# jac99/Egonn

Hardware: AMD Instinct MI355X
Metric: LiDAR scans/sec (descriptor extraction), 50k-pt clouds @ 0.1m voxel (higher is better)
Workload: dtype f32

## Files before the change

### egonn_amd/_lib.py

```python
from __future__ import annotations

import ctypes as C
import os
from typing import List, Optional, Sequence

import numpy as np
import torch

_HERE = os.path.dirname(os.path.abspath(__file__))
LIB_PATH = os.path.join(_HERE, "lib", "libegonn_hip.so")

QUANT_CARTESIAN, QUANT_POLAR = 0, 1
FLAG_DISABLE_GLOBAL, FLAG_DISABLE_LOCAL, FLAG_IGNORE_KP_REGRESSOR, FLAG_BF16 = 1, 2, 4, 8
FLAG_POOL_SPOC, FLAG_POOL_MAC = 16, 32
MINKFPN_SPLIT_TOPDOWN = 1
MINKFPN_BLOCKS = {'BasicBlock': 0, 'ECABasicBlock': 1}
MINKFPN_POOLING = {None: 0, 'GeM': 1, 'MAC': 2, 'SPoC': 3}

_P = C.c_void_p
_SIGS = [
    ("egonn_ctx_create", C.c_int, [C.POINTER(_P), C.c_int, C.c_int]),
    ("egonn_ctx_destroy", None, [_P]),
    ("egonn_last_error", C.c_char_p, []),
    ("egonn_debug_set_naive_conv", C.c_int, [_P, C.c_int]),
    ("egonn_debug_set_ksplit", C.c_int, [_P, C.c_int, C.c_int, C.c_int, C.c_int, C.c_int]),
    ("egonn_debug_set_resident", C.c_int, [_P, C.c_int, C.c_int]),
    ("egonn_debug_keep_level_features", C.c_int, [_P, C.c_int]),
    ("egonn_debug_set_trace", C.c_int, [_P]),
    ("egonn_prepare_maps", C.c_int, [_P, C.c_int, _P]),
    ("egonn_debug_rowgroup_tables", C.c_int, [_P, C.c_int, C.c_int, _P, _P, C.c_int64, C.POINTER(C.c_int64), _P]),
    ("egonn_debug_rowgroup_perm", C.c_int, [_P, C.c_int, C.c_int, _P, C.c_int64, C.POINTER(C.c_int64), _P]),
    ("egonn_debug_radix_sort_scratch_bytes", C.c_int64, [C.c_int64, C.c_int]),
    ("egonn_debug_radix_sort", C.c_int, [_P, _P, _P, _P, C.c_int64, C.c_int, _P, _P, C.c_int, C.c_int, C.c_int,
                                         C.POINTER(C.c_int32), _P, C.c_int64, _P]),
    ("egonn_debug_dense_group3", C.c_int, [_P, _P, _P, _P, _P, _P, _P]),
    ("egonn_debug_global_tail_scratch_bytes", C.c_int64, [C.c_int64]),
    ("egonn_debug_global_tail", C.c_int, [_P, _P, C.c_int, C.c_int64, _P, _P, _P, _P, _P, _P, C.c_int, C.c_int, _P, _P, _P, C.c_int64, _P]),
    ("egonn_voxelize", C.c_int, [_P, _P, C.POINTER(C.c_int64), C.c_int, C.c_int, C.POINTER(C.c_float), _P]),
    ("egonn_ctx_reserve", C.c_int, [_P, C.c_int64, C.c_int, C.POINTER(C.c_int64)]),
    ("egonn_voxelize_device", C.c_int, [_P, _P, C.c_int64, _P, C.c_int, C.c_int, C.POINTER(C.c_float), _P]),
    ("egonn_plan_status", C.c_int, [_P, _P]),
    ("egonn_ctx_set_exact_fp32", C.c_int, [_P, C.c_int]),
    ("egonn_ctx_set_operand_autoscale", C.c_int, [_P, C.c_int]),
    ("egonn_level_capacity", C.c_int, [_P, C.c_int, C.POINTER(C.c_int64)]),
    ("egonn_graph_begin", C.c_int, [_P]),
    ("egonn_graph_end", C.c_int, [_P, C.POINTER(_P)]),
    ("egonn_graph_launch", C.c_int, [_P, _P]),
    ("egonn_graph_destroy", None, [_P]),
    ("egonn_coords_set", C.c_int, [_P, _P, C.c_int64, C.c_int, _P]),
    ("egonn_level_count", C.c_int, [_P, C.c_int, C.POINTER(C.c_int64)]),
    ("egonn_level_batch_offsets", C.c_int, [_P, C.c_int, C.POINTER(C.c_int64)]),
    ("egonn_level_coords", C.c_int, [_P, C.c_int, _P, _P]),
    ("egonn_input_index", C.c_int, [_P, _P, _P]),
    ("egonn_conv", C.c_int, [_P, C.c_int, C.c_int, C.c_int, _P, C.c_int, _P, C.c_int, _P, _P, C.c_int, _P, _P]),
    ("egonn_conv_transpose", C.c_int, [_P, C.c_int, _P, C.c_int, _P, C.c_int, _P, _P]),
    ("egonn_sparse_conv", C.c_int, [_P, C.c_int, C.c_int, _P, C.c_int, _P, C.c_int, C.c_int, _P, _P, C.c_int, _P, _P, _P]),
    ("egonn_map_groups", C.c_int, [_P, C.c_int, C.c_int, C.POINTER(C.c_int64), C.POINTER(C.c_int64), _P]),
    ("egonn_global_avg_pool", C.c_int, [_P, C.c_int, _P, C.c_int, _P, _P]),
    ("egonn_bn_fold", C.c_int, [_P, _P, _P, _P, C.c_float, C.c_int, _P, _P, _P]),
    ("egonn_block_tail", C.c_int, [_P, C.c_int, _P, _P, C.c_int, _P, C.c_int, _P, _P]),
    ("egonn_gem", C.c_int, [_P, C.c_int, _P, C.c_int, _P, _P, _P]),
    ("egonn_global_max_pool", C.c_int, [_P, C.c_int, _P, C.c_int, _P, _P]),
    ("egonn_netvlad", C.c_int, [_P, C.c_int, _P, C.c_int, _P, _P, _P, _P, _P, _P, _P, _P, _P, _P, C.c_int, C.c_int, _P, _P]),
    ("egonn_netvlad_train_forward", C.c_int, [_P, C.c_int, _P, C.c_int, C.c_int, _P, _P, _P, _P, C.c_float, C.c_float, _P, _P,
                                              _P, C.c_int, _P, _P, _P, _P, _P, _P, _P]),
    ("egonn_netvlad_train_backward", C.c_int, [_P, C.c_int, _P, C.c_int, C.c_int, _P, _P, _P, _P, C.c_int, _P, _P, _P, _P, _P,
                                               _P, _P, _P, _P, _P, _P, _P]),
    ("egonn_global_max_pool_argmax", C.c_int, [_P, C.c_int, _P, C.c_int, _P, _P, _P]),
    ("egonn_global_max_pool_backward", C.c_int, [_P, C.c_int, _P, _P, C.c_int, _P, _P]),
    ("egonn_sigmoid_gate", C.c_int, [_P, _P, _P, C.c_int64, _P, _P, _P, _P]),
    ("egonn_add", C.c_int, [_P, _P, C.c_int64, _P, _P]),
    ("egonn_gather_input", C.c_int, [_P, _P, C.c_int, _P, _P]),
    ("egonn_model_create", C.c_int, [C.POINTER(_P)]),
    ("egonn_model_destroy", None, [_P]),
    ("egonn_model_set_tensor", C.c_int, [_P, C.c_char_p, _P, C.c_int, C.POINTER(C.c_int64)]),
    ("egonn_model_finalize", C.c_int, [_P, _P]),
    ("egonn_forward", C.c_int, [_P, _P, _P, C.c_int, C.POINTER(C.c_float), C.c_int, _P, _P, _P, _P, _P]),
    ("egonn_forward_level_features", C.c_int, [_P, C.c_int, _P, C.c_int, _P]),
    ("egonn_minkfpn_finalize", C.c_int, [_P, C.c_int, C.POINTER(C.c_int), C.POINTER(C.c_int), C.c_int, C.c_int, C.c_int, C.c_int, _P]),
    ("egonn_minkfpn_out_level", C.c_int, [C.c_int, C.c_int, C.POINTER(C.c_int)]),
    ("egonn_minkfpn_forward", C.c_int, [_P, _P, C.c_int, _P, _P, _P]),
    ("egonn_topdown_step", C.c_int, [_P, C.c_int, _P, _P, _P, _P, C.c_int, C.c_int, _P, _P]),
    ("egonn_select_keypoints", C.c_int, [_P, _P, _P, _P, C.c_int, _P, _P, _P, _P, _P]),
    ("egonn_topk_rows", C.c_int, [_P, _P, C.c_int, C.c_int, _P, _P, _P]),
    ("egonn_triplet_loss_scratch_floats", C.c_int64, [C.c_int]),
    ("egonn_triplet_loss", C.c_int, [_P, C.c_int, C.c_int, _P, _P, C.c_float, _P, _P, _P, _P, _P]),
    ("egonn_nn_search", C.c_int, [_P, C.c_int64, _P, _P, C.c_int64, _P, _P, _P]),
    ("egonn_matrix_min", C.c_int, [_P, C.c_int64, C.c_int64, _P, _P, _P, _P, _P]),
    ("egonn_softmax_cross_entropy", C.c_int, [_P, C.c_int64, C.c_int64, _P, _P, _P, _P, _P]),
    ("egonn_local_loss_scratch_bytes", C.c_int64, [C.c_int, C.c_int64, C.c_int64, C.c_int]),
    ("egonn_local_loss", C.c_int, [C.c_int, C.c_int64, C.c_int64, C.c_int64, C.c_int64, C.c_int] + [_P] * 13 +
                                  [C.POINTER(C.c_float)] + [_P] * 9 + [C.c_int64, _P]),
    ("egonn_dense", C.c_int, [_P, C.c_int64, C.c_int, _P, C.c_int, _P, C.c_int, C.c_int, _P, _P]),
    ("egonn_dense_pack_fragments", C.c_int, [_P, C.c_int, C.c_int, C.c_int, _P, _P]),
    ("egonn_dense_pack_fragments_host", C.c_int, [_P, C.c_int, C.c_int, C.c_int, _P]),
    ("egonn_debug_dense", C.c_int, [_P, C.c_int, C.c_int64, _P, C.c_int, C.c_int, _P, C.c_int, _P, _P, _P, _P, C.c_int, _P, C.c_int,
                                    _P, _P, C.c_int, _P, C.c_int, C.c_int, _P]),
    ("egonn_debug_dense_route", C.c_int, [C.c_int64, C.c_int, C.c_int, C.c_int, C.c_int, C.POINTER(C.c_int32)]),
    ("egonn_debug_sconv_choice", C.c_int, [C.POINTER(C.c_int32), C.c_int64, C.POINTER(C.c_int32)]),
    ("egonn_dense_backward_weight", C.c_int, [_P, C.c_int, _P, C.c_int, C.c_int64, _P, _P, C.c_int64, _P]),
    ("egonn_conv_backward_weight", C.c_int, [_P, C.c_int, C.c_int, C.c_int, C.c_int, _P, C.c_int, _P, C.c_int, _P, _P,
                                             C.c_int64, _P]),
    ("egonn_col_stats", C.c_int, [C.c_int, _P, _P, _P, _P, C.c_int64, C.c_int, _P, _P, C.c_int64, _P]),
    ("egonn_bn_train_finalize", C.c_int, [_P, _P, C.c_double, C.c_int, _P, _P, C.c_float, C.c_float, _P, _P, _P, _P]),
    ("egonn_bn_backward_finalize", C.c_int, [_P, _P, C.c_double, C.c_int, _P, _P, _P, _P, _P]),
    ("egonn_affine_act", C.c_int, [_P, _P, _P, C.c_int64, C.c_int, C.c_int, _P, _P]),
    ("egonn_affine3", C.c_int, [_P, _P, _P, _P, _P, _P, C.c_int64, C.c_int, _P, _P]),
    ("egonn_relu_backward", C.c_int, [_P, _P, C.c_int64, C.c_int, _P, _P]),
    ("egonn_contrastive_loss_scratch_floats", C.c_int64, [C.c_int]),
    ("egonn_contrastive_loss", C.c_int, [_P, C.c_int, C.c_int, _P, _P, C.c_float, C.c_float, _P, _P, _P, _P, _P]),
    ("egonn_se_gate", C.c_int, [_P, _P, _P, _P, _P, C.c_int, C.c_int, C.c_int, _P, _P, _P]),
    ("egonn_se_gate_backward", C.c_int, [_P, _P, _P, _P, _P, _P, C.c_int, C.c_int, C.c_int, _P, _P, _P, _P, _P, _P]),
    ("egonn_eca_gate", C.c_int, [_P, _P, C.c_int, C.c_int, C.c_int, _P, _P]),
    ("egonn_eca_gate_backward", C.c_int, [_P, _P, _P, _P, C.c_int, C.c_int, C.c_int, _P, _P, _P]),
    ("egonn_act_backward", C.c_int, [C.c_int, _P, _P, C.c_int64, C.c_int, _P, _P]),
    ("egonn_l2_normalize", C.c_int, [_P, _P, C.c_int64, C.c_int, _P, _P]),
    ("egonn_gate_residual", C.c_int, [_P, C.c_int, _P, _P, _P, C.c_int, C.c_int, _P, _P]),
    ("egonn_gate_residual_backward", C.c_int, [_P, C.c_int, _P, _P, _P, C.c_int, _P, _P, _P]),
    ("egonn_segment_sums", C.c_int, [_P, C.c_int, C.c_int, _P, _P, _P, _P, C.c_int, _P, _P, C.c_int64, _P]),
    ("egonn_segment_broadcast", C.c_int, [_P, C.c_int, _P, C.c_int, C.c_int, _P, _P]),
    ("egonn_gem_backward", C.c_int, [_P, C.c_int, _P, _P, _P, C.c_int, _P, _P]),
    ("egonn_filter_points_scratch_ints", C.c_int64, [C.c_int64]),
    ("egonn_filter_points", C.c_int, [_P, C.c_int64, C.c_int, _P, C.c_int, C.c_int, C.c_int, C.c_float, _P, _P, _P,
                                      C.c_int64, _P]),
    ("egonn_knn", C.c_int, [_P, C.c_int64, _P, C.c_int64, C.c_int, C.c_int, _P, _P, _P, C.c_int64, _P]),
    ("egonn_recall_counts", C.c_int, [_P, _P, _P, C.c_int64, C.c_int, C.c_int, _P, C.c_int, _P, _P]),
    ("egonn_registration_scratch_bytes", C.c_int64, [C.c_int, C.c_int, C.c_int]),
    ("egonn_match_mutual_scratch_bytes", C.c_int64, [C.c_int, C.c_int]),
    ("egonn_match_mutual", C.c_int, [_P, _P, _P, _P, C.c_int, C.c_int, C.c_int, _P, _P, _P, C.c_int64, _P]),
    ("egonn_ransac_pairs", C.c_int, [_P, _P, _P, _P, _P, _P, _P, C.c_int, C.c_int, C.c_int, C.c_uint64, C.c_double, _P,
                                     C.c_int64, _P, _P, _P]),
    ("egonn_registration_finish", C.c_int, [_P, _P, _P, _P, _P, _P, _P, C.c_int, C.c_int, C.c_int, C.c_uint64, C.c_double, _P,
                                            C.c_int64, _P, C.c_double, _P, _P, _P, _P, _P, _P, _P, _P, _P, _P, _P, _P]),
    ("egonn_spectral_verify_scratch_bytes", C.c_int64, [C.c_int, C.c_int]),
    ("egonn_spectral_verify", C.c_int, [_P] * 6 + [C.c_int, C.c_int, C.c_double, C.c_int, C.c_double, C.c_double, _P, C.c_double,
                                        _P, C.c_int64] + [_P] * 15),
    ("egonn_voxel_downsample_scratch_bytes", C.c_int64, [C.c_int64, C.c_int]),
    ("egonn_voxel_downsample", C.c_int, [_P, C.c_int64, _P, C.c_int, C.c_double, C.POINTER(C.c_float), _P, _P, _P, _P, _P,
                                         C.c_int64, _P]),
    ("egonn_icp_scratch_bytes", C.c_int64, [C.c_int64, C.c_int64, C.c_int]),
    ("egonn_icp_pairs", C.c_int, [_P, C.c_int64, _P, _P, C.c_int64, _P, C.c_int, _P, C.c_double, C.c_int, C.c_double, C.c_double,
                                  _P, _P, _P, _P, _P, _P, _P, _P, _P, C.c_int64, _P]),
    ("egonn_estimate_normals_scratch_bytes", C.c_int64, [C.c_int64, C.c_int]),
    ("egonn_estimate_normals", C.c_int, [_P, C.c_int64, _P, C.c_int, C.c_int, _P, _P, _P, _P, _P, C.c_int64, _P]),
    ("egonn_icp_plane_scratch_bytes", C.c_int64, [C.c_int64, C.c_int64, C.c_int]),
    ("egonn_icp_plane_pairs", C.c_int, [_P, C.c_int64, _P, _P, C.c_int64, _P, _P, C.c_int, _P, C.c_double, C.c_int, C.c_double,
                                        C.c_double, _P, _P, _P, _P, _P, _P, _P, _P, _P, C.c_int64, _P]),
    ("egonn_augment_scratch_bytes", C.c_int64, [C.c_int64, C.c_int]),
    ("egonn_augment_points", C.c_int, [_P, C.c_int64, _P, C.c_int, _P, _P, _P, _P, _P, _P, _P, _P, _P, C.c_int64, _P]),
    ("egonn_scan_context", C.c_int, [_P, C.c_int64, _P, C.c_int, C.c_int, C.c_int, C.c_double, C.c_double, _P, _P, _P]),
    ("egonn_scan_context_ringkey", C.c_int, [_P, C.c_int64, C.c_int, C.c_int, _P, _P]),
    ("egonn_scan_context_distance", C.c_int, [_P, C.c_int64, _P, C.c_int64, C.c_int, C.c_int, _P, C.c_int, _P, _P, _P]),
    ("egonn_scan_context_rerank", C.c_int, [_P, _P, _P, C.c_int64, C.c_int, _P, _P, _P, _P]),
    ("egonn_radius_count", C.c_int, [_P, C.c_int64, _P, C.c_int64, C.POINTER(C.c_double), C.c_int, C.c_int, _P, _P]),
    ("egonn_radius_fill", C.c_int, [_P, C.c_int64, _P, C.c_int64, C.c_double, C.c_int, _P, _P, C.c_int64, _P, _P]),
    ("egonn_pair_masks", C.c_int, [_P, C.c_int, _P, _P, C.c_int64, _P, _P, C.c_int64, C.c_int64, _P, _P, _P, _P]),
    ("egonn_relative_poses", C.c_int, [_P, C.c_int64, _P, _P, C.c_int64, C.c_int, _P, _P, _P]),
    ("egonn_gather_clouds", C.c_int, [_P, C.c_int64, _P, C.c_int64, _P, C.c_int, _P, C.c_int64, _P, _P, _P]),
    ("egonn_match_candidates_scratch_bytes", C.c_int64, [C.c_int, C.c_int, C.c_int]),
    ("egonn_match_candidates", C.c_int, [_P, _P, _P, _P, _P, C.c_int, C.c_int, C.c_int, C.c_int, C.c_int, _P, _P, _P, _P,
                                         C.c_int64, _P]),
    ("egonn_gather_candidates", C.c_int, [_P, _P, _P, _P, _P, _P, C.c_int, C.c_int, C.c_int, C.c_int, _P, _P, _P, _P, _P, _P]),
    ("egonn_pick_candidates", C.c_int, [_P, C.c_int, C.c_int, C.c_int, _P, _P, _P, _P, _P, _P, _P, _P, C.c_int] + [_P] * 12),
    ("egonn_time_windows", C.c_int, [_P, C.c_int64, _P, C.c_int64, C.c_double, C.c_double, _P, _P, _P, _P]),
    ("egonn_knn_window_scratch_bytes", C.c_int64, [C.c_int64, C.c_int]),
    ("egonn_knn_window", C.c_int, [_P, C.c_int64, _P, C.c_int64, C.c_int, C.c_int, _P, _P, _P, _P, _P, C.c_int64, _P]),
    ("egonn_window_radius", C.c_int, [_P, C.c_int64, _P, C.c_int64, C.c_int, _P, _P, C.c_float, _P, _P, _P, _P]),
    ("egonn_pr_curve_scratch_bytes", C.c_int64, [C.c_int64]),
    ("egonn_pr_curve", C.c_int, [_P, _P, _P, C.c_int64, _P, _P, _P, _P, _P, _P, _P, C.c_int64, _P]),
    ("egonn_pose_graph_scratch_bytes", C.c_int64, [C.c_int64, C.c_int64, C.c_int]),
    ("egonn_pose_graph_odometry", C.c_int, [_P, C.c_int64, _P, _P, _P]),
    ("egonn_pose_graph_plan", C.c_int, [_P, _P, _P, _P, C.c_int64, C.c_int64, _P, _P, _P, C.c_int64, _P]),
    ("egonn_pose_graph_cost", C.c_int, [_P, C.c_int64, C.c_int64, _P, C.c_double, _P, _P, _P, _P, _P, _P, _P, C.c_int64, _P]),
    ("egonn_pose_graph_hessvec", C.c_int, [_P, C.c_int64, C.c_int64, _P, C.c_double, C.c_double, _P, _P, _P, _P, C.c_int64, _P]),
    ("egonn_pose_graph_optimize", C.c_int, [_P, C.c_int64, C.c_int64, _P, C.c_double, C.c_int, C.c_int] + [C.c_double] * 6 +
     [_P] * 8 + [C.c_int64, _P]),
    ("egonn_loop_consistency_scratch_bytes", C.c_int64, [C.c_int64, C.c_int]),
    ("egonn_loop_consistency", C.c_int, [_P, C.c_int64, _P, _P, _P, C.c_int64, C.c_int] + [C.c_double] * 4 + [C.c_int] * 3 +
     [_P] * 8 + [C.c_int64, _P]),
    ("egonn_loop_cycle_errors", C.c_int, [_P, C.c_int64, _P, _P, C.c_int64, _P, C.c_int64, _P, _P]),
    ("egonn_profile_enable", C.c_int, [_P, C.c_int, C.c_char_p]),
    ("egonn_profile_fetch", C.c_int, [_P, C.c_int, C.POINTER(C.c_int), C.c_char_p, C.POINTER(C.c_float),
                                      C.POINTER(C.c_double), C.POINTER(C.c_double), _P]),
]
EXPORTED_SYMBOLS = [s[0] for s in _SIGS]

_lib = None


def load() -> C.CDLL:
# ... 48 lines not shown

def _ptr(t: Optional[torch.Tensor]) -> Optional[int]:
    return None if t is None else t.data_ptr()


def call(device: torch.device, fn, *args):
    idx = device.index
    if idx is None or torch.cuda.current_device() == idx:
        rc = fn(*args, _stream())
    else:
        with torch.cuda.device(device):
            rc = fn(*args, _stream())
    if rc != 0:
        check(rc)


def _dev_f32(t: torch.Tensor, device) -> torch.Tensor:
    return t.to(device=device, dtype=torch.float32).contiguous()


def as_dev(x, dev, dtype) -> torch.Tensor:
    return torch.as_tensor(x).to(device=dev, dtype=dtype).contiguous()


def scratch(nbytes: int, dev) -> torch.Tensor:
    return torch.empty((max(int(nbytes), 8) + 7) // 8, dtype=torch.int64, device=dev)


def check_cloud(name, x):
    shape = tuple(getattr(x, "shape", ()))
    if len(shape) != 2 or shape[1] != 3:
        raise ValueError(f"{name}: expected (n, 3) points, got shape {shape}")


def check_offsets(name, off) -> int:
    shape = tuple(getattr(off, "shape", (len(off),) if hasattr(off, "__len__") else ()))
    if len(shape) != 1 or shape[0] < 2:
        raise ValueError(f"{name}: offsets must be a 1-D sequence of n_clouds + 1 entries, got shape {shape}")
    return shape[0] - 1


def concat_clouds(clouds, dev):
    ts = [torch.as_tensor(c) for c in clouds]
    for c in ts:
        check_cloud("cloud", c)
    off = [0]
    for c in ts:
        off.append(off[-1] + c.shape[0])
    pts = torch.cat([c.to(device=dev, dtype=torch.float32) for c in ts]) if ts else torch.zeros((0, 3), device=dev)
    return pts, torch.tensor(off, dtype=torch.int64, device=dev)


def dense_pack_fragments(weight, out_in: bool):
    lib = load()
    co, ci = (weight.shape if out_in else weight.shape[::-1])
    if isinstance(weight, np.ndarray):
        w = np.ascontiguousarray(weight, dtype=np.float32)
        out = np.empty(ci * co, dtype=np.float32)
        check(lib.egonn_dense_pack_fragments_host(w.ctypes.data, int(bool(out_in)), int(ci), int(co), out.ctypes.data))
        return out
    w = weight.contiguous()
    out = torch.empty(ci * co, dtype=torch.float32, device=w.device)
    call(w.device, lib.egonn_dense_pack_fragments, w.data_ptr(), int(bool(out_in)), int(ci), int(co), out.data_ptr())
    return out


def debug_dense(x, weight, out_in: bool, out, form: int, n_dev=None, packed=None, bias=None, scale=None, shift=None, act: int = 0,
                residual=None, gate=None, boff=None):
    lib = load()
    cap, cin = x.shape
    cout = out.shape[1]
    B = 0 if boff is None else boff.numel() - 1
    bf = lambda t: int(t is not None and t.dtype == torch.bfloat16)
    call(x.device, lib.egonn_debug_dense, x.data_ptr(), bf(x), int(cap), _ptr(n_dev), int(cin), int(cout), weight.data_ptr(),
         int(bool(out_in)), _ptr(packed), _ptr(bias), _ptr(scale), _ptr(shift), int(act), _ptr(residual), bf(residual), _ptr(gate),
         _ptr(boff), B, out.data_ptr(), bf(out), int(form))
    return out


CONV_PRODUCT, CONV_PLAIN, CONV_RING, CONV_COOP, CONV_RING2, CONV_DMA, CONV_DMA3, CONV_TRACED = 0, 1, 2, 4, 8, 16, 32, 128
CONV_SPLIT = 1000
CFG_NW4, CFG_NW8, CFG_RESIDENT = 142, 182, 183
CFG_PARTS, CFG_TRACED = 400, 9000
SCONV_ROUTES = ("plain", "split", "tail_split", "wg", "dma", "rg")
SCONV_CHOICE_FIELDS = ("route", "kernel", "NW", "NSW", "KW", "KS", "GATED", "TRACE", "resident", "KSP", "D", "G", "SPLIT", "PIPE",
                       "gx", "gy", "gz", "block", "lds", "kparts")


def debug_sconv_choice(kind: int, level: int, cin: int, cout: int, cap_groups: int, *, code: int = 0, bf16: int = 0, gated: int = 0,
                       split_io: int = 0, residual: int = 0, split_max_level: int = 5, autoscale: int = 0, resident_mask: int = -1,
                       max_workgroups: int = 0, kparts: int = -1, kw: int = -1, col_parts: int = -1) -> dict:
    arg = (C.c_int32 * 16)(int(code), kind, level, cin, cout, int(bf16), int(gated), split_io, int(residual), split_max_level,
                           int(autoscale), resident_mask, max_workgroups, kparts, kw, col_parts)
    out = (C.c_int32 * 20)()
    check(load().egonn_debug_sconv_choice(arg, int(cap_groups), out))
    d = dict(zip(SCONV_CHOICE_FIELDS, out))
    d["route"], d["kernel"] = SCONV_ROUTES[d["route"]], SCONV_ROUTES[d["kernel"]]
    return d


DENSE_ROUTES = ("none", "stream", "lds", "small", "tile", "plain")


def debug_dense_route(rows: int, cin: int, cout: int, form: int = -1, gate_scans: int = 0):
    out = (C.c_int32 * 5)()
    check(load().egonn_debug_dense_route(int(rows), int(cin), int(cout), int(form), int(gate_scans), out))
    return (DENSE_ROUTES[out[0]],) + tuple(out[1:])


def debug_radix_sort(keys_in, vals_in, keys_out, vals_out, n: int, nbits: int, n_dev=None, seg_offsets=None, idx_bits: int = 0,
                     either_pair: bool = False, scratch_buf=None, scratch_bytes: Optional[int] = None) -> int:
    lib = load()
    B = 0 if seg_offsets is None else seg_offsets.numel() - 1
    need = lib.egonn_debug_radix_sort_scratch_bytes(int(n), B)
    if scratch_buf is None:
        scratch_buf = scratch(need, keys_in.device)
    pair = C.c_int32(-1)
    call(keys_in.device, lib.egonn_debug_radix_sort, keys_in.data_ptr(), vals_in.data_ptr(), keys_out.data_ptr(),
         vals_out.data_ptr(), int(n), int(nbits), _ptr(n_dev), _ptr(seg_offsets), B, int(idx_bits), int(bool(either_pair)),
         C.byref(pair), scratch_buf.data_ptr(), need if scratch_bytes is None else int(scratch_bytes))
    return pair.value


def debug_dense_group3(xs, capacities, counts, ws, packed: bool):
    lib = load()
    dev = xs[0].device
    arr = lambda ptrs: (C.c_void_p * 3)(*ptrs)
    nds = [torch.tensor([int(c)], dtype=torch.int32, device=dev) for c in counts]
    pks = [dense_pack_fragments(w, False) for w in ws] if packed else [None] * 3
    bufs = [torch.full((max(int(c), 1), 128), -12345.0, dtype=torch.float32, device=dev) for c in capacities]
    call(dev, lib.egonn_debug_dense_group3, arr([x.data_ptr() for x in xs]), (C.c_int64 * 3)(*[int(c) for c in capacities]),
         arr([n.data_ptr() for n in nds]), arr([w.data_ptr() for w in ws]), arr([_ptr(p) for p in pks]),
         arr([b.data_ptr() for b in bufs]))
    return [b[:int(c)] for b, c in zip(bufs, capacities)]


GLOBAL_TAIL_POOLING = {"GeM": 1, "MAC": 2, "SPoC": 3}


def debug_global_tail(g5, row_offsets, n_dev, w0, b0, w1, b1, p, pooling: str, form: int):
    lib = load()
    B = row_offsets.numel() - 1
    cap = g5.shape[0]
    need = lib.egonn_debug_global_tail_scratch_bytes(int(cap))
    buf = scratch(need, g5.device)
    partial = torch.empty((B, 32, 256), dtype=torch.float32, device=g5.device)
    out = torch.empty((B, 256), dtype=torch.float32, device=g5.device)
    call(g5.device, lib.egonn_debug_global_tail, g5.data_ptr(), row_offsets.data_ptr(), B, int(cap), n_dev.data_ptr(), w0.data_ptr(),
         b0.data_ptr(), w1.data_ptr(), b1.data_ptr(), _ptr(p), GLOBAL_TAIL_POOLING[pooling], int(form), partial.data_ptr(),
         out.data_ptr(), buf.data_ptr(), need)
    return partial, out


def require_gpu() -> torch.device:
    if not torch.cuda.is_available():
        raise RuntimeError("egonn_amd: no HIP device visible (torch.cuda.is_available() is False); "
                           "the descriptor-extraction path runs on MI355X only — there is no CPU fallback.")
    return torch.device("cuda", torch.cuda.current_device())


class Context:

    def __init__(self, device: Optional[torch.device] = None, coord_bits: int = 16):
        self.lib = load()
        self.device = torch.device(device) if device is not None else require_gpu()
        if self.device.type != "cuda":
            raise RuntimeError(f"egonn_amd: device {self.device} is not a HIP device; there is no CPU fallback.")
        if self.device.index is None:
            self.device = torch.device("cuda", torch.cuda.current_device())
        h = _P()
        check(self.lib.egonn_ctx_create(C.byref(h), self.device.index, coord_bits))
        self.h = h
        self.batch_size = 0
        self._keep = []

    def __del__(self):
        try:
            if getattr(self, "h", None):
                self.lib.egonn_ctx_destroy(self.h)
                self.h = None
        except Exception:
            pass

    def voxelize(self, points: torch.Tensor, scan_offsets: Sequence[int], mode: int, step: Sequence[float]):
        assert points.is_cuda and points.dtype == torch.float32 and points.is_contiguous()
        assert points.dim() == 2 and points.shape[1] == 3
        B = len(scan_offsets) - 1
        off = (C.c_int64 * (B + 1))(*[int(o) for o in scan_offsets])
        st = (C.c_float * 3)(*([float(s) for s in step] + [0.0, 0.0])[:3])
        self._call(self.lib.egonn_voxelize, self.h, points.data_ptr(), off, B, mode, st)
        self.batch_size = B

    def reserve(self, max_points: int, batch_size: int, level_capacity: Optional[Sequence[int]] = None):
        caps = None
        if level_capacity is not None:
            assert len(level_capacity) == 8
            caps = (C.c_int64 * 8)(*[int(v) for v in level_capacity])
        with torch.cuda.device(self.device):
            check(self.lib.egonn_ctx_reserve(self.h, int(max_points), int(batch_size), caps))
        self.batch_size = int(batch_size)

    def voxelize_device(self, points: torch.Tensor, scan_offsets: torch.Tensor, batch_size: int, mode: int,
                        step: Sequence[float]):
        assert points.is_cuda and points.dtype == torch.float32 and points.is_contiguous() and points.shape[1] == 3
        assert scan_offsets.is_cuda and scan_offsets.dtype == torch.int64 and scan_offsets.numel() == batch_size + 1
        st = (C.c_float * 3)(*([float(s) for s in step] + [0.0, 0.0])[:3])
        self._call(self.lib.egonn_voxelize_device, self.h, points.data_ptr(), points.shape[0], scan_offsets.data_ptr(),
                   int(batch_size), mode, st)
        self.batch_size = int(batch_size)

    def plan_status(self):
        self._call(self.lib.egonn_plan_status, self.h)

    def level_capacity(self, level: int) -> int:
        n = C.c_int64()
        check(self.lib.egonn_level_capacity(self.h, level, C.byref(n)))
        return n.value

    def coords_set(self, coords: torch.Tensor, batch_size: int):
        assert coords.is_cuda and coords.dtype == torch.int32 and coords.is_contiguous()
        assert coords.dim() == 2 and coords.shape[1] == 4
        self._call(self.lib.egonn_coords_set, self.h, coords.data_ptr(), coords.shape[0], int(batch_size))
        self.batch_size = int(batch_size)

    def level_count(self, level: int) -> int:
        n = C.c_int64()
        check(self.lib.egonn_level_count(self.h, level, C.byref(n)))
        return n.value

    def level_batch_offsets(self, level: int) -> List[int]:
        off = (C.c_int64 * (self.batch_size + 1))()
        check(self.lib.egonn_level_batch_offsets(self.h, level, off))
        return list(off)

    def level_coords(self, level: int) -> torch.Tensor:
        out = torch.empty((self.level_count(level), 4), dtype=torch.int32, device=self.device)
        self._call(self.lib.egonn_level_coords, self.h, level, out.data_ptr())
        return out

    def input_index(self) -> torch.Tensor:
        out = torch.empty((self.level_count(0),), dtype=torch.int64, device=self.device)
        self._call(self.lib.egonn_input_index, self.h, out.data_ptr())
        return out

    def conv(self, level_in: int, level_out: int, kernel_size: int, x: torch.Tensor, kernel: torch.Tensor,
             scale: Optional[torch.Tensor] = None, shift: Optional[torch.Tensor] = None, relu: bool = False):
        kernel = _dev_f32(kernel, self.device)
        cin, cout = kernel.shape[-2], kernel.shape[-1]
        if x is None:
            assert kernel_size == 5 and cin == 1, "x=None (all-ones features) is the k=5 input layer only"
        else:
            x = _dev_f32(x, self.device)
            assert x.shape == (self.level_count(level_in), cin), (x.shape, self.level_count(level_in), cin)
        out = torch.empty((self.level_count(level_out), cout), dtype=torch.float32, device=self.device)
        sc = None if scale is None else _dev_f32(scale, self.device)
        sh = None if shift is None else _dev_f32(shift, self.device)
        self._call(self.lib.egonn_conv, self.h, level_in, level_out, kernel_size, _ptr(x), cin, kernel.data_ptr(), cout,
                   _ptr(sc), _ptr(sh), int(relu), out.data_ptr())
        return out

    def conv_transpose(self, level_in: int, x: torch.Tensor, kernel: torch.Tensor):
        x = _dev_f32(x, self.device)
        kernel = _dev_f32(kernel, self.device)
        cin, cout = kernel.shape[-2], kernel.shape[-1]
        assert x.shape == (self.level_count(level_in), cin)
        out = torch.empty((self.level_count(level_in - 1), cout), dtype=torch.float32, device=self.device)
        self._call(self.lib.egonn_conv_transpose, self.h, level_in, x.data_ptr(), cin, kernel.data_ptr(), cout, out.data_ptr())
        return out

    def sparse_conv(self, map_kind: int, level_out: int, x: torch.Tensor, kernel: torch.Tensor, scale=None, shift=None,
                    relu: bool = False, group_sums: bool = False):
        assert x.is_cuda and x.dtype in (torch.float32, torch.bfloat16) and x.is_contiguous()
        kernel = _dev_f32(kernel, self.device)
        cin, cout = kernel.shape[-2], kernel.shape[-1]
        assert x.shape[1] == cin
        out = torch.empty((self.level_count(level_out), cout), dtype=x.dtype, device=self.device)
        sc = None if scale is None else _dev_f32(scale, self.device)
        sh = None if shift is None else _dev_f32(shift, self.device)
        sums = None
        if group_sums:
            sums = torch.zeros((self.map_groups(map_kind, level_out)[0], cout), dtype=torch.float32, device=self.device)
        self._call(self.lib.egonn_sparse_conv, self.h, map_kind, level_out, x.data_ptr(), cin, kernel.data_ptr(), cout,
                   int(x.dtype == torch.bfloat16), _ptr(sc), _ptr(sh), int(relu), out.data_ptr(), _ptr(sums))
        return (out, sums) if group_sums else out

    def prepare_maps(self, with_level0_transpose: bool = False):
        self._call(self.lib.egonn_prepare_maps, self.h, int(with_level0_transpose))

    def map_groups(self, map_kind: int, level_out: int):
        n = C.c_int64()
        first = (C.c_int64 * (self.batch_size + 1))()
        self._call(self.lib.egonn_map_groups, self.h, map_kind, level_out, C.byref(n), first)
        return n.value, list(first)

    def rowgroup_tables(self, map_kind: int, level_out: int, with_rows: bool = True):
        ng, _ = self.map_groups(map_kind, level_out)
        K = 27 if map_kind == 0 else 8
        gm = torch.empty(ng, dtype=torch.int32, device=self.device)
        sn = torch.empty((ng, K, 16), dtype=torch.int32, device=self.device) if with_rows else None
        n = C.c_int64()
        self._call(self.lib.egonn_debug_rowgroup_tables, self.h, map_kind, level_out, gm.data_ptr(),
                   sn.data_ptr() if with_rows else None, ng, C.byref(n))
        return gm, sn

    def rowgroup_perm(self, map_kind: int, level_out: int):
        ng, _ = self.map_groups(map_kind, level_out)
# ... 409 lines not shown
```

### egonn_amd/csrc/conv.hip

```cpp
#include <algorithm>
#include <type_traits>
#include <utility>

#include "common.h"
#include <hip/hip_ext.h>
#include "kernels.h"
#include "rowmath.h"

namespace egonn {

__global__ void sconv_naive_kernel(const float* __restrict__ in, const int32_t* __restrict__ nbr,
                                   const float* __restrict__ W, const float* __restrict__ scale,
                                   const float* __restrict__ shift, int relu, float* __restrict__ out, int32_t n_out,
                                   int K, int cin, int cout) {
  const int64_t t = (int64_t)blockIdx.x * blockDim.x + threadIdx.x;
  if (t >= (int64_t)n_out * cout) return;
  const int32_t o = (int32_t)(t / cout);
  const int co = (int)(t - (int64_t)o * cout);
  float acc = 0.f;
  for (int k = 0; k < K; ++k) {
    const int32_t j = nbr[(int64_t)o * K + k];
    if (j < 0) continue;
    const float* f = in + (int64_t)j * cin;
    const float* w = W + ((int64_t)k * cin) * cout + co;
    float part = 0.f;
    for (int ci = 0; ci < cin; ++ci) part = fmaf(f[ci], w[(int64_t)ci * cout], part);
    acc += part;
  }
  if (scale) acc = acc * scale[co] + shift[co];
  if (relu) acc = fmaxf(acc, 0.f);
  out[t] = acc;
}

int sconv_naive(const float* in, const int32_t* nbr, const float* W, const float* scale, const float* shift, int relu,
                float* out, int64_t n_out, int K, int cin, int cout, hipStream_t stream) {
  if (n_out == 0) return EGONN_OK;
  const int64_t total = n_out * cout;
  hipLaunchKernelGGL(sconv_naive_kernel, dim3((unsigned)cdiv(total, 256)), dim3(256), 0, stream, in, nbr, W, scale,
                     shift, relu, out, (int32_t)n_out, K, cin, cout);
  HIP_CHECK(hipGetLastError());
  return EGONN_OK;
}

static constexpr int COUT0 = 32;

template <bool UNIT, bool OUT_BF16>
__global__ __launch_bounds__(256) void conv0_k5_kernel(const float* __restrict__ feat,
                                                        const uint64_t* __restrict__ vkeys,
                                                        const int32_t* __restrict__ g0,
                                                        const uint64_t* __restrict__ t2m,
                                                        const int32_t* __restrict__ t2s,
                                                        const int32_t* __restrict__ counts,
                                                        int32_t cap2, int32_t cap0,
                                                        const float* __restrict__ W,
                                                        const float* __restrict__ scale,
                                                        const float* __restrict__ shift, int relu,
                                                        void* __restrict__ out_v,
                                                        const uint16_t* __restrict__ lut) {
  constexpr int MS = 29;
  __shared__ uint64_t s_m[4][16][MS];
  __shared__ int32_t s_s[4][16][27];
  constexpr int LUT_STRIDE = 132;
  __shared__ __attribute__((aligned(8))) uint16_t s_lut[64 * LUT_STRIDE];
  const int tid = threadIdx.x, lane = tid & 63, wave = tid >> 6;
  const int l15 = lane & 15, g4 = lane >> 4;
  const int32_t nvox = min(__builtin_amdgcn_readfirstlane(counts[0]), cap0);
  const int32_t n2 = min(__builtin_amdgcn_readfirstlane(counts[2]), cap2);
  const int32_t ntiles = (nvox + 15) >> 4;
  for (int e = tid; e < 64 * 128 / 2; e += 256) {
    const int r = e >> 6, c = e & 63;
    reinterpret_cast<uint32_t*>(s_lut)[r * (LUT_STRIDE / 2) + c] = reinterpret_cast<const uint32_t*>(lut)[e];
  }
  if (tid < 64) s_m[tid >> 4][tid & 15][27] = 0ull;
  float breg[2][32];
#pragma unroll
  for (int q = 0; q < 32; ++q) {
    const int k = 16 * (q >> 2) + 4 * g4 + (q & 3);
#pragma unroll
    for (int nt = 0; nt < 2; ++nt) breg[nt][q] = (k < 125) ? W[k * COUT0 + nt * 16 + l15] : 0.f;
  }
  f32x4 sc[2], sh[2];
#pragma unroll
  for (int nt = 0; nt < 2; ++nt) {
    sc[nt] = scale ? *reinterpret_cast<const f32x4*>(scale + nt * 16 + 4 * g4) : (f32x4){1.f, 1.f, 1.f, 1.f};
    sh[nt] = scale ? *reinterpret_cast<const f32x4*>(shift + nt * 16 + 4 * g4) : (f32x4){0.f, 0.f, 0.f, 0.f};
  }
  __syncthreads();
  const __amdgpu_buffer_rsrc_t m_rsrc =
      __builtin_amdgcn_make_buffer_rsrc(const_cast<uint64_t*>(t2m), 0, (int)((uint32_t)n2 * 27u * 8u), 0x00020000);
  const __amdgpu_buffer_rsrc_t s_rsrc =
      __builtin_amdgcn_make_buffer_rsrc(const_cast<int32_t*>(t2s), 0, (int)((uint32_t)n2 * 27u * 4u), 0x00020000);
  const int tstep = gridDim.x * 4;
  constexpr int NE = (16 * 27 + 63) / 64;
  uint64_t pm[NE];
  int32_t ps[NE];
  const __amdgpu_buffer_rsrc_t g_rsrc =
      __builtin_amdgcn_make_buffer_rsrc(const_cast<int32_t*>(g0), 0, (int)((uint32_t)nvox * 4u), 0x00020000);
  const __amdgpu_buffer_rsrc_t k_rsrc =
      __builtin_amdgcn_make_buffer_rsrc(const_cast<uint64_t*>(vkeys), 0, (int)((uint32_t)nvox * 8u), 0x00020000);
  auto row_info = [&](int32_t tile, int32_t& g, uint32_t& lkbits) {
    const uint32_t r = (uint32_t)tile * 16u + (uint32_t)l15;
    g = __builtin_amdgcn_raw_buffer_load_b32(g_rsrc, (int)(r * 4u), 0, 0);
    lkbits = (uint32_t)__builtin_amdgcn_raw_buffer_load_b32(k_rsrc, (int)(r * 8u), 0, 0) & 63u;
  };
  auto table_issue = [&](int32_t g_of_lane) {
#pragma unroll
    for (int e = 0; e < NE; ++e) {
      const int idx = lane + 64 * e;
      const int row = idx / 27, slot = idx - row * 27;
      const int32_t g = __shfl(g_of_lane, row & 15, 64);
      const uint32_t ent = (idx < 16 * 27) ? (uint32_t)g * 27u + (uint32_t)slot : 0x3FFFFFFFu;
      const auto m2 = __builtin_amdgcn_raw_buffer_load_b64(m_rsrc, (int)(ent * 8u), 0, 0);
      pm[e] = ((uint64_t)m2[1] << 32) | (uint64_t)m2[0];
      ps[e] = __builtin_amdgcn_raw_buffer_load_b32(s_rsrc, (int)(ent * 4u), 0, 0);
    }
  };
  int32_t tile = blockIdx.x * 4 + wave;
  int32_t g_cur, g_nxt;
  uint32_t lk_cur, lk_nxt, lk_nn;
  int32_t g_nn;
  row_info(tile, g_cur, lk_cur);
  row_info(tile + tstep, g_nxt, lk_nxt);
  table_issue(g_cur);
  for (; tile < ntiles; tile += tstep) {
    const int32_t r0 = tile * 16;
#pragma unroll
    for (int e = 0; e < NE; ++e) {
      const int idx = lane + 64 * e;
      if (idx < 16 * 27) {
        const int row = idx / 27, slot = idx - row * 27;
        s_m[wave][row][slot] = pm[e];
        (&s_s[wave][0][0])[idx] = ps[e];
      }
    }
    __builtin_amdgcn_fence(__ATOMIC_ACQ_REL, "wavefront");
    __builtin_amdgcn_wave_barrier();
    table_issue(g_nxt);
    row_info(tile + 2 * tstep, g_nn, lk_nn);
    const uint32_t lk = lk_cur;
    const uint16_t* lrow = s_lut + lk * LUT_STRIDE + 4 * g4;
    uint2 ent4[8];
#pragma unroll
    for (int j = 0; j < 8; ++j) ent4[j] = *reinterpret_cast<const uint2*>(lrow + 16 * j);
    float a[32];
    const char* mrow = reinterpret_cast<const char*>(&s_m[wave][l15][0]);
#pragma unroll
    for (int q = 0; q < 32; ++q) {
      const uint32_t pair = (q & 2) ? ent4[q >> 2].y : ent4[q >> 2].x;
      const uint32_t en = (q & 1) ? (pair >> 16) : (pair & 0xFFFFu);
      const uint64_t m = *reinterpret_cast<const uint64_t*>(mrow + (en >> 6));
      const uint32_t hit = (uint32_t)(m >> (en & 63)) & 1u;
      float v = (float)hit;
      if constexpr (!UNIT) {
        v = 0.f;
        if (hit) v = feat[s_s[wave][l15][en >> 9] + __popcll(m & ((1ull << (en & 63)) - 1))];
      }
      a[q] = v;
    }
    f32x4 acc[2] = {{0.f, 0.f, 0.f, 0.f}, {0.f, 0.f, 0.f, 0.f}};
#pragma unroll
    for (int q = 0; q < 32; ++q) {
      acc[0] = __builtin_amdgcn_mfma_f32_16x16x4f32(breg[0][q], a[q], acc[0], 0, 0, 0);
      acc[1] = __builtin_amdgcn_mfma_f32_16x16x4f32(breg[1][q], a[q], acc[1], 0, 0, 0);
    }
    const int32_t orow = r0 + l15;
    if (orow < nvox) {
#pragma unroll
      for (int nt = 0; nt < 2; ++nt) {
        f32x4 o = acc[nt] * sc[nt] + sh[nt];
        if (relu) {
#pragma unroll
          for (int u = 0; u < 4; ++u) o[u] = fmaxf(o[u], 0.f);
        }
        if constexpr (OUT_BF16) {
          uint32_t w[4];
#pragma unroll
          for (int u = 0; u < 4; ++u) {
            uint32_t x = __float_as_uint(o[u]);
            x += 0x7FFFu + ((x >> 16) & 1u);
            w[u] = x >> 16;
          }
          *reinterpret_cast<uint2*>(reinterpret_cast<uint16_t*>(out_v) + (int64_t)orow * COUT0 + nt * 16 + 4 * g4) =
              make_uint2(w[0] | (w[1] << 16), w[2] | (w[3] << 16));
        } else {
          *reinterpret_cast<f32x4*>(reinterpret_cast<float*>(out_v) + (int64_t)orow * COUT0 + nt * 16 + 4 * g4) = o;
        }
      }
    }
    __builtin_amdgcn_wave_barrier();
    g_cur = g_nxt; lk_cur = lk_nxt;
    g_nxt = g_nn; lk_nxt = lk_nn;
  }
}

typedef short bf16x8_c0 __attribute__((ext_vector_type(8)));
template <bool OUT_BF16>
__global__ __launch_bounds__(256) void conv0_k5_unit_kernel(const uint64_t* __restrict__ vkeys,
                                                             const int32_t* __restrict__ g0,
                                                             const uint64_t* __restrict__ t2m,
                                                             const int32_t* __restrict__ counts, int32_t cap2, int32_t cap0,
                                                             const float* __restrict__ W,
                                                             const float* __restrict__ scale, const float* __restrict__ shift,
                                                             int relu, void* __restrict__ out_v,
                                                             const uint16_t* __restrict__ lut,
                                                             const uint4* __restrict__ wpk) {
  constexpr int MS = 29;
  constexpr int LUT_STRIDE = 136;
  __shared__ uint64_t s_m[4][16][MS];
  __shared__ __attribute__((aligned(16))) uint16_t s_lut[64 * LUT_STRIDE];
  const int tid = threadIdx.x, lane = tid & 63, wave = tid >> 6;
  const int l15 = lane & 15, g4 = lane >> 4;
  const int32_t nvox = min(__builtin_amdgcn_readfirstlane(counts[0]), cap0);
  const int32_t n2 = min(__builtin_amdgcn_readfirstlane(counts[2]), cap2);
  const int32_t ntiles = (nvox + 15) >> 4;
  for (int e = tid; e < 64 * 128 / 2; e += 256) {
    const int r = e >> 6, c = e & 63;
    reinterpret_cast<uint32_t*>(s_lut)[r * (LUT_STRIDE / 2) + c] = reinterpret_cast<const uint32_t*>(lut)[e];
  }
  if (tid < 64) s_m[tid >> 4][tid & 15][27] = 0ull;
  bf16x8_c0 wf[2][4][3];
  if (wpk) {
#pragma unroll
    for (int nt = 0; nt < 2; ++nt)
#pragma unroll
      for (int j = 0; j < 4; ++j)
#pragma unroll
        for (int sp = 0; sp < 3; ++sp) wf[nt][j][sp] = __builtin_bit_cast(bf16x8_c0, wpk[((nt * 4 + j) * 3 + sp) * 64 + lane]);
  } else
#pragma unroll
  for (int nt = 0; nt < 2; ++nt)
#pragma unroll
    for (int j = 0; j < 4; ++j) {
      uint32_t h[3][8];
#pragma unroll
      for (int e = 0; e < 8; ++e) {
        const int k = 32 * j + 8 * g4 + e;
        float w = (k < 125) ? W[k * COUT0 + nt * 16 + l15] : 0.f;
#pragma unroll
        for (int sp = 0; sp < 3; ++sp) {
          const uint32_t b = f2bf_rn(w);
          h[sp][e] = b;
          w -= __uint_as_float(b << 16);
        }
      }
#pragma unroll
      for (int sp = 0; sp < 3; ++sp) {
        const uint4 pk = make_uint4(h[sp][0] | (h[sp][1] << 16), h[sp][2] | (h[sp][3] << 16), h[sp][4] | (h[sp][5] << 16),
                                    h[sp][6] | (h[sp][7] << 16));
        wf[nt][j][sp] = __builtin_bit_cast(bf16x8_c0, pk);
      }
    }
  f32x4 sc[2], sh[2];
#pragma unroll
  for (int nt = 0; nt < 2; ++nt) {
    sc[nt] = scale ? *reinterpret_cast<const f32x4*>(scale + nt * 16 + 4 * g4) : (f32x4){1.f, 1.f, 1.f, 1.f};
    sh[nt] = scale ? *reinterpret_cast<const f32x4*>(shift + nt * 16 + 4 * g4) : (f32x4){0.f, 0.f, 0.f, 0.f};
  }
  __syncthreads();
  const __amdgpu_buffer_rsrc_t m_rsrc =
      __builtin_amdgcn_make_buffer_rsrc(const_cast<uint64_t*>(t2m), 0, (int)((uint32_t)n2 * 27u * 8u), 0x00020000);
  const __amdgpu_buffer_rsrc_t g_rsrc =
      __builtin_amdgcn_make_buffer_rsrc(const_cast<int32_t*>(g0), 0, (int)((uint32_t)nvox * 4u), 0x00020000);
  const __amdgpu_buffer_rsrc_t k_rsrc =
      __builtin_amdgcn_make_buffer_rsrc(const_cast<uint64_t*>(vkeys), 0, (int)((uint32_t)nvox * 8u), 0x00020000);
  const int tstep = gridDim.x * 4;
  constexpr int NE = (16 * 27 + 63) / 64;
  uint64_t pm[NE];
  auto row_info = [&](int32_t tile, int32_t& g, uint32_t& lkbits) {
    const uint32_t r = (uint32_t)tile * 16u + (uint32_t)l15;
    g = __builtin_amdgcn_raw_buffer_load_b32(g_rsrc, (int)(r * 4u), 0, 0);
    lkbits = (uint32_t)__builtin_amdgcn_raw_buffer_load_b32(k_rsrc, (int)(r * 8u), 0, 0) & 63u;
  };
  auto table_issue = [&](int32_t g_of_lane) {
#pragma unroll
    for (int e = 0; e < NE; ++e) {
      const int idx = lane + 64 * e;
      const int row = idx / 27, slot = idx - row * 27;
      const int32_t g = __shfl(g_of_lane, row & 15, 64);
      const uint32_t ent = (idx < 16 * 27) ? (uint32_t)g * 27u + (uint32_t)slot : 0x3FFFFFFFu;
      const auto m2 = __builtin_amdgcn_raw_buffer_load_b64(m_rsrc, (int)(ent * 8u), 0, 0);
      pm[e] = ((uint64_t)m2[1] << 32) | (uint64_t)m2[0];
    }
  };
  int32_t tile = blockIdx.x * 4 + wave;
  int32_t g_cur, g_nxt, g_nn;
  uint32_t lk_cur, lk_nxt, lk_nn;
  row_info(tile, g_cur, lk_cur);
  row_info(tile + tstep, g_nxt, lk_nxt);
  table_issue(g_cur);
  for (; tile < ntiles; tile += tstep) {
    const int32_t r0 = tile * 16;
#pragma unroll
    for (int e = 0; e < NE; ++e) {
      const int idx = lane + 64 * e;
      if (idx < 16 * 27) {
        const int row = idx / 27, slot = idx - row * 27;
        s_m[wave][row][slot] = pm[e];
      }
    }
    __builtin_amdgcn_fence(__ATOMIC_ACQ_REL, "wavefront");
    __builtin_amdgcn_wave_barrier();
    table_issue(g_nxt);
    row_info(tile + 2 * tstep, g_nn, lk_nn);
    const uint16_t* lrow = s_lut + lk_cur * LUT_STRIDE + 8 * g4;
    const char* mrow = reinterpret_cast<const char*>(&s_m[wave][l15][0]);
    f32x4 acc[2] = {{0.f, 0.f, 0.f, 0.f}, {0.f, 0.f, 0.f, 0.f}};
#pragma unroll
    for (int j = 0; j < 4; ++j) {
      const uint4 ent = *reinterpret_cast<const uint4*>(lrow + 32 * j);
      const uint32_t ew[4] = {ent.x, ent.y, ent.z, ent.w};
      uint32_t pk[4];
#pragma unroll
      for (int q = 0; q < 4; ++q) {
        const uint32_t e0 = ew[q] & 0xFFFFu, e1 = ew[q] >> 16;
        const uint64_t m0 = *reinterpret_cast<const uint64_t*>(mrow + (e0 >> 6));
        const uint64_t m1 = *reinterpret_cast<const uint64_t*>(mrow + (e1 >> 6));
        const uint32_t h0 = (uint32_t)(m0 >> (e0 & 63)) & 1u, h1 = (uint32_t)(m1 >> (e1 & 63)) & 1u;
        pk[q] = h0 * 0x3F80u + h1 * 0x3F800000u;
      }
      const bf16x8_c0 av = __builtin_bit_cast(bf16x8_c0, make_uint4(pk[0], pk[1], pk[2], pk[3]));
#pragma unroll
      for (int sp = 0; sp < 3; ++sp)
#pragma unroll
        for (int nt = 0; nt < 2; ++nt) acc[nt] = __builtin_amdgcn_mfma_f32_16x16x32_bf16(wf[nt][j][sp], av, acc[nt], 0, 0, 0);
    }
    const int32_t orow = r0 + l15;
    if (orow < nvox) {
#pragma unroll
      for (int nt = 0; nt < 2; ++nt) {
        f32x4 o = acc[nt] * sc[nt] + sh[nt];
        if (relu) {
#pragma unroll
          for (int u = 0; u < 4; ++u) o[u] = fmaxf(o[u], 0.f);
        }
        if constexpr (OUT_BF16) {
          *reinterpret_cast<uint2*>(reinterpret_cast<uint16_t*>(out_v) + (int64_t)orow * COUT0 + nt * 16 + 4 * g4) =
              make_uint2(f2bf_rn(o[0]) | (f2bf_rn(o[1]) << 16), f2bf_rn(o[2]) | (f2bf_rn(o[3]) << 16));
        } else {
          *reinterpret_cast<f32x4*>(reinterpret_cast<float*>(out_v) + (int64_t)orow * COUT0 + nt * 16 + 4 * g4) = o;
        }
      }
    }
    __builtin_amdgcn_wave_barrier();
    g_cur = g_nxt; lk_cur = lk_nxt;
    g_nxt = g_nn; lk_nxt = lk_nn;
  }
}

__global__ void conv0_pack_unit_kernel(const float* __restrict__ W, uint4* __restrict__ wpk) {
  const int t = blockIdx.x * blockDim.x + threadIdx.x;
  if (t >= 2 * 4 * 64) return;
  const int lane = t & 63, j = (t >> 6) & 3, nt = t >> 8;
  const int l15 = lane & 15, g4 = lane >> 4;
  uint32_t h[3][8];
#pragma unroll
  for (int e = 0; e < 8; ++e) {
    const int k = 32 * j + 8 * g4 + e;
    float w = (k < 125) ? W[k * COUT0 + nt * 16 + l15] : 0.f;
#pragma unroll
    for (int sp = 0; sp < 3; ++sp) {
      const uint32_t b = f2bf_rn(w);
      h[sp][e] = b;
      w -= __uint_as_float(b << 16);
    }
  }
#pragma unroll
  for (int sp = 0; sp < 3; ++sp)
    wpk[((nt * 4 + j) * 3 + sp) * 64 + lane] = make_uint4(h[sp][0] | (h[sp][1] << 16), h[sp][2] | (h[sp][3] << 16),
                                                          h[sp][4] | (h[sp][5] << 16), h[sp][6] | (h[sp][7] << 16));
}
int conv0_pack_unit(const float* W, void* wpk, hipStream_t stream) {
  hipLaunchKernelGGL(conv0_pack_unit_kernel, dim3(2), dim3(256), 0, stream, W, reinterpret_cast<uint4*>(wpk));
  HIP_CHECK(hipGetLastError());
  return EGONN_OK;
}

static void conv0_lut_host(uint16_t* lut) {
  for (int lk = 0; lk < 64; ++lk)
    for (int k = 0; k < 128; ++k) {
      uint32_t v = (uint32_t)(27 * 8) << 6;
      if (k < 125) {
        const int lx = (lk & 1) | ((lk >> 2) & 2), ly = ((lk >> 1) & 1) | ((lk >> 3) & 2), lz = ((lk >> 2) & 1) | ((lk >> 4) & 2);
        const int nx = lx + k % 5 - 2, ny = ly + (k / 5) % 5 - 2, nz = lz + k / 25 - 2;
        const int slot = ((nx < 0) ? 0 : (nx > 3 ? 2 : 1)) + 3 * ((ny < 0) ? 0 : (ny > 3 ? 2 : 1)) +
                         9 * ((nz < 0) ? 0 : (nz > 3 ? 2 : 1));
        const uint32_t ux = (uint32_t)nx & 3, uy = (uint32_t)ny & 3, uz = (uint32_t)nz & 3;
        const uint32_t bit = (ux & 1) | ((uy & 1) << 1) | ((uz & 1) << 2) | ((ux & 2) << 2) | ((uy & 2) << 3) | ((uz & 2) << 4);
        v = ((uint32_t)(slot * 8) << 6) | bit;
      }
      lut[lk * 128 + k] = (uint16_t)v;
    }
}

int conv0_lut_init(Ctx* ctx) {
  if (ctx->conv0_lut) return EGONN_OK;
  std::vector<uint16_t> h(64 * 128);
  conv0_lut_host(h.data());
  HIP_CHECK(hipMalloc(reinterpret_cast<void**>(&ctx->conv0_lut), h.size() * sizeof(uint16_t)));
  HIP_CHECK(hipMemcpy(ctx->conv0_lut, h.data(), h.size() * sizeof(uint16_t), hipMemcpyHostToDevice));
  return EGONN_OK;
}

int conv0_k5_forward(Ctx* ctx, const float* feat, const float* W, int cout, const float* scale,
                     const float* shift, int relu, void* out, int out_bf16, hipStream_t stream, const void* wpk) {
  const Plan& P = ctx->plan;
  EGONN_TRY(conv0_lut_init(ctx));
  EGONN_REQUIRE(cout == COUT0, EGONN_ERR_INVALID, "conv0: %d output channels not supported (expected %d)", cout, COUT0);
  const Level& V = P.lv[0];
  const Level& B = P.lv[2];
  if (P.cap[0] == 0) return EGONN_OK;
  const int32_t ntiles = (int32_t)cdiv(P.cap[0], 16);
  const unsigned grid = (unsigned)std::min<int64_t>(cdiv(ntiles, 4), 512);
  EGONN_REQUIRE(P.g0 && P.t2m && P.t2s, EGONN_ERR_STATE, "conv0: plan has no block-neighbourhood table");
#define EGONN_CONV0_LAUNCH(U, OB)                                                                                      \
  hipLaunchKernelGGL((conv0_k5_kernel<U, OB>), dim3(grid), dim3(256), 0, stream, feat, V.keys, P.g0, P.t2m, P.t2s,       \
                     ctx->dev_counts, (int32_t)P.cap[2], (int32_t)P.cap[0], W, scale, shift, relu, out, ctx->conv0_lut)
  if (feat) {
    if (out_bf16) EGONN_CONV0_LAUNCH(false, true); else EGONN_CONV0_LAUNCH(false, false);
  } else if (ctx->sconv.set.family == SCONV_PLAIN) {
    if (out_bf16) EGONN_CONV0_LAUNCH(true, true); else EGONN_CONV0_LAUNCH(true, false);
  } else {
    if (out_bf16)
      hipLaunchKernelGGL((conv0_k5_unit_kernel<true>), dim3(grid), dim3(256), 0, stream, V.keys, P.g0, P.t2m, ctx->dev_counts,
                         (int32_t)P.cap[2], (int32_t)P.cap[0], W, scale, shift, relu, out, ctx->conv0_lut,
                         reinterpret_cast<const uint4*>(wpk));
    else
      hipLaunchKernelGGL((conv0_k5_unit_kernel<false>), dim3(grid), dim3(256), 0, stream, V.keys, P.g0, P.t2m, ctx->dev_counts,
                         (int32_t)P.cap[2], (int32_t)P.cap[0], W, scale, shift, relu, out, ctx->conv0_lut,
                         reinterpret_cast<const uint4*>(wpk));
  }
#undef EGONN_CONV0_LAUNCH
  HIP_CHECK(hipGetLastError());
  return EGONN_OK;
}

}
```

### egonn_amd/csrc/heads.hip

```cpp
#include <algorithm>

#include "common.h"
#include "kernels.h"
#include "rowmath.h"
#include "split16.h"

namespace egonn {

__device__ static inline void keypoint_position(uint64_t key, int level, int cb, float ox, float oy, float oz, int mode,
                                                float s0, float s1, float s2, float* __restrict__ out3) {
  const int cbL = cb - level;
  const uint64_t mort = key & ((1ull << (3 * cbL)) - 1);
  const int32_t bias = 1 << (cb - 1);
  const float cx = (float)(((int32_t)compact1by2(mort) << level) - bias);
  const float cy = (float)(((int32_t)compact1by2(mort >> 1) << level) - bias);
  const float cz = (float)(((int32_t)compact1by2(mort >> 2) << level) - bias);
  const float stride = (float)(1 << level);
  const float px = __fadd_rn(__fmul_rn(__fadd_rn(cx, 0.5f), s0), __fdiv_rn(__fmul_rn(ox, __fmul_rn(stride, s0)), 2.f));
  const float py = __fadd_rn(__fmul_rn(__fadd_rn(cy, 0.5f), s1), __fdiv_rn(__fmul_rn(oy, __fmul_rn(stride, s1)), 2.f));
  const float pz = __fadd_rn(__fmul_rn(__fadd_rn(cz, 0.5f), s2), __fdiv_rn(__fmul_rn(oz, __fmul_rn(stride, s2)), 2.f));
  if (mode == 0) {
    out3[0] = px; out3[1] = py; out3[2] = pz;
  } else {
    const float theta = __fdiv_rn(__fmul_rn(3.14159265358979323846f, __fadd_rn(px, -180.f)), 180.f);
    out3[0] = cosf(theta) * py;
    out3[1] = sinf(theta) * py;
    out3[2] = pz;
  }
}

__global__ void keypoint_kernel(const uint64_t* __restrict__ keys, int64_t n, int level, int cb,
                                const float* __restrict__ offs, int mode, float s0, float s1, float s2, int ignore,
                                float* __restrict__ out, const int32_t* __restrict__ n_dev) {
  const int64_t i = (int64_t)blockIdx.x * blockDim.x + threadIdx.x;
  if (n_dev) n = min((int64_t)*n_dev, n);
  if (i >= n) return;
  const float kox = ignore ? 0.f : offs[3 * i + 0], koy = ignore ? 0.f : offs[3 * i + 1],
              koz = ignore ? 0.f : offs[3 * i + 2];
  keypoint_position(keys[i], level, cb, kox, koy, koz, mode, s0, s1, s2, out + 3 * i);
}
int keypoint_positions(const uint64_t* keys, int64_t n, int level, int cb, const float* offsets, int mode,
                       const float* step, int ignore_offsets, float* out, hipStream_t stream, const int32_t* n_dev) {
  if (n == 0) return EGONN_OK;
  const float s0 = step[0], s1 = mode ? step[1] : step[0], s2 = mode ? step[2] : step[0];
  hipLaunchKernelGGL(keypoint_kernel, dim3((unsigned)cdiv(n, 256)), dim3(256), 0, stream, keys, n, level, cb, offsets,
                     mode, s0, s1, s2, ignore_offsets, out, n_dev);
  HIP_CHECK(hipGetLastError());
  return EGONN_OK;
}

struct LocalHeadsArgs {
  const float* x;
  const float *lw, *lres;
  const float *dw0, *db0, *dw1, *db1;
  const float *kw0, *kb0, *kw1, *kb1;
  const float *sw0, *sb0, *sw1, *sb1;
  const uint64_t* keys;
  const int32_t* n_dev;
  float *out_desc, *out_kp, *out_sigma;
  int64_t n;
  int level, cb, mode, ignore_offsets;
  int in_bf16;
  float s0, s1, s2;
};
template <int CIN, int NT>
__device__ static inline void stage_frags(const float* __restrict__ W, int rows_w, f32x4* __restrict__ dst, int tid, int nthreads) {
  constexpr int T = CIN / 16;
  for (int i = tid; i < NT * T * 64; i += nthreads) {
    const int lane = i & 63, ft = i >> 6;
    const int nt = ft / T, t = ft - nt * T;
    const int unit = 16 * nt + (lane & 15);
    f32x4 v = {0.f, 0.f, 0.f, 0.f};
    if (unit < rows_w) v = *reinterpret_cast<const f32x4*>(W + (int64_t)unit * CIN + 16 * t + 4 * (lane >> 4));
    dst[i] = v;
  }
}
template <int CIN, int NT>
__device__ static inline void mlp_layer(const f32x4* __restrict__ frags, const f32x4* __restrict__ in, int lane,
                                        f32x4* __restrict__ out) {
  constexpr int T = CIN / 16;
#pragma unroll
  for (int nt = 0; nt < NT; ++nt) {
    f32x4 acc = {0.f, 0.f, 0.f, 0.f};
#pragma unroll
    for (int t = 0; t < T; ++t) {
      const f32x4 wf = frags[(nt * T + t) * 64 + lane];
#pragma unroll
      for (int u = 0; u < 4; ++u) acc = __builtin_amdgcn_mfma_f32_16x16x4f32(wf[u], in[t][u], acc, 0, 0, 0);
    }
    out[nt] = acc;
    __builtin_amdgcn_sched_barrier(0);
  }
}
template <int CIN, int NT>
__device__ static inline void stage_frags_t(const float* __restrict__ W, int cout, f32x4* __restrict__ dst, int tid, int nthreads) {
  constexpr int T = CIN / 16;
  for (int i = tid; i < NT * T * 64; i += nthreads) {
    const int lane = i & 63, ft = i >> 6;
    const int nt = ft / T, t = ft - nt * T;
    const float* wp = W + (int64_t)(16 * t + 4 * (lane >> 4)) * cout + 16 * nt + (lane & 15);
    dst[i] = (f32x4){wp[0], wp[cout], wp[2 * (int64_t)cout], wp[3 * (int64_t)cout]};
  }
}
constexpr int LH_F_DW0 = 0, LH_F_DW1 = LH_F_DW0 + 6 * 4, LH_F_KW0 = LH_F_DW1 + 8 * 6, LH_F_KW1 = LH_F_KW0 + 2 * 4,
              LH_F_SW0 = LH_F_KW1 + 1 * 2, LH_F_SW1 = LH_F_SW0 + 2 * 4, LH_FRAGS = LH_F_SW1 + 1 * 2;
__global__ __launch_bounds__(LH_WAVES * 64) void local_heads_kernel(const LocalHeadsArgs p) {
  extern __shared__ __attribute__((aligned(16))) f32x4 lh_frags[];
  const int tid = threadIdx.x, lane = tid & 63, wave = tid >> 6;
  const int l15 = lane & 15, g4 = lane >> 4;
  stage_frags<64, 6>(p.dw0, 96, lh_frags + LH_F_DW0 * 64, tid, LH_WAVES * 64);
  stage_frags<96, 8>(p.dw1, 128, lh_frags + LH_F_DW1 * 64, tid, LH_WAVES * 64);
  stage_frags<64, 2>(p.kw0, 32, lh_frags + LH_F_KW0 * 64, tid, LH_WAVES * 64);
  stage_frags<32, 1>(p.kw1, 3, lh_frags + LH_F_KW1 * 64, tid, LH_WAVES * 64);
  stage_frags<64, 2>(p.sw0, 32, lh_frags + LH_F_SW0 * 64, tid, LH_WAVES * 64);
  stage_frags<32, 1>(p.sw1, 1, lh_frags + LH_F_SW1 * 64, tid, LH_WAVES * 64);
  if (p.lw) stage_frags_t<64, 4>(p.lw, 64, lh_frags + LH_FRAGS * 64, tid, LH_WAVES * 64);
  __syncthreads();
  int64_t n = p.n;
  if (p.n_dev) n = min((int64_t)*p.n_dev, n);
  const int64_t ntiles = (n + 15) >> 4;
  for (int64_t tile = (int64_t)blockIdx.x * LH_WAVES + wave; tile < ntiles; tile += (int64_t)gridDim.x * LH_WAVES) {
    const int64_t row = tile * 16 + l15;
    const bool ok = row < n;
    f32x4 x[4];
    auto load4 = [&](const float* base, int t) -> f32x4 {
      if (!ok) return (f32x4){0.f, 0.f, 0.f, 0.f};
      if (p.in_bf16) {
        const uint2 h = *reinterpret_cast<const uint2*>(reinterpret_cast<const uint16_t*>(base) + row * 64 + 16 * t + 4 * g4);
        return (f32x4){bf2f(h.x & 0xFFFFu), bf2f(h.x >> 16), bf2f(h.y & 0xFFFFu), bf2f(h.y >> 16)};
      }
      return *reinterpret_cast<const f32x4*>(base + row * 64 + 16 * t + 4 * g4);
    };
#pragma unroll
    for (int t = 0; t < 4; ++t) x[t] = load4(p.x, t);
    if (p.lw) {
      f32x4 r[4], l[4];
#pragma unroll
      for (int t = 0; t < 4; ++t) r[t] = load4(p.lres, t);
      mlp_layer<64, 4>(lh_frags + LH_FRAGS * 64, x, lane, l);
#pragma unroll
      for (int t = 0; t < 4; ++t) x[t] = l[t] + r[t];
    }
    {
      f32x4 h[6], o[8];
      mlp_layer<64, 6>(lh_frags + LH_F_DW0 * 64, x, lane, h);
#pragma unroll
      for (int nt = 0; nt < 6; ++nt) {
        const f32x4 b = *reinterpret_cast<const f32x4*>(p.db0 + 16 * nt + 4 * g4);
#pragma unroll
        for (int r = 0; r < 4; ++r) h[nt][r] = fmaxf(h[nt][r] + b[r], 0.f);
      }
      mlp_layer<96, 8>(lh_frags + LH_F_DW1 * 64, h, lane, o);
      float ss = 0.f;
#pragma unroll
      for (int nt = 0; nt < 8; ++nt) {
        const f32x4 b = *reinterpret_cast<const f32x4*>(p.db1 + 16 * nt + 4 * g4);
#pragma unroll
        for (int r = 0; r < 4; ++r) {
          o[nt][r] += b[r];
          ss += o[nt][r] * o[nt][r];
        }
      }
      ss += __shfl_xor(ss, 16, 64);
      ss += __shfl_xor(ss, 32, 64);
      const float inv = 1.f / fmaxf(sqrtf(ss), 1e-12f);
      if (ok) {
#pragma unroll
        for (int nt = 0; nt < 8; ++nt)
          *reinterpret_cast<f32x4*>(p.out_desc + row * 128 + 16 * nt + 4 * g4) = o[nt] * inv;
      }
    }
    {
      f32x4 h[2], o[1];
      mlp_layer<64, 2>(lh_frags + LH_F_KW0 * 64, x, lane, h);
#pragma unroll
      for (int nt = 0; nt < 2; ++nt) {
        const f32x4 b = *reinterpret_cast<const f32x4*>(p.kb0 + 16 * nt + 4 * g4);
#pragma unroll
        for (int r = 0; r < 4; ++r) h[nt][r] = fmaxf(h[nt][r] + b[r], 0.f);
      }
      mlp_layer<32, 1>(lh_frags + LH_F_KW1 * 64, h, lane, o);
      if (ok && g4 == 0) {
        const float ox = p.ignore_offsets ? 0.f : tanhf(o[0][0] + p.kb1[0]);
        const float oy = p.ignore_offsets ? 0.f : tanhf(o[0][1] + p.kb1[1]);
        const float oz = p.ignore_offsets ? 0.f : tanhf(o[0][2] + p.kb1[2]);
        keypoint_position(p.keys[row], p.level, p.cb, ox, oy, oz, p.mode, p.s0, p.s1, p.s2, p.out_kp + row * 3);
      }
    }
    {
      f32x4 h[2], o[1];
      mlp_layer<64, 2>(lh_frags + LH_F_SW0 * 64, x, lane, h);
#pragma unroll
      for (int nt = 0; nt < 2; ++nt) {
        const f32x4 b = *reinterpret_cast<const f32x4*>(p.sb0 + 16 * nt + 4 * g4);
#pragma unroll
        for (int r = 0; r < 4; ++r) h[nt][r] = fmaxf(h[nt][r] + b[r], 0.f);
      }
      mlp_layer<32, 1>(lh_frags + LH_F_SW1 * 64, h, lane, o);
      if (ok && g4 == 0) p.out_sigma[row] = apply_act(o[0][0] + p.sb1[0], ACT_SOFTPLUS);
    }
  }
}
constexpr int LHS_DW0 = 0, LHS_DW1 = LHS_DW0 + 6 * 2, LHS_KW0 = LHS_DW1 + 8 * 3, LHS_KW1 = LHS_KW0 + 2 * 2, LHS_SW0 = LHS_KW1 + 1 * 1,
              LHS_SW1 = LHS_SW0 + 2 * 2, LHS_FRAGS = LHS_SW1 + 1 * 1;
struct LhsMat { int cin, nout, nt, first; };
__constant__ LhsMat lhs_mats[6] = {{64, 96, 6, LHS_DW0}, {96, 128, 8, LHS_DW1}, {64, 32, 2, LHS_KW0}, {32, 3, 1, LHS_KW1},
                                   {64, 32, 2, LHS_SW0}, {32, 1, 1, LHS_SW1}};
__global__ void lhs_absmax_kernel(const float* const* __restrict__ W, uint32_t* __restrict__ trailer) {
  const int mi = blockIdx.x;
  const LhsMat M = lhs_mats[mi];
  const float* w = W[mi];
  const float m = split_finite_absmax(w, M.cin * M.nout, (int)threadIdx.x, blockDim.x);
  if ((threadIdx.x & 63) == 0) atomicMax(trailer + 8 + mi, __float_as_uint(m));
}
__global__ void lhs_pack_kernel(const float* const* __restrict__ W, uint16_t* __restrict__ out, uint32_t* __restrict__ trailer) {
  const int mi = blockIdx.y;
  const LhsMat M = lhs_mats[mi];
  const int KB = M.cin / 32;
  const int t = blockIdx.x * blockDim.x + threadIdx.x;
  const float sc = split_scale_of(trailer[8 + mi]);
  if (t == 0) reinterpret_cast<float*>(trailer)[mi] = 1.f / sc;
  if (t >= M.nt * KB * 2 * 64 * 8) return;
  int r = t;
  const int e = r & 7; r >>= 3;
  const int lane = r & 63; r >>= 6;
  const int part = r & 1; r >>= 1;
  const int kb = r % KB, nt = r / KB;
  const int unit = 16 * nt + (lane & 15), k = 32 * kb + split_chan(lane >> 4, e);
  const float v = unit < M.nout ? sc * W[mi][(int64_t)unit * M.cin + k] : 0.f;
  out[(int64_t)M.first * 2 * 512 + t] = __builtin_bit_cast(uint16_t, split_part(v, part));
}
size_t local_heads_pack_bytes() { return (size_t)LHS_FRAGS * 2048 + 64; }
int local_heads_pack(const float* const* w6_dev , void* out, hipStream_t stream) {
  uint32_t* trailer = reinterpret_cast<uint32_t*>(reinterpret_cast<char*>(out) + (size_t)LHS_FRAGS * 2048);
  HIP_CHECK(hipMemsetAsync(trailer, 0, 64, stream));
  hipLaunchKernelGGL(lhs_absmax_kernel, dim3(6), dim3(256), 0, stream, w6_dev, trailer);
  hipLaunchKernelGGL(lhs_pack_kernel, dim3((8 * 3 * 2 * 64 * 8 + 255) / 256, 6), dim3(256), 0, stream, w6_dev,
                     reinterpret_cast<uint16_t*>(out), trailer);
  HIP_CHECK(hipGetLastError());
  return EGONN_OK;
}
template <int CIN, int NT>
__device__ static inline void lhs_layer(const f32x4* __restrict__ frags , const f32x4* __restrict__ in, int lane,
                                        float winv, f32x4* __restrict__ out) {
  constexpr int KB = CIN / 32;
  f16x8_t ah[KB], al[KB];
#pragma unroll
  for (int kb = 0; kb < KB; ++kb) split8h(in[2 * kb], in[2 * kb + 1], ah[kb], al[kb]);
#pragma unroll
  for (int nt = 0; nt < NT; ++nt) {
    f32x4 acc = {0.f, 0.f, 0.f, 0.f};
#pragma unroll
    for (int kb = 0; kb < KB; ++kb) {
      const f16x8_t wh = __builtin_bit_cast(f16x8_t, frags[((nt * KB + kb) * 2) * 64 + lane]);
      const f16x8_t wl = __builtin_bit_cast(f16x8_t, frags[((nt * KB + kb) * 2 + 1) * 64 + lane]);
      split_mfma3(wh, wl, ah[kb], al[kb], acc);
    }
    out[nt] = acc * winv;
    __builtin_amdgcn_sched_barrier(0);
  }
}
struct LocalHeadsSplitArgs {
  LocalHeadsArgs a;
  const void* pack;
  int32_t* flags;
};
__global__ __launch_bounds__(LH_WAVES * 64) void local_heads_split_kernel(const LocalHeadsSplitArgs q) {
  const LocalHeadsArgs& p = q.a;
  extern __shared__ __attribute__((aligned(16))) f32x4 lh_frags[];
  const int tid = threadIdx.x, lane = tid & 63, wave = tid >> 6;
  const int l15 = lane & 15, g4 = lane >> 4;
  {
    const f32x4* src = reinterpret_cast<const f32x4*>(q.pack);
    for (int i = tid; i < LHS_FRAGS * 2 * 64; i += LH_WAVES * 64) lh_frags[i] = src[i];
  }
  f32x4* const lat = lh_frags + LHS_FRAGS * 2 * 64;
  if (p.lw) stage_frags_t<64, 4>(p.lw, 64, lat, tid, LH_WAVES * 64);
  const float* winv = reinterpret_cast<const float*>(reinterpret_cast<const char*>(q.pack) + (size_t)LHS_FRAGS * 2048);
  const float wi0 = winv[0], wi1 = winv[1], wi2 = winv[2], wi3 = winv[3], wi4 = winv[4], wi5 = winv[5];
  __syncthreads();
  int64_t n = p.n;
  if (p.n_dev) n = min((int64_t)*p.n_dev, n);
  const int64_t ntiles = (n + 15) >> 4;
  for (int64_t tile = (int64_t)blockIdx.x * LH_WAVES + wave; tile < ntiles; tile += (int64_t)gridDim.x * LH_WAVES) {
    const int64_t row = tile * 16 + l15;
    const bool ok = row < n;
    f32x4 x[4];
    auto load4 = [&](const float* base, int t) -> f32x4 {
      if (!ok) return (f32x4){0.f, 0.f, 0.f, 0.f};
      if (p.in_bf16) {
        const uint2 h = *reinterpret_cast<const uint2*>(reinterpret_cast<const uint16_t*>(base) + row * 64 + 16 * t + 4 * g4);
        return (f32x4){bf2f(h.x & 0xFFFFu), bf2f(h.x >> 16), bf2f(h.y & 0xFFFFu), bf2f(h.y >> 16)};
      }
      return *reinterpret_cast<const f32x4*>(base + row * 64 + 16 * t + 4 * g4);
    };
#pragma unroll
    for (int t = 0; t < 4; ++t) x[t] = load4(p.x, t);
    if (p.lw) {
      f32x4 r[4], l[4];
#pragma unroll
      for (int t = 0; t < 4; ++t) r[t] = load4(p.lres, t);
      mlp_layer<64, 4>(lat, x, lane, l);
#pragma unroll
      for (int t = 0; t < 4; ++t) x[t] = l[t] + r[t];
    }
    float guard = 0.f;
    bool outside = false;
#pragma unroll
    for (int t = 0; t < 4; ++t)
#pragma unroll
      for (int r = 0; r < 4; ++r) outside |= !(fabsf(x[t][r]) < SPLIT_FP16_LIMIT);
    {
      f32x4 h[6], o[8];
      lhs_layer<64, 6>(lh_frags + LHS_DW0 * 2 * 64, x, lane, wi0, h);
#pragma unroll
      for (int nt = 0; nt < 6; ++nt) {
        const f32x4 b = *reinterpret_cast<const f32x4*>(p.db0 + 16 * nt + 4 * g4);
#pragma unroll
        for (int r = 0; r < 4; ++r) h[nt][r] = fmaxf(h[nt][r] + b[r], 0.f);
      }
      lhs_layer<96, 8>(lh_frags + LHS_DW1 * 2 * 64, h, lane, wi1, o);
      float ss = 0.f;
#pragma unroll
      for (int nt = 0; nt < 8; ++nt) {
        const f32x4 b = *reinterpret_cast<const f32x4*>(p.db1 + 16 * nt + 4 * g4);
#pragma unroll
        for (int r = 0; r < 4; ++r) {
          o[nt][r] += b[r];
          ss += o[nt][r] * o[nt][r];
        }
      }
      ss += __shfl_xor(ss, 16, 64);
      ss += __shfl_xor(ss, 32, 64);
      guard += split_nonfinite(ss);
      const float inv = 1.f / fmaxf(sqrtf(ss), 1e-12f);
      if (ok) {
#pragma unroll
        for (int nt = 0; nt < 8; ++nt)
          *reinterpret_cast<f32x4*>(p.out_desc + row * 128 + 16 * nt + 4 * g4) = o[nt] * inv;
      }
    }
    {
      f32x4 h[2], o[1];
      lhs_layer<64, 2>(lh_frags + LHS_KW0 * 2 * 64, x, lane, wi2, h);
#pragma unroll
      for (int nt = 0; nt < 2; ++nt) {
        const f32x4 b = *reinterpret_cast<const f32x4*>(p.kb0 + 16 * nt + 4 * g4);
#pragma unroll
        for (int r = 0; r < 4; ++r) h[nt][r] = fmaxf(h[nt][r] + b[r], 0.f);
      }
      lhs_layer<32, 1>(lh_frags + LHS_KW1 * 2 * 64, h, lane, wi3, o);
      if (ok && g4 == 0) {
        guard += split_nonfinite(o[0][0]) + split_nonfinite(o[0][1]) + split_nonfinite(o[0][2]);
        const float ox = p.ignore_offsets ? 0.f : tanhf(o[0][0] + p.kb1[0]);
        const float oy = p.ignore_offsets ? 0.f : tanhf(o[0][1] + p.kb1[1]);
        const float oz = p.ignore_offsets ? 0.f : tanhf(o[0][2] + p.kb1[2]);
        keypoint_position(p.keys[row], p.level, p.cb, ox, oy, oz, p.mode, p.s0, p.s1, p.s2, p.out_kp + row * 3);
      }
    }
    {
      f32x4 h[2], o[1];
      lhs_layer<64, 2>(lh_frags + LHS_SW0 * 2 * 64, x, lane, wi4, h);
#pragma unroll
      for (int nt = 0; nt < 2; ++nt) {
        const f32x4 b = *reinterpret_cast<const f32x4*>(p.sb0 + 16 * nt + 4 * g4);
#pragma unroll
        for (int r = 0; r < 4; ++r) h[nt][r] = fmaxf(h[nt][r] + b[r], 0.f);
      }
      lhs_layer<32, 1>(lh_frags + LHS_SW1 * 2 * 64, h, lane, wi5, o);
      if (ok && g4 == 0) {
        guard += split_nonfinite(o[0][0]);
        p.out_sigma[row] = apply_act(o[0][0] + p.sb1[0], ACT_SOFTPLUS);
      }
    }
    if (ok && (outside || guard != 0.f) && q.flags) split_raise(q.flags);
  }
}

int local_heads_forward(const float* x, int64_t n, const int32_t* n_dev, const float* const* w ,
                        const uint64_t* keys, int level, int cb, int mode, const float* step, int ignore_offsets,
                        float* out_desc, float* out_kp, float* out_sigma, hipStream_t stream, const float* lateral_w,
                        const float* lateral_res, int in_bf16, const void* split_pack, int32_t* flags) {
  if (n == 0) return EGONN_OK;
  EGONN_REQUIRE((lateral_w == nullptr) == (lateral_res == nullptr), EGONN_ERR_INVALID, "local heads: lateral kernel and residual go together");
  LocalHeadsArgs a;
  a.x = x; a.n = n; a.n_dev = n_dev;
  a.lw = lateral_w; a.lres = lateral_res;
  a.in_bf16 = in_bf16 ? 1 : 0;
  EGONN_REQUIRE(!in_bf16 || lateral_w, EGONN_ERR_INVALID, "local heads: bf16 input rows only through the fused lateral");
  a.dw0 = w[0]; a.db0 = w[1]; a.dw1 = w[2]; a.db1 = w[3];
  a.kw0 = w[4]; a.kb0 = w[5]; a.kw1 = w[6]; a.kb1 = w[7];
  a.sw0 = w[8]; a.sb0 = w[9]; a.sw1 = w[10]; a.sb1 = w[11];
  a.keys = keys; a.level = level; a.cb = cb; a.mode = mode; a.ignore_offsets = ignore_offsets;
  a.s0 = step[0]; a.s1 = mode ? step[1] : step[0]; a.s2 = mode ? step[2] : step[0];
  a.out_desc = out_desc; a.out_kp = out_kp; a.out_sigma = out_sigma;
  const int64_t tiles = cdiv(n, 16);
  const size_t lds = (size_t)(LH_FRAGS + (lateral_w ? 16 : 0)) * 64 * sizeof(f32x4);
  static AttrOnce attr_done;
  if (attr_done.need()) {
    HIP_CHECK(hipFuncSetAttribute(reinterpret_cast<const void*>(&local_heads_kernel), hipFuncAttributeMaxDynamicSharedMemorySize, 160 * 1024));
    attr_done.mark(); 
  }
  const unsigned grid = (unsigned)std::min<int64_t>(cdiv(tiles, LH_WAVES), 256);
  if (split_pack) {
    static AttrOnce attr2;
    if (attr2.need()) {
      HIP_CHECK(hipFuncSetAttribute(reinterpret_cast<const void*>(&local_heads_split_kernel), hipFuncAttributeMaxDynamicSharedMemorySize, 160 * 1024));
      attr2.mark();
    }
    LocalHeadsSplitArgs q;
    q.a = a; q.pack = split_pack; q.flags = flags;
    const size_t lds2 = (size_t)(LHS_FRAGS * 2 + (lateral_w ? 16 : 0)) * 64 * sizeof(f32x4);
    hipLaunchKernelGGL(local_heads_split_kernel, dim3(grid), dim3(LH_WAVES * 64), lds2, stream, q);
    HIP_CHECK(hipGetLastError());
    return EGONN_OK;
  }
  hipLaunchKernelGGL(local_heads_kernel, dim3(grid), dim3(LH_WAVES * 64), lds, stream, a);
  HIP_CHECK(hipGetLastError());
  return EGONN_OK;
}

__device__ static inline uint32_t sigma_bits(float v) {
  const uint32_t u = __float_as_uint(v);
  return (u & 0x80000000u) ? ~u : (u | 0x80000000u);
}
constexpr int TK_THREADS = 1024, TK_BINS = 2048, TK_CACHE = 8;
__global__ __launch_bounds__(TK_THREADS) void select_topk_kernel(const float* __restrict__ sigma, const int32_t* __restrict__ boff,
                                                                 int k, int S, const float* __restrict__ kp,
                                                                 const float* __restrict__ desc, int dc,
                                                                 int32_t* __restrict__ sel_rows, int32_t* __restrict__ sel_count,
                                                                 float* __restrict__ out_kp, float* __restrict__ out_desc) {
  extern __shared__ __attribute__((aligned(16))) unsigned long long skeys[];
  __shared__ uint32_t s_hist[TK_BINS];
  __shared__ uint32_t s_wave[TK_THREADS / 64];
  __shared__ uint32_t s_pick[3];
  __shared__ uint32_t s_n;
  const int b = blockIdx.x, tid = threadIdx.x, lane = tid & 63, wave = tid >> 6;
  const int32_t r0 = boff[b], nb = boff[b + 1] - r0;
  const int kk = min(k, nb);
  uint32_t sb[TK_CACHE];
#pragma unroll
  for (int i = 0; i < TK_CACHE; ++i) {
    const int r = i * TK_THREADS + tid;
    sb[i] = r < nb ? sigma_bits(sigma[r0 + r]) : 0xFFFFFFFFu;
  }
  auto key_of = [&](uint32_t bits, int r) { return ((unsigned long long)bits << 32) | (unsigned)r; };
  unsigned long long T = 0;
  if (kk > 0) {
    unsigned long long prefix = 0;
    uint32_t need = (uint32_t)kk;
    const int shifts[6] = {53, 42, 31, 20, 9, 0};
#pragma unroll 1
    for (int p = 0; p < 6; ++p) {
      const int sh = shifts[p], bits = p == 5 ? 9 : 11;
      const uint32_t dmask = (1u << bits) - 1;
      for (int i = tid; i < TK_BINS; i += TK_THREADS) s_hist[i] = 0;
      __syncthreads();
      auto count = [&](uint32_t sbits, int r) {
        const unsigned long long key = key_of(sbits, r);
        if (p == 0 || (key >> (sh + bits)) == prefix) atomicAdd(&s_hist[(uint32_t)(key >> sh) & dmask], 1u);
      };
#pragma unroll
      for (int i = 0; i < TK_CACHE; ++i) {
        const int r = i * TK_THREADS + tid;
        if (r < nb) count(sb[i], r);
      }
      for (int r = TK_CACHE * TK_THREADS + tid; r < nb; r += TK_THREADS) count(sigma_bits(sigma[r0 + r]), r);
      __syncthreads();
      const uint32_t h0 = s_hist[2 * tid], h1 = s_hist[2 * tid + 1];
      uint32_t inc = h0 + h1;
#pragma unroll
      for (int d = 1; d < 64; d <<= 1) {
        const uint32_t o = __shfl_up(inc, d, 64);
        if (lane >= d) inc += o;
      }
      if (lane == 63) s_wave[wave] = inc;
      __syncthreads();
      uint32_t ex = inc - (h0 + h1);
      for (int w = 0; w < wave; ++w) ex += s_wave[w];
      if (ex < need && need <= ex + h0) {
        s_pick[0] = 2 * tid; s_pick[1] = ex; s_pick[2] = h0;
      } else if (ex + h0 < need && need <= ex + h0 + h1) {
        s_pick[0] = 2 * tid + 1; s_pick[1] = ex + h0; s_pick[2] = h1;
      }
      __syncthreads();
      const uint32_t digit = s_pick[0], below = s_pick[1], inbin = s_pick[2];
      prefix = (prefix << bits) | digit;
      need -= below;
      if (inbin == need || sh == 0) {
        T = sh ? ((prefix << sh) | ((1ull << sh) - 1)) : prefix;
        break;
      }
    }
  }
  if (tid == 0) s_n = 0;
  for (int i = tid; i < S; i += TK_THREADS) skeys[i] = ~0ull;
  __syncthreads();
  if (kk > 0) {
    auto take = [&](uint32_t sbits, int r) {
      const unsigned long long key = key_of(sbits, r);
      if (key <= T) skeys[atomicAdd(&s_n, 1u)] = key;
    };
#pragma unroll
    for (int i = 0; i < TK_CACHE; ++i) {
      const int r = i * TK_THREADS + tid;
      if (r < nb) take(sb[i], r);
    }
    for (int r = TK_CACHE * TK_THREADS + tid; r < nb; r += TK_THREADS) take(sigma_bits(sigma[r0 + r]), r);
  }
  __syncthreads();
  if (k <= 512) {
    unsigned long long* sorted = skeys + S;
    if (tid < kk) {
      const unsigned long long mine = skeys[tid];
      int rank = 0;
      for (int j = 0; j < kk; ++j) rank += skeys[j] < mine ? 1 : 0;
      sorted[rank] = mine;
    }
    __syncthreads();
    if (tid < kk) skeys[tid] = sorted[tid];
    __syncthreads();
  } else {
    for (int k2 = 2; k2 <= S; k2 <<= 1)
      for (int j2 = k2 >> 1; j2 > 0; j2 >>= 1) {
        for (int e = tid; e < S / 2; e += TK_THREADS) {
          const int i = ((e & ~(j2 - 1)) << 1) | (e & (j2 - 1));
          const int q = i | j2;
          const bool up = (i & k2) == 0;
          const unsigned long long x = skeys[i], y = skeys[q];
          if ((x > y) == up) { skeys[i] = y; skeys[q] = x; }
        }
        __syncthreads();
      }
  }
  for (int i = tid; i < k; i += TK_THREADS) sel_rows[(int64_t)b * k + i] = (i < kk) ? r0 + (int32_t)(skeys[i] & 0xFFFFFFFFu) : -1;
  if (tid == 0) sel_count[b] = kk;
  if (out_desc) {
    if ((dc & 3) == 0) {
      const int q4 = dc >> 2;
      for (int t = tid; t < k * q4; t += TK_THREADS) {
        const int i = t / q4, c = t - i * q4;
        float4 v = make_float4(0.f, 0.f, 0.f, 0.f);
        if (i < kk) v = *reinterpret_cast<const float4*>(desc + (int64_t)(r0 + (int32_t)(skeys[i] & 0xFFFFFFFFu)) * dc + 4 * c);
        *reinterpret_cast<float4*>(out_desc + ((int64_t)b * k + i) * dc + 4 * c) = v;
      }
    } else {
      for (int64_t t = tid; t < (int64_t)k * dc; t += TK_THREADS) {
        const int i = (int)(t / dc), c = (int)(t - (int64_t)i * dc);
        out_desc[((int64_t)b * k + i) * dc + c] = (i < kk) ? desc[(int64_t)(r0 + (int32_t)(skeys[i] & 0xFFFFFFFFu)) * dc + c] : 0.f;
      }
    }
    for (int t = tid; t < k * 3; t += TK_THREADS) {
      const int i = t / 3, c = t - i * 3;
      out_kp[((int64_t)b * k + i) * 3 + c] = (i < kk) ? kp[(int64_t)(r0 + (int32_t)(skeys[i] & 0xFFFFFFFFu)) * 3 + c] : 0.f;
    }
  }
}
int select_topk(const float* sigma, const int32_t* boff_dev, int B, int k, const float* kp, const float* desc, int dc,
                int32_t* sel_rows, int32_t* sel_count, float* out_kp, float* out_desc, hipStream_t stream) {
  EGONN_REQUIRE(k >= 1 && k <= 8192, EGONN_ERR_INVALID, "select_keypoints: n_k=%d outside [1, 8192]", k);
  int S = 64;
  while (S < k) S <<= 1;
  const size_t lds = (size_t)(S + (k <= 512 ? k : 0)) * sizeof(unsigned long long);
  static AttrOnce attr_done;
  if (attr_done.need()) {
    HIP_CHECK(hipFuncSetAttribute(reinterpret_cast<const void*>(&select_topk_kernel), hipFuncAttributeMaxDynamicSharedMemorySize,
                                  128 * 1024));
    attr_done.mark(); 
  }
  hipLaunchKernelGGL(select_topk_kernel, dim3(B), dim3(TK_THREADS), lds, stream, sigma, boff_dev, k, S, kp, desc, dc, sel_rows,
                     sel_count, out_kp, out_desc);
  HIP_CHECK(hipGetLastError());
// ... 5 lines not shown
```

### egonn_amd/csrc/kernels.h

```cpp
#pragma once
#include "common.h"

namespace egonn {

const char* last_error();

bool sconv_rg_supported(int cin, int cout);
int pack_rg_weights(const float* W, int K, int cin, int cout, int bf16, int flip, int transpose, void* out,
                    hipStream_t stream);
extern unsigned long long* g_sconv_trace;
struct PackedKernel {
  const void* rg32 = nullptr;
  const void* rg16 = nullptr;
  const void* split = nullptr;
};
struct ConvCall {
  int kind = 0, level = 0;
  const void* in = nullptr; void* out = nullptr;
  int cin = 0, cout = 0, bf16 = 0;
  const float *scale = nullptr, *shift = nullptr;
  int relu = 0;
  float* psum = nullptr;
  const PackedKernel* packed = nullptr;
  const float* W = nullptr; float* scratch = nullptr; size_t scratch_floats = 0;
// ... 2 lines not shown
  const float* residual = nullptr;
};
enum SconvRoute {
  ROUTE_PLAIN,
  ROUTE_SPLIT,
  ROUTE_TAIL_SPLIT,
  ROUTE_WG,
  ROUTE_DMA,
  ROUTE_RG
};
struct SconvLayer {
  int kind = 0, level = 0, cin = 0, cout = 0, bf16 = 0;
  bool gated = false;
  int split_io = 0;
  bool residual = false;
};
struct SconvChoice {
  SconvRoute route = ROUTE_RG;
  SconvRoute kernel = ROUTE_RG;
  int NW = 0, NSW = 0, KW = 0, KS = 0, GATED = 0, TRACE = 0, resident = 0;
  int KSP = 0, D = 0, G = 0, SPLIT = 0, PIPE = 0;
  unsigned gx = 0, gy = 1, gz = 1, block = 0;
  size_t lds = 0;
  int kparts = 1;
  int err = 0;
};
template <auto Kernel, class Args>
static int launch_sconv(const SconvChoice& ch, hipStream_t stream, const Args& a, hipEvent_t* stop_later = nullptr) {
  static AttrOnce attr_done;
  if (ch.lds > 48 * 1024 && attr_done.need()) {
    HIP_CHECK(hipFuncSetAttribute(reinterpret_cast<const void*>(Kernel), hipFuncAttributeMaxDynamicSharedMemorySize, 160 * 1024));
    attr_done.mark();
  }
  const dim3 grid(ch.gx, ch.gy, ch.gz), block(ch.block);
  hipEvent_t* pev = prof_kernel_events();
  if (pev[0]) {
    if (stop_later) *stop_later = pev[1];
    hipExtLaunchKernelGGL(Kernel, grid, block, ch.lds, stream, pev[0], stop_later ? nullptr : pev[1], 0, a);
    pev[0] = pev[1] = nullptr;
  } else {
    hipLaunchKernelGGL(Kernel, grid, block, ch.lds, stream, a);
  }
  HIP_CHECK(hipGetLastError());
  return EGONN_OK;
}
SconvChoice sconv_choose(const SconvSettings& s, const SconvLayer& l, int64_t cap_groups);
SconvSetting sconv_decode(int code);
SplitCfg sconv_decode_cfg(int cfg);
SconvRoute sconv_route(const Ctx* ctx, int kind, int level, int cin, int cout, int bf16);
bool sconv_split_arithmetic(const Ctx* ctx);
const char* sconv_kernel_name(const Ctx* ctx, int kind, int level, int cin, int cout, int bf16);
struct SconvLaunch {
  SconvChoice ch;
  const RowGroups* rg = nullptr;
  int64_t n_in_cap = 0;
  const void* Wp = nullptr;
  int32_t* flags = nullptr;
  int B = 0;
  float* part = nullptr; size_t part_floats = 0;
  uint32_t* in_absmax = nullptr; int64_t in_elems = 0;
};
int sconv_rg_forward(const ConvCall& c, const SconvLaunch& l, hipStream_t stream);
int sconv_map(Ctx* ctx, const ConvCall& c, hipStream_t stream);
bool sconv_split_supported(int cin, int cout);
int pack_split_weights(const float* W, int K, int cin, int cout, int flip, int transpose, void* out, hipStream_t stream);
size_t split_weights_bytes(int K, int cin, int cout);
int sconv_split_forward(const ConvCall& c, const SconvLaunch& l, hipStream_t stream);
size_t sconv_split_part_floats(const RowGroups& rg, int cout, int kparts);
struct KsChoice { int kparts, col_parts, kw; };
KsChoice sconv_ksplit_rule(const KsRule& rule, int kind, int level);
void sconv_ksplit_defaults(KsRule* r);
size_t sconv_ksplit_scratch_floats(const Ctx* ctx);
static constexpr size_t SCONV_SCRATCH_FLOATS = (size_t)2 << 20;
int sconv_naive(const float* in, const int32_t* nbr, const float* W, const float* scale, const float* shift, int relu,
                float* out, int64_t n_out, int K, int cin, int cout, hipStream_t stream);
int conv0_lut_init(Ctx* ctx);
int conv0_k5_forward(Ctx* ctx, const float* feat, const float* W, int cout, const float* scale,
                     const float* shift, int relu, void* out, int out_bf16, hipStream_t stream, const void* wpk = nullptr);
int conv0_pack_unit(const float* W, void* wpk, hipStream_t stream);

enum Act { ACT_NONE = 0, ACT_RELU = 1, ACT_TANH = 2, ACT_SOFTPLUS = 3, ACT_SIGMOID = 4 };
struct DenseCall {
  const void* in = nullptr; int in_bf16 = 0;
  int64_t n = 0;
  const int32_t* n_dev = nullptr;
  int cin = 0, cout = 0;
  const float* W = nullptr;
  int w_out_in = 0;
  const float* wfrag = nullptr;
  const float* bias = nullptr;
  const float *scale = nullptr, *shift = nullptr;
  int act = 0;
  const void* residual = nullptr; int res_bf16 = 0;
  const float* gate = nullptr;
  const int32_t* boff = nullptr;
  int B = 0;
  void* out = nullptr; int out_bf16 = 0;
  int form = -1;
};
enum DenseRoute {
  DENSE_INVALID = -1,
  DENSE_NONE = 0,
  DENSE_STREAM,
  DENSE_LDS,
  DENSE_SMALL,
  DENSE_TILE,
  DENSE_PLAIN
};
struct DenseLaunch {
  DenseRoute route = DENSE_NONE;
  unsigned gx = 0, gy = 0;
  size_t lds = 0;
  int colblk = 0;
};
DenseRoute dense_route(int64_t n, int cin, int cout, int form);
DenseLaunch dense_launch(int64_t n, int cin, int cout, int form, int gate_scans);
int dense_forward(const DenseCall& c, hipStream_t stream);
bool dense_gate_fusable(int64_t n, int cin, int cout);
bool dense_group3_rows(int64_t n);
int dense_small_group3(const float* const* in, const int64_t* n, const int32_t* const* n_dev, const float* const* W,
                       const float* const* wfrag, float* const* out, hipStream_t stream);
int dense_pack_frags(const float* W, int w_out_in, int cin, int cout, float* out, hipStream_t stream);

constexpr int GTAIL_CIN = 128, GTAIL_MID = 192, GTAIL_OUT = 256;
int global_tail_fused(const float* g5, int64_t ncap, const int32_t* boff, int B, const float* wf0, const float* b0, const float* wf1,
                      const float* b1, int pow_mode, const float* p, float* partial, hipStream_t stream);

int bn_fold(const float* w, const float* b, const float* rm, const float* rv, float eps, int c, float* scale,
            float* shift, hipStream_t stream);
int gather_rows(const float* in, const int32_t* perm, int64_t n, int c, float* out, hipStream_t stream,
                const int32_t* n_dev = nullptr);
static constexpr int SEG_CHUNKS = 32;
int segment_partial_sums(const float* in, const int32_t* boff, int B, int c, int pow_mode, const float* p,
                         float* partial, hipStream_t stream);
int eca_apply(const float* x, const float* res, const float* partial, const int32_t* boff, int B, int64_t n, int c,
              const float* wconv, int ksize, float* out, hipStream_t stream);
int eca_gate_groups(const float* psum, const RowGroups& rg, const int32_t* boff, int B, int c, const float* wconv, int ksize,
                    float* gate, hipStream_t stream);
int eca_apply_gate(const void* x, const void* res, const float* gate, const int32_t* boff, int B, int64_t n, int c,
                   void* out, int bf16, hipStream_t stream);
int convert_bf16_to_f32(const void* in, int64_t n, float* out, hipStream_t stream);
int gem_finish(const float* partial, const int32_t* boff, int B, int c, const float* p, float* out,
               hipStream_t stream);
int pool_finish(const float* partial, const int32_t* boff, int B, int c, int mode, float* out, hipStream_t stream);
int l2_normalize_rows(float* x, int64_t n, int c, hipStream_t stream, const int32_t* n_dev = nullptr);
int add_act(const float* a, const float* b, int64_t n, int relu, float* out, hipStream_t stream);

constexpr int LH_WAVES = 8;
int keypoint_positions(const uint64_t* keys, int64_t n, int level, int cb, const float* offsets, int mode,
                       const float* step, int ignore_offsets, float* out, hipStream_t stream, const int32_t* n_dev = nullptr);
int local_heads_forward(const float* x, int64_t n, const int32_t* n_dev, const float* const* w, const uint64_t* keys,
                        int level, int cb, int mode, const float* step, int ignore_offsets, float* out_desc, float* out_kp,
                        float* out_sigma, hipStream_t stream, const float* lateral_w = nullptr, const float* lateral_res = nullptr,
                        int in_bf16 = 0, const void* split_pack = nullptr, int32_t* flags = nullptr);
size_t local_heads_pack_bytes();
int local_heads_pack(const float* const* w6_dev, void* out, hipStream_t stream);
int select_topk(const float* sigma, const int32_t* boff_dev, int B, int k, const float* kp, const float* desc, int dc,
                int32_t* sel_rows , int32_t* sel_count , float* out_kp, float* out_desc, hipStream_t stream);

static constexpr int NV_K = 64;
static constexpr int NV_MAX_CHUNKS = 32;
static constexpr int NV_CHUNK_ROWS = 128;
__host__ __device__ static inline int nv_chunks(int32_t len) {
  if (len <= 0) return 0;
  const int n = (len + NV_CHUNK_ROWS - 1) / NV_CHUNK_ROWS;
  return n < NV_MAX_CHUNKS ? n : NV_MAX_CHUNKS;
}
size_t netvlad_workspace_floats(int B, int C, int D);
void netvlad_workspace_carve(float* ws, int B, int C, float** part, float** vraw, float** sq, float** pp);
int netvlad_forward(const float* x, const int32_t* boff, int B, int C, const float* wc, const float* w2, const float* sc1,
                    const float* sh1, const float* H, int D, const float* sc2, const float* sh2, const float* wg,
                    const float* scg, const float* shg, int gating, float* out, float* ws, hipStream_t stream);

constexpr int LL_CLOUD_CHUNK = 1024;
constexpr int LL_STATS = 16;

}
```

### egonn_amd/csrc/model.hip

```cpp
#include "model.h"

using namespace egonn;

namespace {

const int PLANES[7] = {32, 64, 64, 128, 128, 128, 128};
const int GLOBAL_CH = 128, GLOBAL_DIM = 256, LOCAL_CH = 64, LOCAL_DIM = 128;

}

API const char* egonn_last_error(void) { return last_error(); }

API int egonn_debug_set_naive_conv(egonn_ctx* c, int on) {
  EGONN_REQUIRE(c, EGONN_ERR_INVALID, "debug_set_naive_conv: null context");
  c->sconv.set = sconv_decode(on);
  return EGONN_OK;
}

API int egonn_debug_set_ksplit(egonn_ctx* c, int map_class, int level, int kparts, int kw, int col_parts) {
  EGONN_REQUIRE(c && (map_class == 0 || map_class == 1) && level >= 0 && level < EGONN_NUM_LEVELS, EGONN_ERR_INVALID,
                "debug_set_ksplit: bad argument");
  EGONN_REQUIRE(kparts <= 27 && kw <= 4 && col_parts <= 4, EGONN_ERR_INVALID, "debug_set_ksplit: kparts <= 27, kw <= 4, col_parts <= 4");
  if (kparts >= 0) c->sconv.ks_rule.kparts[map_class][level] = (int8_t)std::max(kparts, 1);
  if (kw >= 0) c->sconv.ks_rule.kw[map_class][level] = (int8_t)kw;
// ... 684 lines not shown
  if (ks) {
    c->ks_part = (*A)->alloc<float>(ks);
    EGONN_REQUIRE(c->ks_part, EGONN_ERR_STATE, "work arena too small (ks_part)");
    c->ks_part_floats = ks;
  }
  return EGONN_OK;
}

int conv_layer(egonn_ctx* c, hipStream_t st, const ConvCall& cc, const char* what) {
  static const int pk[3] = {PK_K3, PK_K2S2, PK_TCONV};
  char tag[64];
  snprintf(tag, sizeof(tag), "%s<%d,%d>/L%d/%s", sconv_kernel_name(c, cc.kind, cc.level, cc.cin, cc.cout, cc.bf16), cc.cin, cc.cout,
           cc.level, what);
  ProfScope ps(c, st, tag, pk[cc.kind], cc.level, cc.kind == 0 ? 27 : 8, cc.cin, cc.cout, cc.bf16 ? 2 : 4);
  return sconv_map(c, cc, st);
}
ConvCall conv_call(int kind, int level, const void* in, const PackedKernel& pk, int cin, int cout, int bf16, const BnRef* bn, int relu,
                   void* out) {
  return ConvCall{.kind = kind, .level = level, .in = in, .out = out, .cin = cin, .cout = cout, .bf16 = bf16,
                  .scale = bn ? bn->scale : nullptr, .shift = bn ? bn->shift : nullptr, .relu = relu, .packed = &pk};
}

int ensure_graph_rowgroups(egonn_ctx* c, int L, const int* tlevels, int nt, hipStream_t st) {
  int kinds[RG_MAX_JOBS], levels[RG_MAX_JOBS], n = 0;
  for (int l = 1; l <= L; ++l) { kinds[n] = 0; levels[n++] = l; }
  for (int l = 1; l <= L; ++l) { kinds[n] = 1; levels[n++] = l; }
  for (int i = 0; i < nt; ++i) { kinds[n] = 2; levels[n++] = tlevels[i]; }
  return ensure_rowgroups(c, kinds, levels, n, st);
}

int block_convs(egonn_ctx* c, hipStream_t st, Arena* A, int level, const BlockRef& b, const PackedKernel& pk1, const PackedKernel& pk2,
                int bf16, const void* in, float* psum, void** t2_out) {
  const size_t bytes = (size_t)c->plan.cap[level] * b.cout * (bf16 ? 2 : 4);
  WALLOC(char, t1, bytes);
  WALLOC(char, t2, bytes);
  const bool t1_split = !switches().no_presplit && sconv_route(c, 0, level, b.cin, b.cout, bf16) == ROUTE_SPLIT &&
                        sconv_route(c, 0, level, b.cout, b.cout, bf16) == ROUTE_SPLIT;
  ConvCall c1 = conv_call(0, level, in, pk1, b.cin, b.cout, bf16, &b.n1, 1, t1);
  c1.split_io = t1_split ? 2 : 0;
  EGONN_TRY(conv_layer(c, st, c1, "k3.conv1"));
  ConvCall c2 = conv_call(0, level, t1, pk2, b.cout, b.cout, bf16, &b.n2, 0, t2);
  c2.split_io = t1_split ? 1 : 0;
  c2.psum = psum;
  EGONN_TRY(conv_layer(c, st, c2, "k3.conv2"));
  *t2_out = t2;
  return EGONN_OK;
}

DenseCall down_call(const BlockRef& b, const void* in, int bf16, int64_t n, const int32_t* n_dev, const void* wfrag) {
  return DenseCall{.in = in, .in_bf16 = bf16, .n = n, .n_dev = n_dev, .cin = b.cin, .cout = b.cout, .W = b.down,
                   .wfrag = static_cast<const float*>(wfrag), .scale = b.dn.scale, .shift = b.dn.shift, .out_bf16 = bf16};
}

static int pool_pow_mode(Pooling method) { return method == POOL_GEM ? 1 : method == POOL_MAC ? 2 : 0; }
static int global_pool_finish(Pooling method, const float* partial, const int32_t* boff, int B, int C, const float* p, float* out,
                              hipStream_t st) {
  if (method == POOL_GEM) return gem_finish(partial, boff, B, C, p, out, st);
  return pool_finish(partial, boff, B, C, pool_pow_mode(method), out, st);
}
int global_pool(Pooling method, const float* x, const int32_t* boff, int B, int C, const float* p, float* partial, float* out,
                hipStream_t st) {
  EGONN_TRY(segment_partial_sums(x, boff, B, C, pool_pow_mode(method), method == POOL_GEM ? p : nullptr, partial, st));
  return global_pool_finish(method, partial, boff, B, C, p, out, st);
}

bool global_tail_fusable(const MlpRef& r) { return r.cin == GTAIL_CIN && r.mid == GTAIL_MID && r.cout == GTAIL_OUT; }
int global_tail(const MlpRef& r, const void* const* pk, const float* g5, int64_t ncap, const int32_t* n_dev, const int32_t* boff, int B,
                Pooling method, const float* p, bool fused, float* gh, float* gd, float* partial, float* out, hipStream_t st) {
  if (fused) {
    EGONN_REQUIRE(global_tail_fusable(r) && pk && pk[0] && pk[1], EGONN_ERR_STATE, "global tail: no fused form for %d->%d->%d", r.cin,
                  r.mid, r.cout);
    EGONN_TRY(global_tail_fused(g5, ncap, boff, B, static_cast<const float*>(pk[0]), r.b0, static_cast<const float*>(pk[1]), r.b1,
                                pool_pow_mode(method), method == POOL_GEM ? p : nullptr, partial, st));
    return global_pool_finish(method, partial, boff, B, r.cout, p, out, st);
  }
  EGONN_TRY(run_mlp(r, g5, ncap, ACT_NONE, gh, gd, st, n_dev));
  return global_pool(method, gd, boff, B, r.cout, p, partial, out, st);
}

int block_tail(const float* x, const float* res, const int32_t* boff, int B, int64_t n, int ch, const float* eca, int eca_k,
               float* partial, float* out, hipStream_t st) {
  if (!eca) return add_act(x, res, n * ch, 1, out, st);
  EGONN_TRY(segment_partial_sums(x, boff, B, ch, 0, nullptr, partial, st));
  return eca_apply(x, res, partial, boff, B, n, ch, eca, eca_k, out, st);
}

}

API int egonn_forward(egonn_ctx* c, egonn_model* m, const float* features, int quant_mode, const float* step, int flags,
                      float* out_global, float* out_desc, float* out_kp, float* out_sigma, void* stream) {
  REQUIRE_PLAN(c);
  EGONN_REQUIRE(m && m->ready, EGONN_ERR_STATE, "model not finalized (call egonn_model_finalize)");
  EGONN_REQUIRE(step, EGONN_ERR_INVALID, "forward: null argument");
  HIP_CHECK(hipSetDevice(c->device));
  hipStream_t st = (hipStream_t)stream;
  Plan& P = c->plan;
  const int B = P.batch;
  const int32_t* cnt = c->dev_counts;
  const int bf16 = (flags & EGONN_FLAG_BF16) ? 1 : 0;
  const size_t es = bf16 ? 2 : 4;
  const bool do_global = !(flags & EGONN_FLAG_DISABLE_GLOBAL);
  const bool do_local = !(flags & EGONN_FLAG_DISABLE_LOCAL);
  EGONN_REQUIRE(!do_global || out_global, EGONN_ERR_INVALID, "forward: out_global is null");
  EGONN_REQUIRE(!do_local || (out_desc && out_kp && out_sigma), EGONN_ERR_INVALID, "forward: local outputs are null");
  HIP_CHECK(hipMemsetAsync(c->dev_fp16_flag, 0, sizeof(int32_t), st));

  {
    const int tlevels[3] = {6, 5, 3};
    EGONN_TRY(ensure_graph_rowgroups(c, 7, tlevels + (do_global ? 0 : 2), (do_global ? 2 : 0) + (do_local ? 1 : 0), st));
    DBG_SYNC("row groups");
  }

  size_t need = (size_t)P.cap[0] * (1 + 32) * 4;
  for (int i = 1; i <= 7; ++i) need += (size_t)P.cap[i] * 128 * 4 * 6 + (size_t)P.lv[i].rg27.cap_groups * 128 * 4;
  need += (size_t)P.cap[5] * (192 + 256 + 128 * 2) * 4 + (size_t)P.cap[3] * (96 + 32 + 32 + 3 + 64 * 2) * 4;
  need += (size_t)B * SEG_CHUNKS * 256 * 4 * 10 + (size_t)P.cap[3] * 32 + (4u << 20);
  need += sconv_ksplit_scratch_floats(c) * 4 + 4096;
  Arena* A;
  EGONN_TRY(claim_work(c, need, true, &A));

  const int64_t n0 = P.cap[0];
  const float* f0 = features;
  if (features && !c->from_points) {
    WALLOC(float, fg, n0);
    EGONN_TRY(gather_rows(features, P.perm0, n0, 1, fg, st, cnt));
    f0 = fg;
  }
  WALLOC(char, x0, n0 * 32 * es);
  {
    ProfScope ps(c, st, "conv0_k5_kernel/L0", PK_CONV0, 0, 125, 1, 32, (int)es);
    EGONN_TRY(conv0_k5_forward(c, f0, m->conv0, 32, m->bn[0].scale, m->bn[0].shift, 1, x0, bf16, st, m->conv0_unit));
  }
  DBG_SYNC("conv0");
  const void* x[8] = {x0};
  c->level_feat[0] = x0;
  c->level_ch[0] = 32;
  c->level_bf16 = bf16;
  auto local_head = [&](hipStream_t st) -> int {
    const int64_t n3 = P.cap[3], n4 = P.cap[4];
    WALLOC(char, l4, n4 * LOCAL_CH * es);
    EGONN_TRY(dense_forward({.in = x[4], .in_bf16 = bf16, .n = n4, .n_dev = cnt + 4, .cin = 128, .cout = LOCAL_CH, .W = m->l1x1[4],
                             .wfrag = static_cast<const float*>(m->pk_l1x1[4]), .out = l4, .out_bf16 = bf16},
                            st));
    WALLOC(char, u3, n3 * LOCAL_CH * es);
    EGONN_TRY(conv_layer(c, st, conv_call(2, 3, l4, m->pk_lt[4], LOCAL_CH, LOCAL_CH, bf16, nullptr, 0, u3), "tconv"));
    EGONN_REQUIRE(m->ldec.cin == 64 && m->ldec.mid == 96 && m->ldec.cout == 128 && m->kp.mid == 32 && m->sg.mid == 32,
                  EGONN_ERR_STATE, "local heads: unexpected layer sizes");
    const float* hw[12] = {m->ldec.w0, m->ldec.b0, m->ldec.w1, m->ldec.b1, m->kp.w0, m->kp.b0, m->kp.w1, m->kp.b1,
                           m->sg.w0, m->sg.b0, m->sg.w1, m->sg.b1};
    const void* lh_pack = (!switches().no_split_heads && sconv_split_arithmetic(c)) ? m->lh_pack : nullptr;
    if (!switches().no_fused_lateral && LOCAL_CH == 64) {
      EGONN_TRY(local_heads_forward(reinterpret_cast<const float*>(x[3]), n3, cnt + 3, hw, P.lv[3].keys, 3, P.coord_bits, quant_mode,
                                    step, (flags & EGONN_FLAG_IGNORE_KP_REGRESSOR) ? 1 : 0, out_desc, out_kp, out_sigma, st,
                                    m->l1x1[3], reinterpret_cast<const float*>(u3), bf16, lh_pack, c->dev_fp16_flag));
      return EGONN_OK;
    }
    WALLOC(float, l3, n3 * LOCAL_CH);
    EGONN_TRY(dense_forward({.in = x[3], .in_bf16 = bf16, .n = n3, .n_dev = cnt + 3, .cin = 64, .cout = LOCAL_CH, .W = m->l1x1[3],
                             .wfrag = static_cast<const float*>(m->pk_l1x1[3]), .residual = u3, .res_bf16 = bf16, .out = l3},
                            st));
    EGONN_TRY(local_heads_forward(l3, n3, cnt + 3, hw, P.lv[3].keys, 3, P.coord_bits, quant_mode, step,
                                  (flags & EGONN_FLAG_IGNORE_KP_REGRESSOR) ? 1 : 0, out_desc, out_kp, out_sigma, st, nullptr, nullptr, 0,
                                  lh_pack, c->dev_fp16_flag));
    return EGONN_OK;
  };
  const float *gated_t2 = nullptr, *gated_res = nullptr, *gated_gate = nullptr;
  for (int i = 1; i <= 7; ++i) {
    const BlockRef& b = m->blk[i];
    const Level& L = P.lv[i];
    const int64_t n = P.cap[i];
    WALLOC(char, y, n * b.cin * es);
    {
      ConvCall cc = conv_call(1, i, x[i - 1], m->pk_convs[i], b.cin, b.cin, bf16, &m->bn[i], 1, y);
      if (gated_t2 && i == 2) {
        cc.in = gated_t2;
        cc.in2 = gated_res;
        cc.gate = gated_gate;
      }
      EGONN_TRY(conv_layer(c, st, cc, "k2s2"));
    }
    DBG_SYNC("L%d k2s2", i);
    WALLOC(float, psum, (size_t)L.rg27.cap_groups * b.cout);
    void* t2 = nullptr;
    EGONN_TRY(block_convs(c, st, A, i, b, m->pk_c1[i], m->pk_c2[i], bf16, y, psum, &t2));
    WALLOC(float, gate, (size_t)B * b.cout);
    DBG_SYNC("L%d convs", i);
    EGONN_TRY(eca_gate_groups(psum, L.rg27, L.boff, B, b.cout, b.eca, b.eca_k, gate, st));
    DBG_SYNC("L%d eca gate", i);
    const void* res = y;
    if (i == 1 && !switches().no_gated_k2s2 && !c->keep_level_features && !bf16 && !b.down && c->sconv.set.product() && b.cout == 32 &&
        m->blk[2].cin == 32 && sconv_route(c, 1, 2, 32, 32, 0) == ROUTE_SPLIT) {
      gated_t2 = reinterpret_cast<const float*>(t2);
      gated_res = reinterpret_cast<const float*>(y);
      gated_gate = gate;
      x[i] = nullptr;
      c->level_feat[i] = nullptr;
      c->level_ch[i] = b.cout;
      continue;
    }
    WALLOC(char, xo, n * b.cout * es);
    const DenseCall down = down_call(b, y, bf16, n, cnt + i, m->pk_down[i]);
    if (b.down && !switches().no_fused_down && dense_gate_fusable(n, b.cin, b.cout)) {
      DenseCall dc = down;
      dc.residual = t2; dc.res_bf16 = bf16;
      dc.gate = gate; dc.boff = L.boff; dc.B = B;
      dc.out = xo;
      EGONN_TRY(dense_forward(dc, st));
    } else {
      if (b.down) {
        WALLOC(char, rd, n * b.cout * es);
        DenseCall dc = down;
        dc.out = rd;
        EGONN_TRY(dense_forward(dc, st));
        res = rd;
      }
      EGONN_TRY(eca_apply_gate(t2, res, gate, L.boff, B, n, b.cout, xo, bf16, st));
    }
    DBG_SYNC("L%d eca apply", i);
    x[i] = xo;
    c->level_feat[i] = xo;
    c->level_ch[i] = b.cout;
  }
  if (do_local) EGONN_TRY(local_head(st));
  DBG_SYNC("local head");

  void* g5_fused = nullptr;
  if (do_global && !switches().no_fused_ghead && !bf16 && c->sconv.set.product() && dense_group3_rows(P.cap[5]) &&
      dense_group3_rows(P.cap[6]) && dense_group3_rows(P.cap[7])) {
    WALLOC(float, l7, P.cap[7] * GLOBAL_CH);
    WALLOC(float, l6, P.cap[6] * GLOBAL_CH);
    WALLOC(float, l5, P.cap[5] * GLOBAL_CH);
    WALLOC(float, g6f, P.cap[6] * GLOBAL_CH);
    WALLOC(float, g5f, P.cap[5] * GLOBAL_CH);
    const float* gin[3] = {reinterpret_cast<const float*>(x[7]), reinterpret_cast<const float*>(x[6]), reinterpret_cast<const float*>(x[5])};
    const int64_t gn[3] = {P.cap[7], P.cap[6], P.cap[5]};
    const int32_t* gnd[3] = {cnt + 7, cnt + 6, cnt + 5};
    const float* gw[3] = {m->g1x1[7], m->g1x1[6], m->g1x1[5]};
    float* gout[3] = {l7, l6, l5};
    const float* gpk[3] = {static_cast<const float*>(m->pk_g1x1[7]), static_cast<const float*>(m->pk_g1x1[6]),
                           static_cast<const float*>(m->pk_g1x1[5])};
    EGONN_TRY(dense_small_group3(gin, gn, gnd, gw, switches().no_packed_laterals ? nullptr : gpk, gout, st));
    for (int lv = 6; lv >= 5; --lv) {
      ConvCall cc = conv_call(2, lv, lv == 6 ? l7 : g6f, m->pk_gt[lv + 1], GLOBAL_CH, GLOBAL_CH, 0, nullptr, 0, lv == 6 ? g6f : g5f);
      cc.residual = lv == 6 ? l6 : l5;
      EGONN_TRY(conv_layer(c, st, cc, "tconv"));
    }
    g5_fused = g5f;
    DBG_SYNC("global head (fused)");
  }
  if (do_global) {
    const float* g5 = reinterpret_cast<const float*>(g5_fused);
    if (!g5) {
    auto lateral = [&](int l, const void* up, void* out, int out_bf16) {
      return dense_forward({.in = x[l], .in_bf16 = bf16, .n = P.cap[l], .n_dev = cnt + l, .cin = 128, .cout = GLOBAL_CH, .W = m->g1x1[l],
                            .residual = up, .res_bf16 = up ? bf16 : 0, .out = out, .out_bf16 = out_bf16},
                           st);
    };
    WALLOC(char, g7, P.cap[7] * GLOBAL_CH * es);
    EGONN_TRY(lateral(7, nullptr, g7, bf16));
    WALLOC(char, u6, P.cap[6] * GLOBAL_CH * es);
    EGONN_TRY(conv_layer(c, st, conv_call(2, 6, g7, m->pk_gt[7], GLOBAL_CH, GLOBAL_CH, bf16, nullptr, 0, u6), "tconv"));
    WALLOC(char, g6, P.cap[6] * GLOBAL_CH * es);
    EGONN_TRY(lateral(6, u6, g6, bf16));
    WALLOC(char, u5, P.cap[5] * GLOBAL_CH * es);
    EGONN_TRY(conv_layer(c, st, conv_call(2, 5, g6, m->pk_gt[6], GLOBAL_CH, GLOBAL_CH, bf16, nullptr, 0, u5), "tconv"));
    WALLOC(float, g5u, P.cap[5] * GLOBAL_CH);
    EGONN_TRY(lateral(5, u5, g5u, 0));
    g5 = g5u;
    DBG_SYNC("global head");
    }
    WALLOC(float, gh, P.cap[5] * m->gdec.mid);
    WALLOC(float, gd, P.cap[5] * GLOBAL_DIM);
    WALLOC(float, gp, (size_t)B * SEG_CHUNKS * GLOBAL_DIM);
    const Pooling pool = (flags & EGONN_FLAG_POOL_MAC) ? POOL_MAC : (flags & EGONN_FLAG_POOL_SPOC) ? POOL_SPOC : POOL_GEM;
    EGONN_REQUIRE(pool != POOL_GEM || m->gem_p, EGONN_ERR_STATE, "forward: GeM pooling needs the tensor 'global_pooling.pooling.p'");
    const bool fused_tail = !switches().no_fused_gtail && global_tail_fusable(m->gdec) && m->pk_gdec[0] && m->pk_gdec[1];
    EGONN_TRY(global_tail(m->gdec, m->pk_gdec, g5, P.cap[5], cnt + 5, P.lv[5].boff, B, pool, m->gem_p, fused_tail, gh, gd, gp, out_global, st));
  }

  DBG_SYNC("global decoder + pooling");
  return EGONN_OK;
}

static size_t debug_tail_span(int64_t ncap) {
  return align_up((size_t)ncap * GTAIL_MID * 4, 256) + align_up((size_t)ncap * GTAIL_OUT * 4, 256) +
         align_up((size_t)GTAIL_CIN * GTAIL_MID * 4, 256) + align_up((size_t)GTAIL_MID * GTAIL_OUT * 4, 256) + 1024;
}
API int64_t egonn_debug_global_tail_scratch_bytes(int64_t rows_capacity) {
  if (rows_capacity < 0 || rows_capacity >= (1ll << 31) / GTAIL_OUT) return -1;
  return (int64_t)debug_tail_span(rows_capacity);
}
API int egonn_debug_global_tail(const float* g5, const int32_t* row_offsets, int batch_size, int64_t rows_capacity, const int32_t* n_dev,
                                const float* w0, const float* b0, const float* w1, const float* b1, const float* p, int pooling, int form,
                                float* partial, float* out, void* scratch, int64_t scratch_bytes, void* stream) {
  EGONN_REQUIRE(g5 && row_offsets && n_dev && w0 && b0 && w1 && b1 && partial && out && scratch, EGONN_ERR_INVALID,
                "debug_global_tail: null pointer");
  EGONN_REQUIRE(batch_size >= 1 && batch_size <= EGONN_MAX_BATCH, EGONN_ERR_INVALID, "debug_global_tail: batch_size=%d outside [1, %d]",
                batch_size, EGONN_MAX_BATCH);
  EGONN_REQUIRE(rows_capacity >= 0 && rows_capacity < (1ll << 31) / GTAIL_OUT, EGONN_ERR_INVALID,
                "debug_global_tail: rows_capacity=%lld outside [0, 2^31 / %d)", (long long)rows_capacity, GTAIL_OUT);
  EGONN_REQUIRE(pooling >= POOL_GEM && pooling <= POOL_SPOC && (pooling != POOL_GEM || p), EGONN_ERR_INVALID,
                "debug_global_tail: pooling=%d (1 GeM with its exponent, 2 MAC, 3 SPoC)", pooling);
  EGONN_REQUIRE(form == 0 || form == 1, EGONN_ERR_INVALID, "debug_global_tail: form=%d (0 three launches, 1 the fused launch)", form);
  const size_t need = debug_tail_span(rows_capacity);
  EGONN_REQUIRE(scratch_bytes >= (int64_t)need && ((uintptr_t)scratch & 255) == 0, EGONN_ERR_INVALID,
                "debug_global_tail: scratch needs %lld bytes, 256-byte aligned", (long long)need);
  hipStream_t st = (hipStream_t)stream;
  Arena ws = Arena::view(scratch, need);
  float* gh = ws.alloc<float>((size_t)rows_capacity * GTAIL_MID);
  float* gd = ws.alloc<float>((size_t)rows_capacity * GTAIL_OUT);
  float* pk0 = ws.alloc<float>((size_t)GTAIL_CIN * GTAIL_MID);
  float* pk1 = ws.alloc<float>((size_t)GTAIL_MID * GTAIL_OUT);
  EGONN_REQUIRE(gh && gd && pk0 && pk1, EGONN_ERR_STATE, "debug_global_tail: scratch span too small");
  const MlpRef r{.w0 = w0, .b0 = b0, .w1 = w1, .b1 = b1, .cin = GTAIL_CIN, .mid = GTAIL_MID, .cout = GTAIL_OUT};
  const void* pk[2] = {pk0, pk1};
  if (form == 1) {
    EGONN_TRY(dense_pack_frags(w0, 1, r.cin, r.mid, pk0, st));
    EGONN_TRY(dense_pack_frags(w1, 1, r.mid, r.cout, pk1, st));
  }
  return global_tail(r, pk, g5, rows_capacity, n_dev, row_offsets, batch_size, (Pooling)pooling, p, form == 1, gh, gd, partial, out, st);
}

API int egonn_forward_level_features(egonn_ctx* c, int level, float* out, int channels, void* stream) {
  REQUIRE_PLAN(c);
  EGONN_REQUIRE(level >= 0 && level < EGONN_NUM_LEVELS && c->level_feat[level], EGONN_ERR_STATE,
                "no features for level %d (run egonn_forward first; level 1 of fp32 maps is materialised only after "
                "egonn_debug_keep_level_features(ctx, 1))", level);
  EGONN_REQUIRE(channels == c->level_ch[level], EGONN_ERR_INVALID, "level %d has %d channels, caller expects %d", level,
                c->level_ch[level], channels);
  const int64_t cnt = c->plan.lv[level].n * channels;
  if (c->level_bf16) return convert_bf16_to_f32(c->level_feat[level], cnt, out, (hipStream_t)stream);
  HIP_CHECK(hipMemcpyAsync(out, c->level_feat[level], sizeof(float) * cnt, hipMemcpyDeviceToDevice, (hipStream_t)stream));
  return EGONN_OK;
}

API int egonn_select_keypoints(egonn_ctx* c, const float* sigma, const float* keypoints, const float* descriptors,
                               int n_k, float* sel_kp, float* sel_desc, int32_t* sel_rows, int32_t* sel_count,
                               void* stream) {
  REQUIRE_PLAN(c);
  EGONN_REQUIRE(sigma && keypoints && descriptors && sel_kp && sel_desc && sel_rows && sel_count, EGONN_ERR_INVALID,
                "select_keypoints: null argument");
  HIP_CHECK(hipSetDevice(c->device));
  return select_topk(sigma, c->plan.lv[3].boff, c->plan.batch, n_k, keypoints, descriptors, LOCAL_DIM, sel_rows, sel_count,
                     sel_kp, sel_desc, (hipStream_t)stream);
}


API int egonn_topk_rows(const float* sigma, const int32_t* row_offsets, int batch_size, int n_k, int32_t* sel_rows,
                        int32_t* sel_count, void* stream) {
  EGONN_REQUIRE(sigma && row_offsets && sel_rows && sel_count && batch_size >= 1, EGONN_ERR_INVALID, "topk_rows: bad argument");
  return select_topk(sigma, row_offsets, batch_size, n_k, nullptr, nullptr, 0, sel_rows, sel_count, nullptr, nullptr,
                     (hipStream_t)stream);
}

API int egonn_profile_enable(egonn_ctx* c, int mode, const char* filter) {
  EGONN_REQUIRE(c && mode >= 0 && mode <= 3, EGONN_ERR_INVALID, "profile_enable: bad argument");
  c->prof.mode = mode;
  snprintf(c->prof.filter, sizeof(c->prof.filter), "%s", filter ? filter : "");
  return EGONN_OK;
}

API int egonn_profile_fetch(egonn_ctx* c, int cap, int* n, char* names, float* ms, double* bytes, double* flops,
                            void* stream) {
  EGONN_REQUIRE(c && n && names && ms && bytes && flops, EGONN_ERR_INVALID, "profile_fetch: null argument");
  HIP_CHECK(hipSetDevice(c->device));
  Plan& P = c->plan;
  if (P.valid) {
    if (P.built_reserved) P.exact = false;
    EGONN_TRY(plan_sync(c, (hipStream_t)stream));
    EGONN_TRY(count_map_pairs(c, (hipStream_t)stream));
  }
  HIP_CHECK(hipStreamSynchronize((hipStream_t)stream));
  unsigned long long pairs[16];
  HIP_CHECK(hipMemcpy(pairs, c->dev_pairs, sizeof(pairs), hipMemcpyDeviceToHost));
  int w = 0;
  std::vector<ProfRec> all(c->prof.recs);
  all.insert(all.end(), c->prof.graph_recs.begin(), c->prof.graph_recs.end());
  const size_t n_plain = c->prof.recs.size();
  size_t ri = 0;
  for (auto& r : all) {
    const bool plain = ri++ < n_plain;
    float t = 0.f;
    if (hipEventSynchronize(r.e1) != hipSuccess || hipEventElapsedTime(&t, r.e0, r.e1) != hipSuccess) {
      (void)hipGetLastError();
      if (plain) { c->prof.pool.push_back(r.e0); c->prof.pool.push_back(r.e1); }
      continue;
    }
    if (w < cap) {
      const double n_out = (double)P.lv[r.level].n;
      double Pn = 0;
      switch (r.kind) {
        case PK_CONV0: Pn = (double)pairs[0]; break;
        case PK_K3: Pn = (double)pairs[r.level]; break;
        case PK_K2S2: Pn = (double)P.lv[r.level - 1].n; break;
        case PK_TCONV: Pn = n_out; break;
        default: Pn = n_out; break;
      }
      snprintf(names + (size_t)w * 64, 64, "%s", r.name);
      ms[w] = t;
      bytes[w] = Pn * r.cin * r.es + n_out * r.cout * r.es + (double)r.K * r.cin * r.cout * r.es + 8.0 * Pn;
      flops[w] = 2.0 * Pn * r.cin * r.cout;
      ++w;
    }
    if (plain) { c->prof.pool.push_back(r.e0); c->prof.pool.push_back(r.e1); }
  }
  c->prof.recs.clear();
  *n = w;
  return EGONN_OK;
}
```

### include/egonn_hip.h

```cpp
#ifndef EGONN_HIP_H
#define EGONN_HIP_H

#include <stdint.h>

#ifdef __cplusplus
extern "C" {
#endif

typedef struct egonn_ctx egonn_ctx;
typedef struct egonn_model egonn_model;

enum { EGONN_QUANT_CARTESIAN = 0, EGONN_QUANT_POLAR = 1 };
enum { EGONN_STATUS_OK = 0, EGONN_STATUS_INVALID = 1, EGONN_STATUS_HIP = 2, EGONN_STATUS_RANGE = 3, EGONN_STATUS_STATE = 4,
       EGONN_STATUS_CAPACITY = 5,
       EGONN_STATUS_FP16_RANGE = 6 };
enum { EGONN_FLAG_DISABLE_GLOBAL = 1, EGONN_FLAG_DISABLE_LOCAL = 2, EGONN_FLAG_IGNORE_KP_REGRESSOR = 4,
       EGONN_FLAG_BF16 = 8,
       EGONN_FLAG_POOL_SPOC = 16, EGONN_FLAG_POOL_MAC = 32 };

int egonn_ctx_create(egonn_ctx** ctx, int device, int coord_bits);
void egonn_ctx_destroy(egonn_ctx* ctx);
const char* egonn_last_error(void);
int egonn_debug_set_naive_conv(egonn_ctx* ctx, int on);
int egonn_debug_set_ksplit(egonn_ctx* ctx, int map_class, int level, int kparts, int kw, int col_parts);
int egonn_debug_set_resident(egonn_ctx* ctx, int mask, int max_workgroups);
int egonn_debug_keep_level_features(egonn_ctx* ctx, int on);
int egonn_debug_set_trace(void* device_buffer);
int egonn_debug_rowgroup_tables(egonn_ctx* ctx, int map_kind, int level_out, uint32_t* gmask_out, int32_t* snbr_out,
                                int64_t capacity_groups, int64_t* n_groups, void* stream);
int egonn_debug_rowgroup_perm(egonn_ctx* ctx, int map_kind, int level_out, int32_t* perm_out, int64_t capacity_groups,
                              int64_t* n_groups, void* stream);
int64_t egonn_debug_radix_sort_scratch_bytes(int64_t n, int n_segments);
int egonn_debug_radix_sort(uint64_t* keys_in, uint32_t* vals_in, uint64_t* keys_out, uint32_t* vals_out, int64_t n, int nbits,
                           const int64_t* n_dev, const int64_t* seg_offsets, int n_segments, int idx_bits, int either_pair,
                           int32_t* result_pair, void* scratch, int64_t scratch_bytes, void* stream);
int egonn_debug_dense_group3(const float* const in[3], const int64_t rows_capacity[3], const int32_t* const n_dev[3],
                             const float* const weight[3], const float* const packed[3], float* const out[3], void* stream);
int64_t egonn_debug_global_tail_scratch_bytes(int64_t rows_capacity);
int egonn_debug_global_tail(const float* g5, const int32_t* row_offsets, int batch_size, int64_t rows_capacity, const int32_t* n_dev,
                            const float* w0, const float* b0, const float* w1, const float* b1, const float* p, int pooling, int form,
                            float* partial, float* out, void* scratch, int64_t scratch_bytes, void* stream);

int egonn_voxelize(egonn_ctx* ctx, const float* points, const int64_t* scan_offsets, int batch_size, int quant_mode,
                   const float* step, void* stream);
int egonn_ctx_reserve(egonn_ctx* ctx, int64_t max_points, int batch_size, const int64_t* level_capacity);
int egonn_voxelize_device(egonn_ctx* ctx, const float* points, int64_t n_rows, const int64_t* scan_offsets_dev,
                          int batch_size, int quant_mode, const float* step, void* stream);
int egonn_plan_status(egonn_ctx* ctx, void* stream);
int egonn_ctx_set_exact_fp32(egonn_ctx* ctx, int on);
int egonn_ctx_set_operand_autoscale(egonn_ctx* ctx, int on);
int egonn_level_capacity(egonn_ctx* ctx, int level, int64_t* capacity);
typedef struct egonn_graph egonn_graph;
int egonn_graph_begin(void* stream);
int egonn_graph_end(void* stream, egonn_graph** graph);
int egonn_graph_launch(egonn_graph* graph, void* stream);
void egonn_graph_destroy(egonn_graph* graph);
int egonn_coords_set(egonn_ctx* ctx, const int32_t* coords, int64_t n, int batch_size, void* stream);

int egonn_level_count(egonn_ctx* ctx, int level, int64_t* n_rows);
int egonn_level_batch_offsets(egonn_ctx* ctx, int level, int64_t* offsets );
int egonn_level_coords(egonn_ctx* ctx, int level, int32_t* out, void* stream);
int egonn_input_index(egonn_ctx* ctx, int64_t* out , void* stream);

int egonn_conv(egonn_ctx* ctx, int level_in, int level_out, int kernel_size, const float* in, int cin,
               const float* kernel, int cout, const float* scale, const float* shift, int relu, float* out,
               void* stream);
int egonn_conv_transpose(egonn_ctx* ctx, int level_in, const float* in, int cin, const float* kernel, int cout,
                         float* out, void* stream);
int egonn_sparse_conv(egonn_ctx* ctx, int map_kind, int level_out, const void* in, int cin, const float* kernel, int cout,
                      int bf16, const float* scale, const float* shift, int relu, void* out, float* group_sums,
                      void* stream);
int egonn_prepare_maps(egonn_ctx* ctx, int with_level0_transpose, void* stream);
int egonn_map_groups(egonn_ctx* ctx, int map_kind, int level_out, int64_t* n_groups, int64_t* first_group, void* stream);
int egonn_global_avg_pool(egonn_ctx* ctx, int level, const float* in, int channels, float* out, void* stream);

int egonn_bn_fold(const float* weight, const float* bias, const float* running_mean, const float* running_var,
                  float eps, int channels, float* scale, float* shift, void* stream);
int egonn_block_tail(egonn_ctx* ctx, int level, const float* x, const float* residual, int channels,
                     const float* eca_weight, int eca_ksize, float* out, void* stream);
int egonn_add(const float* a, const float* b, int64_t n, float* out, void* stream);
int egonn_gather_input(egonn_ctx* ctx, const float* features, int channels, float* out, void* stream);
int egonn_gem(egonn_ctx* ctx, int level, const float* x, int channels, const float* p, float* out, void* stream);
int egonn_global_max_pool(egonn_ctx* ctx, int level, const float* in, int channels, float* out, void* stream);
int egonn_netvlad(egonn_ctx* ctx, int level, const float* x, int channels, const float* cluster_weights,
                  const float* cluster_weights2, const float* bn1_scale, const float* bn1_shift,
                  const float* hidden1_weights, const float* bn2_scale, const float* bn2_shift,
                  const float* gating_weights, const float* gate_scale, const float* gate_shift, int out_dim, int gating,
                  float* out, void* stream);
int egonn_netvlad_train_forward(egonn_ctx* ctx, int level, const float* x, int channels, int nmax,
                                const float* cluster_weights, const float* cluster_weights2, const float* bn1_weight,
                                const float* bn1_bias, float bn1_eps, float bn1_momentum, float* bn1_running_mean,
                                float* bn1_running_var, const float* hidden1_weights, int out_dim, float* out, float* save_z,
                                float* save_bn1, float* save_v, float* save_sq, float* save_asum, void* stream);
int egonn_netvlad_train_backward(egonn_ctx* ctx, int level, const float* x, int channels, int nmax,
                                 const float* cluster_weights, const float* cluster_weights2, const float* bn1_weight,
                                 const float* hidden1_weights, int out_dim, const float* grad_out, const float* save_z,
                                 const float* save_bn1, const float* save_v, const float* save_sq, const float* save_asum,
                                 float* grad_x, float* grad_cluster_weights, float* grad_cluster_weights2, float* out_bn1,
                                 float* grad_hidden1_weights, void* stream);
int egonn_global_max_pool_argmax(egonn_ctx* ctx, int level, const float* in, int channels, float* out, int32_t* out_rows,
                                 void* stream);
int egonn_global_max_pool_backward(egonn_ctx* ctx, int level, const float* grad_out, const int32_t* rows, int channels,
                                   float* grad_in, void* stream);
int egonn_sigmoid_gate(const float* y, const float* t, const float* grad_out, int64_t n, float* out, float* grad_y,
                       float* grad_t, void* stream);

int egonn_model_create(egonn_model** model);
void egonn_model_destroy(egonn_model* model);
int egonn_model_set_tensor(egonn_model* model, const char* key, const float* data, int ndim, const int64_t* shape);
int egonn_model_finalize(egonn_model* model, void* stream);

int egonn_forward(egonn_ctx* ctx, egonn_model* model, const float* features, int quant_mode, const float* step,
                  int flags, float* out_global, float* out_descriptors, float* out_keypoints, float* out_sigma,
                  void* stream);
int egonn_forward_level_features(egonn_ctx* ctx, int level, float* out, int channels, void* stream);

int egonn_minkfpn_finalize(egonn_model* model, int n_levels, const int* planes, const int* layers, int num_top_down,
                           int feature_size, int block, int pooling, void* stream);
int egonn_minkfpn_out_level(int n_levels, int num_top_down, int* level);
enum { EGONN_MINKFPN_SPLIT_TOPDOWN = 1 };
int egonn_minkfpn_forward(egonn_ctx* ctx, egonn_model* model, int flags, float* out_global, float* out_map, void* stream);
int egonn_topdown_step(egonn_ctx* ctx, int level_out, const float* x_coarse, const float* w_tconv, const float* x_lateral,
                       const float* w_lateral, int C, int Cl, float* out, void* stream);

int egonn_select_keypoints(egonn_ctx* ctx, const float* sigma, const float* keypoints, const float* descriptors,
                           int n_k, float* sel_keypoints, float* sel_descriptors, int32_t* sel_rows,
                           int32_t* sel_count, void* stream);

int egonn_topk_rows(const float* sigma, const int32_t* row_offsets, int batch_size, int n_k, int32_t* sel_rows,
                    int32_t* sel_count, void* stream);

int64_t egonn_triplet_loss_scratch_floats(int n);
int egonn_triplet_loss(const float* embeddings, int n, int d, const uint8_t* positives_mask,
                       const uint8_t* negatives_mask, float margin, float* out_stats, int32_t* out_triplets,
                       float* out_grad, float* scratch, void* stream);

int64_t egonn_contrastive_loss_scratch_floats(int n);
int egonn_contrastive_loss(const float* embeddings, int n, int d, const uint8_t* positives_mask,
                           const uint8_t* negatives_mask, float pos_margin, float neg_margin, float* out_stats,
                           int32_t* out_triplets, float* out_grad, float* scratch, void* stream);

int egonn_nn_search(const float* a, int64_t n, const float* transform, const float* b, int64_t m, float* out_dist,
                    int32_t* out_index, void* stream);
int egonn_matrix_min(const float* d, int64_t n, int64_t m, float* row_min, int32_t* row_index, float* col_min,
                     int32_t* col_index, void* stream);
int egonn_softmax_cross_entropy(const float* logits, int64_t n, int64_t m, const int32_t* target, float* out_loss,
                                int32_t* out_argmax, float* out_dlogits, void* stream);

#define EGONN_LOCAL_LOSS_STATS 16
enum { EGONN_LL_LOSS = 0, EGONN_LL_KP_PER_CLOUD = 1, EGONN_LL_REPEATABILITY = 2, EGONN_LL_CHAMFER_PURE = 3,
       EGONN_LL_CHAMFER_WEIGHTED = 4, EGONN_LL_MEAN_SIGMA = 5, EGONN_LL_LOSS_CHAMFER = 6, EGONN_LL_LOSS_P2P = 7,
       EGONN_LL_KEYPOINT_LOSS = 8, EGONN_LL_CORRESPONDENCE_LOSS = 9, EGONN_LL_MATCHING_KEYPOINTS = 10,
       EGONN_LL_MATCHING_DESCRIPTORS = 11, EGONN_LL_POS_SIMILARITY = 12, EGONN_LL_NEG_SIMILARITY = 13  };
int64_t egonn_local_loss_scratch_bytes(int pairs, int64_t n_kp1, int64_t n_kp2, int dim);
int egonn_local_loss(int pairs, int64_t n_cloud1, int64_t n_cloud2, int64_t n_kp1, int64_t n_kp2, int dim,
                     const float* clouds1, const int32_t* cloud_off1, const float* clouds2, const int32_t* cloud_off2,
                     const float* kp1, const float* sigma1, const float* desc1, const int32_t* kp_off1,
                     const float* kp2, const float* sigma2, const float* desc2, const int32_t* kp_off2,
                     const float* transforms, const float* params, float* out_pair, float* out_batch,
                     float* g_kp1, float* g_sigma1, float* g_desc1, float* g_kp2, float* g_sigma2, float* g_desc2,
                     void* scratch, int64_t scratch_bytes, void* stream);

enum { EGONN_ACT_NONE = 0, EGONN_ACT_RELU = 1, EGONN_ACT_TANH = 2, EGONN_ACT_SOFTPLUS = 3, EGONN_ACT_SIGMOID = 4 };
int egonn_dense(const float* x, int64_t n, int cin, const float* weight, int weight_out_in, const float* bias, int cout,
                int act, float* out, void* stream);
int egonn_dense_pack_fragments(const float* weight, int weight_out_in, int cin, int cout, float* packed, void* stream);
int egonn_dense_pack_fragments_host(const float* weight, int weight_out_in, int cin, int cout, float* packed);
int egonn_debug_dense(const void* in, int in_bf16, int64_t rows_capacity, const int32_t* n_dev, int cin, int cout, const float* weight,
                      int weight_out_in, const float* packed, const float* bias, const float* scale, const float* shift, int act,
                      const void* residual, int res_bf16, const float* gate, const int32_t* boff, int B, void* out, int out_bf16,
                      int form, void* stream);
int egonn_debug_dense_route(int64_t rows, int cin, int cout, int form, int gate_scans, int32_t out[5]);
int egonn_debug_sconv_choice(const int32_t in[16], int64_t cap_groups, int32_t out[20]);
int egonn_dense_backward_weight(const float* a, int ca, const float* b, int cb, int64_t n, float* out, float* scratch,
                                int64_t scratch_floats, void* stream);
int egonn_conv_backward_weight(egonn_ctx* ctx, int level_in, int level_out, int kernel_size, int transposed,
                               const float* in, int cin, const float* grad_out, int cout, float* grad_kernel,
                               float* scratch, int64_t scratch_floats, void* stream);
int egonn_col_stats(int mode, const float* a, const float* b, const float* mask, const float* mean, int64_t n, int c,
                    double* out, float* scratch, int64_t scratch_floats, void* stream);
int egonn_bn_train_finalize(const double* sums, const float* shift_point, double count, int c, const float* weight,
                            const float* bias, float eps, float momentum, float* running_mean, float* running_var,
                            float* out_mean_invstd_scale_shift, void* stream);
int egonn_bn_backward_finalize(const double* local_sums, const double* global_sums, double count, int c, const float* weight,
                               const float* mean, const float* invstd, float* out_abc_dgamma_dbeta, void* stream);
int egonn_affine_act(const float* x, const float* scale, const float* shift, int64_t n, int c, int relu, float* out,
                     void* stream);
int egonn_affine3(const float* g, const float* mask, const float* x, const float* A, const float* B, const float* C,
                  int64_t n, int c, float* out, void* stream);
int egonn_relu_backward(const float* grad_out, const float* out, int64_t n, int c, float* grad_in, void* stream);
int egonn_act_backward(int act, const float* grad_out, const float* out, int64_t n, int c, float* grad_in, void* stream);
int egonn_l2_normalize(const float* x, const float* grad_out, int64_t n, int c, float* out, void* stream);
int egonn_eca_gate(const float* mean, const float* conv_weight, int kernel_size, int batch_size, int channels, float* gate,
                   void* stream);
// ... 211 lines not shown
```

Baseline: 23390.

## Overlap prologue loads in conv0 and local-heads kernels, specialize by template

The conv0 kernels now issue their first row-info loads and a register-staged copy of the LUT before the weight loads, and write LDS afterwards so the global-load latency overlaps the setup. Weight and scale loads become branch-free, with the zeroing deferred. The local-heads kernel stages biases and fragments through registers in request/commit form, is templated on lateral form and bf16 input, and can take prepacked lateral fragments. A debug entry point is added for testing. These changes add template instantiations and code size, and the keypoint math moves from explicit rounding intrinsics to plain arithmetic with contraction disabled.

```diff
diff --git a/egonn_amd/_lib.py b/egonn_amd/_lib.py
--- a/egonn_amd/_lib.py
+++ b/egonn_amd/_lib.py
@@ -36,6 +36,9 @@
     ("egonn_debug_dense_group3", C.c_int, [_P, _P, _P, _P, _P, _P, _P]),
     ("egonn_debug_global_tail_scratch_bytes", C.c_int64, [C.c_int64]),
     ("egonn_debug_global_tail", C.c_int, [_P, _P, C.c_int, C.c_int64, _P, _P, _P, _P, _P, _P, C.c_int, C.c_int, _P, _P, _P, C.c_int64, _P]),
+    ("egonn_debug_local_heads_scratch_bytes", C.c_int64, []),
+    ("egonn_debug_local_heads", C.c_int, [_P, C.c_int64, _P, _P, _P, _P, _P, C.c_int, C.c_int, C.c_int, C.c_int, C.c_float, _P, _P, _P,
+                                          _P, _P, C.c_int64, _P]),
     ("egonn_voxelize", C.c_int, [_P, _P, C.POINTER(C.c_int64), C.c_int, C.c_int, C.POINTER(C.c_float), _P]),
     ("egonn_ctx_reserve", C.c_int, [_P, C.c_int64, C.c_int, C.POINTER(C.c_int64)]),
     ("egonn_voxelize_device", C.c_int, [_P, _P, C.c_int64, _P, C.c_int, C.c_int, C.POINTER(C.c_float), _P]),
@@ -390,6 +393,23 @@
     return partial, out
 
 
+def debug_local_heads(x, n_dev, weights, keys, lateral_w=None, lateral_res=None, lateral_packed: bool = False, exact: bool = False,
+                      coord_bits: int = 16, quant_step: float = 0.1, flags=None, canary: float = -12345.0):
+    lib = load()
+    dev = x.device
+    cap = x.shape[0]
+    need = lib.egonn_debug_local_heads_scratch_bytes()
+    buf = scratch(need, dev)
+    desc = torch.full((cap, 128), canary, dtype=torch.float32, device=dev)
+    kp = torch.full((cap, 3), canary, dtype=torch.float32, device=dev)
+    sigma = torch.full((cap,), canary, dtype=torch.float32, device=dev)
+    w12 = (C.c_void_p * 12)(*[w.data_ptr() for w in weights])
+    call(dev, lib.egonn_debug_local_heads, x.data_ptr(), int(cap), n_dev.data_ptr(), w12, keys.data_ptr(), _ptr(lateral_w),
+         _ptr(lateral_res), int(bool(lateral_packed)), int(x.dtype == torch.bfloat16), int(bool(exact)), int(coord_bits),
+         float(quant_step), desc.data_ptr(), kp.data_ptr(), sigma.data_ptr(), _ptr(flags), buf.data_ptr(), need)
+    return desc, kp, sigma
+
+
 def require_gpu() -> torch.device:
     if not torch.cuda.is_available():
         raise RuntimeError("egonn_amd: no HIP device visible (torch.cuda.is_available() is False); "
diff --git a/egonn_amd/csrc/conv.hip b/egonn_amd/csrc/conv.hip
--- a/egonn_amd/csrc/conv.hip
+++ b/egonn_amd/csrc/conv.hip
@@ -67,30 +67,42 @@
   const int32_t nvox = min(__builtin_amdgcn_readfirstlane(counts[0]), cap0);
   const int32_t n2 = min(__builtin_amdgcn_readfirstlane(counts[2]), cap2);
   const int32_t ntiles = (nvox + 15) >> 4;
-  for (int e = tid; e < 64 * 128 / 2; e += 256) {
-    const int r = e >> 6, c = e & 63;
-    reinterpret_cast<uint32_t*>(s_lut)[r * (LUT_STRIDE / 2) + c] = reinterpret_cast<const uint32_t*>(lut)[e];
-  }
-  if (tid < 64) s_m[tid >> 4][tid & 15][27] = 0ull;
+  const int tstep = gridDim.x * 4;
+  int32_t tile = blockIdx.x * 4 + wave;
+  int32_t g_cur, g_nxt;
+  uint32_t lk_cur, lk_nxt, lk_nn;
+  int32_t g_nn;
+  {
+    const __amdgpu_buffer_rsrc_t gc_rsrc =
+        __builtin_amdgcn_make_buffer_rsrc(const_cast<int32_t*>(g0), 0, (int)((uint32_t)cap0 * 4u), 0x00020000);
+    const __amdgpu_buffer_rsrc_t kc_rsrc =
+        __builtin_amdgcn_make_buffer_rsrc(const_cast<uint64_t*>(vkeys), 0, (int)((uint32_t)cap0 * 8u), 0x00020000);
+    const uint32_t ra = (uint32_t)tile * 16u + (uint32_t)l15, rb = (uint32_t)(tile + tstep) * 16u + (uint32_t)l15;
+    g_cur = __builtin_amdgcn_raw_buffer_load_b32(gc_rsrc, (int)(ra * 4u), 0, 0);
+    lk_cur = (uint32_t)__builtin_amdgcn_raw_buffer_load_b32(kc_rsrc, (int)(ra * 8u), 0, 0);
+    g_nxt = __builtin_amdgcn_raw_buffer_load_b32(gc_rsrc, (int)(rb * 4u), 0, 0);
+    lk_nxt = (uint32_t)__builtin_amdgcn_raw_buffer_load_b32(kc_rsrc, (int)(rb * 8u), 0, 0);
+  }
+  uint4 lq[4];
+#pragma unroll
+  for (int u = 0; u < 4; ++u) lq[u] = reinterpret_cast<const uint4*>(lut)[tid + 256 * u];
   float breg[2][32];
 #pragma unroll
   for (int q = 0; q < 32; ++q) {
     const int k = 16 * (q >> 2) + 4 * g4 + (q & 3);
 #pragma unroll
-    for (int nt = 0; nt < 2; ++nt) breg[nt][q] = (k < 125) ? W[k * COUT0 + nt * 16 + l15] : 0.f;
+    for (int nt = 0; nt < 2; ++nt) breg[nt][q] = W[min(k, 124) * COUT0 + nt * 16 + l15];
   }
   f32x4 sc[2], sh[2];
 #pragma unroll
   for (int nt = 0; nt < 2; ++nt) {
-    sc[nt] = scale ? *reinterpret_cast<const f32x4*>(scale + nt * 16 + 4 * g4) : (f32x4){1.f, 1.f, 1.f, 1.f};
-    sh[nt] = scale ? *reinterpret_cast<const f32x4*>(shift + nt * 16 + 4 * g4) : (f32x4){0.f, 0.f, 0.f, 0.f};
-  }
-  __syncthreads();
+    sc[nt] = *reinterpret_cast<const f32x4*>((scale ? scale : W) + nt * 16 + 4 * g4);
+    sh[nt] = *reinterpret_cast<const f32x4*>((scale ? shift : W) + nt * 16 + 4 * g4);
+  }
   const __amdgpu_buffer_rsrc_t m_rsrc =
       __builtin_amdgcn_make_buffer_rsrc(const_cast<uint64_t*>(t2m), 0, (int)((uint32_t)n2 * 27u * 8u), 0x00020000);
   const __amdgpu_buffer_rsrc_t s_rsrc =
       __builtin_amdgcn_make_buffer_rsrc(const_cast<int32_t*>(t2s), 0, (int)((uint32_t)n2 * 27u * 4u), 0x00020000);
-  const int tstep = gridDim.x * 4;
   constexpr int NE = (16 * 27 + 63) / 64;
   uint64_t pm[NE];
   int32_t ps[NE];
@@ -115,13 +127,33 @@
       ps[e] = __builtin_amdgcn_raw_buffer_load_b32(s_rsrc, (int)(ent * 4u), 0, 0);
     }
   };
-  int32_t tile = blockIdx.x * 4 + wave;
-  int32_t g_cur, g_nxt;
-  uint32_t lk_cur, lk_nxt, lk_nn;
-  int32_t g_nn;
-  row_info(tile, g_cur, lk_cur);
-  row_info(tile + tstep, g_nxt, lk_nxt);
+  {
+    const bool in_a = tile * 16 + l15 < nvox, in_b = (tile + tstep) * 16 + l15 < nvox;
+    g_cur = in_a ? g_cur : 0; lk_cur = in_a ? (lk_cur & 63u) : 0u;
+    g_nxt = in_b ? g_nxt : 0; lk_nxt = in_b ? (lk_nxt & 63u) : 0u;
+  }
   table_issue(g_cur);
+#pragma unroll
+  for (int u = 0; u < 4; ++u) {
+    const int e = tid + 256 * u, r = e >> 4, c = e & 15;
+    uint2* d = reinterpret_cast<uint2*>(s_lut + r * LUT_STRIDE + 8 * c);
+    d[0] = make_uint2(lq[u].x, lq[u].y);
+    d[1] = make_uint2(lq[u].z, lq[u].w);
+  }
+  if (tid < 64) s_m[tid >> 4][tid & 15][27] = 0ull;
+#pragma unroll
+  for (int q = 0; q < 32; ++q) {
+    const int k = 16 * (q >> 2) + 4 * g4 + (q & 3);
+    if (k >= 125) breg[0][q] = breg[1][q] = 0.f;
+  }
+  if (!scale) {
+#pragma unroll
+    for (int nt = 0; nt < 2; ++nt) {
+      sc[nt] = (f32x4){1.f, 1.f, 1.f, 1.f};
+      sh[nt] = (f32x4){0.f, 0.f, 0.f, 0.f};
+    }
+  }
+  __syncthreads();
   for (; tile < ntiles; tile += tstep) {
     const int32_t r0 = tile * 16;
 #pragma unroll
@@ -194,7 +226,7 @@
 }
 
 typedef short bf16x8_c0 __attribute__((ext_vector_type(8)));
-template <bool OUT_BF16>
+template <bool OUT_BF16, bool PACKED>
 __global__ __launch_bounds__(256) void conv0_k5_unit_kernel(const uint64_t* __restrict__ vkeys,
                                                              const int32_t* __restrict__ g0,
                                                              const uint64_t* __restrict__ t2m,
@@ -213,13 +245,26 @@
   const int32_t nvox = min(__builtin_amdgcn_readfirstlane(counts[0]), cap0);
   const int32_t n2 = min(__builtin_amdgcn_readfirstlane(counts[2]), cap2);
   const int32_t ntiles = (nvox + 15) >> 4;
-  for (int e = tid; e < 64 * 128 / 2; e += 256) {
-    const int r = e >> 6, c = e & 63;
-    reinterpret_cast<uint32_t*>(s_lut)[r * (LUT_STRIDE / 2) + c] = reinterpret_cast<const uint32_t*>(lut)[e];
-  }
-  if (tid < 64) s_m[tid >> 4][tid & 15][27] = 0ull;
+  const int tstep = gridDim.x * 4;
+  int32_t tile = blockIdx.x * 4 + wave;
+  int32_t g_cur, g_nxt, g_nn;
+  uint32_t lk_cur, lk_nxt, lk_nn;
+  {
+    const __amdgpu_buffer_rsrc_t gc_rsrc =
+        __builtin_amdgcn_make_buffer_rsrc(const_cast<int32_t*>(g0), 0, (int)((uint32_t)cap0 * 4u), 0x00020000);
+    const __amdgpu_buffer_rsrc_t kc_rsrc =
+        __builtin_amdgcn_make_buffer_rsrc(const_cast<uint64_t*>(vkeys), 0, (int)((uint32_t)cap0 * 8u), 0x00020000);
+    const uint32_t ra = (uint32_t)tile * 16u + (uint32_t)l15, rb = (uint32_t)(tile + tstep) * 16u + (uint32_t)l15;
+    g_cur = __builtin_amdgcn_raw_buffer_load_b32(gc_rsrc, (int)(ra * 4u), 0, 0);
+    lk_cur = (uint32_t)__builtin_amdgcn_raw_buffer_load_b32(kc_rsrc, (int)(ra * 8u), 0, 0);
+    g_nxt = __builtin_amdgcn_raw_buffer_load_b32(gc_rsrc, (int)(rb * 4u), 0, 0);
+    lk_nxt = (uint32_t)__builtin_amdgcn_raw_buffer_load_b32(kc_rsrc, (int)(rb * 8u), 0, 0);
+  }
+  uint4 lq[4];
+#pragma unroll
+  for (int u = 0; u < 4; ++u) lq[u] = reinterpret_cast<const uint4*>(lut)[tid + 256 * u];
   bf16x8_c0 wf[2][4][3];
-  if (wpk) {
+  if constexpr (PACKED) {
 #pragma unroll
     for (int nt = 0; nt < 2; ++nt)
 #pragma unroll
@@ -253,17 +298,15 @@
   f32x4 sc[2], sh[2];
 #pragma unroll
   for (int nt = 0; nt < 2; ++nt) {
-    sc[nt] = scale ? *reinterpret_cast<const f32x4*>(scale + nt * 16 + 4 * g4) : (f32x4){1.f, 1.f, 1.f, 1.f};
-    sh[nt] = scale ? *reinterpret_cast<const f32x4*>(shift + nt * 16 + 4 * g4) : (f32x4){0.f, 0.f, 0.f, 0.f};
-  }
-  __syncthreads();
+    sc[nt] = *reinterpret_cast<const f32x4*>((scale ? scale : W) + nt * 16 + 4 * g4);
+    sh[nt] = *reinterpret_cast<const f32x4*>((scale ? shift : W) + nt * 16 + 4 * g4);
+  }
   const __amdgpu_buffer_rsrc_t m_rsrc =
       __builtin_amdgcn_make_buffer_rsrc(const_cast<uint64_t*>(t2m), 0, (int)((uint32_t)n2 * 27u * 8u), 0x00020000);
   const __amdgpu_buffer_rsrc_t g_rsrc =
       __builtin_amdgcn_make_buffer_rsrc(const_cast<int32_t*>(g0), 0, (int)((uint32_t)nvox * 4u), 0x00020000);
   const __amdgpu_buffer_rsrc_t k_rsrc =
       __builtin_amdgcn_make_buffer_rsrc(const_cast<uint64_t*>(vkeys), 0, (int)((uint32_t)nvox * 8u), 0x00020000);
-  const int tstep = gridDim.x * 4;
   constexpr int NE = (16 * 27 + 63) / 64;
   uint64_t pm[NE];
   auto row_info = [&](int32_t tile, int32_t& g, uint32_t& lkbits) {
@@ -282,12 +325,26 @@
       pm[e] = ((uint64_t)m2[1] << 32) | (uint64_t)m2[0];
     }
   };
-  int32_t tile = blockIdx.x * 4 + wave;
-  int32_t g_cur, g_nxt, g_nn;
-  uint32_t lk_cur, lk_nxt, lk_nn;
-  row_info(tile, g_cur, lk_cur);
-  row_info(tile + tstep, g_nxt, lk_nxt);
+  {
+    const bool in_a = tile * 16 + l15 < nvox, in_b = (tile + tstep) * 16 + l15 < nvox;
+    g_cur = in_a ? g_cur : 0; lk_cur = in_a ? (lk_cur & 63u) : 0u;
+    g_nxt = in_b ? g_nxt : 0; lk_nxt = in_b ? (lk_nxt & 63u) : 0u;
+  }
   table_issue(g_cur);
+#pragma unroll
+  for (int u = 0; u < 4; ++u) {
+    const int e = tid + 256 * u, r = e >> 4, c = e & 15;
+    *reinterpret_cast<uint4*>(s_lut + r * LUT_STRIDE + 8 * c) = lq[u];
+  }
+  if (tid < 64) s_m[tid >> 4][tid & 15][27] = 0ull;
+  if (!scale) {
+#pragma unroll
+    for (int nt = 0; nt < 2; ++nt) {
+      sc[nt] = (f32x4){1.f, 1.f, 1.f, 1.f};
+      sh[nt] = (f32x4){0.f, 0.f, 0.f, 0.f};
+    }
+  }
+  __syncthreads();
   for (; tile < ntiles; tile += tstep) {
     const int32_t r0 = tile * 16;
 #pragma unroll
@@ -420,14 +477,13 @@
   } else if (ctx->sconv.set.family == SCONV_PLAIN) {
     if (out_bf16) EGONN_CONV0_LAUNCH(true, true); else EGONN_CONV0_LAUNCH(true, false);
   } else {
-    if (out_bf16)
-      hipLaunchKernelGGL((conv0_k5_unit_kernel<true>), dim3(grid), dim3(256), 0, stream, V.keys, P.g0, P.t2m, ctx->dev_counts,
-                         (int32_t)P.cap[2], (int32_t)P.cap[0], W, scale, shift, relu, out, ctx->conv0_lut,
-                         reinterpret_cast<const uint4*>(wpk));
-    else
-      hipLaunchKernelGGL((conv0_k5_unit_kernel<false>), dim3(grid), dim3(256), 0, stream, V.keys, P.g0, P.t2m, ctx->dev_counts,
-                         (int32_t)P.cap[2], (int32_t)P.cap[0], W, scale, shift, relu, out, ctx->conv0_lut,
-                         reinterpret_cast<const uint4*>(wpk));
+#define EGONN_CONV0_UNIT(OB, PK)                                                                                       \
+  hipLaunchKernelGGL((conv0_k5_unit_kernel<OB, PK>), dim3(grid), dim3(256), 0, stream, V.keys, P.g0, P.t2m, ctx->dev_counts, \
+                     (int32_t)P.cap[2], (int32_t)P.cap[0], W, scale, shift, relu, out, ctx->conv0_lut,                  \
+                     reinterpret_cast<const uint4*>(wpk))
+    if (out_bf16) { if (wpk) EGONN_CONV0_UNIT(true, true); else EGONN_CONV0_UNIT(true, false); }
+    else { if (wpk) EGONN_CONV0_UNIT(false, true); else EGONN_CONV0_UNIT(false, false); }
+#undef EGONN_CONV0_UNIT
   }
 #undef EGONN_CONV0_LAUNCH
   HIP_CHECK(hipGetLastError());
diff --git a/egonn_amd/csrc/heads.hip b/egonn_amd/csrc/heads.hip
--- a/egonn_amd/csrc/heads.hip
+++ b/egonn_amd/csrc/heads.hip
@@ -1,4 +1,5 @@
 #include <algorithm>
+#include <type_traits>
 
 #include "common.h"
 #include "kernels.h"
@@ -9,6 +10,7 @@
 
 __device__ static inline void keypoint_position(uint64_t key, int level, int cb, float ox, float oy, float oz, int mode,
                                                 float s0, float s1, float s2, float* __restrict__ out3) {
+#pragma clang fp contract(off)
   const int cbL = cb - level;
   const uint64_t mort = key & ((1ull << (3 * cbL)) - 1);
   const int32_t bias = 1 << (cb - 1);
@@ -16,13 +18,13 @@
   const float cy = (float)(((int32_t)compact1by2(mort >> 1) << level) - bias);
   const float cz = (float)(((int32_t)compact1by2(mort >> 2) << level) - bias);
   const float stride = (float)(1 << level);
-  const float px = __fadd_rn(__fmul_rn(__fadd_rn(cx, 0.5f), s0), __fdiv_rn(__fmul_rn(ox, __fmul_rn(stride, s0)), 2.f));
-  const float py = __fadd_rn(__fmul_rn(__fadd_rn(cy, 0.5f), s1), __fdiv_rn(__fmul_rn(oy, __fmul_rn(stride, s1)), 2.f));
-  const float pz = __fadd_rn(__fmul_rn(__fadd_rn(cz, 0.5f), s2), __fdiv_rn(__fmul_rn(oz, __fmul_rn(stride, s2)), 2.f));
+  const float px = (cx + 0.5f) * s0 + (ox * (stride * s0)) / 2.f;
+  const float py = (cy + 0.5f) * s1 + (oy * (stride * s1)) / 2.f;
+  const float pz = (cz + 0.5f) * s2 + (oz * (stride * s2)) / 2.f;
   if (mode == 0) {
     out3[0] = px; out3[1] = py; out3[2] = pz;
   } else {
-    const float theta = __fdiv_rn(__fmul_rn(3.14159265358979323846f, __fadd_rn(px, -180.f)), 180.f);
+    const float theta = (3.14159265358979323846f * (px + -180.f)) / 180.f;
     out3[0] = cosf(theta) * py;
     out3[1] = sinf(theta) * py;
     out3[2] = pz;
@@ -52,6 +54,7 @@
 struct LocalHeadsArgs {
   const float* x;
   const float *lw, *lres;
+  const float* lpk;
   const float *dw0, *db0, *dw1, *db1;
   const float *kw0, *kb0, *kw1, *kb1;
   const float *sw0, *sb0, *sw1, *sb1;
@@ -60,21 +63,8 @@
   float *out_desc, *out_kp, *out_sigma;
   int64_t n;
   int level, cb, mode, ignore_offsets;
-  int in_bf16;
   float s0, s1, s2;
 };
-template <int CIN, int NT>
-__device__ static inline void stage_frags(const float* __restrict__ W, int rows_w, f32x4* __restrict__ dst, int tid, int nthreads) {
-  constexpr int T = CIN / 16;
-  for (int i = tid; i < NT * T * 64; i += nthreads) {
-    const int lane = i & 63, ft = i >> 6;
-    const int nt = ft / T, t = ft - nt * T;
-    const int unit = 16 * nt + (lane & 15);
-    f32x4 v = {0.f, 0.f, 0.f, 0.f};
-    if (unit < rows_w) v = *reinterpret_cast<const f32x4*>(W + (int64_t)unit * CIN + 16 * t + 4 * (lane >> 4));
-    dst[i] = v;
-  }
-}
 template <int CIN, int NT>
 __device__ static inline void mlp_layer(const f32x4* __restrict__ frags, const f32x4* __restrict__ in, int lane,
                                         f32x4* __restrict__ out) {
@@ -92,61 +82,158 @@
     __builtin_amdgcn_sched_barrier(0);
   }
 }
+constexpr int LH_THREADS = LH_WAVES * 64;
+constexpr int LH_B_DB0 = 0, LH_B_DB1 = LH_B_DB0 + 96, LH_B_KB0 = LH_B_DB1 + 128, LH_B_SB0 = LH_B_KB0 + 32, LH_B_KB1 = LH_B_SB0 + 32,
+              LH_B_SB1 = LH_B_KB1 + 3, LH_BIAS = LH_B_SB1 + 1, LH_BIAS_LDS = 304;
+struct LhBiasStage {
+  float v[6];
+  __device__ inline void request(const LocalHeadsArgs& p, int tid) {
+    v[0] = p.db0[min(tid, 95)]; v[1] = p.db1[min(tid, 127)]; v[2] = p.kb0[min(tid, 31)];
+    v[3] = p.sb0[min(tid, 31)]; v[4] = p.kb1[min(tid, 2)]; v[5] = p.sb1[0];
+  }
+  __device__ inline void commit(float* __restrict__ s_bias, int tid) const {
+    if (tid < 96) s_bias[LH_B_DB0 + tid] = v[0];
+    if (tid < 128) s_bias[LH_B_DB1 + tid] = v[1];
+    if (tid < 32) {
+      s_bias[LH_B_KB0 + tid] = v[2];
+      s_bias[LH_B_SB0 + tid] = v[3];
+    }
+    if (tid < 3) s_bias[LH_B_KB1 + tid] = v[4];
+    if (tid == 0) s_bias[LH_B_SB1] = v[5];
+  }
+};
 template <int CIN, int NT>
-__device__ static inline void stage_frags_t(const float* __restrict__ W, int cout, f32x4* __restrict__ dst, int tid, int nthreads) {
-  constexpr int T = CIN / 16;
-  for (int i = tid; i < NT * T * 64; i += nthreads) {
-    const int lane = i & 63, ft = i >> 6;
-    const int nt = ft / T, t = ft - nt * T;
-    const float* wp = W + (int64_t)(16 * t + 4 * (lane >> 4)) * cout + 16 * nt + (lane & 15);
-    dst[i] = (f32x4){wp[0], wp[cout], wp[2 * (int64_t)cout], wp[3 * (int64_t)cout]};
-  }
-}
+struct LhFragStage {
+  static constexpr int T = CIN / 16, N = NT * T * 64, PER = (N + LH_THREADS - 1) / LH_THREADS;
+  f32x4 v[PER];
+  __device__ inline void request(const float* __restrict__ W, int rows_w, int tid) {
+#pragma unroll
+    for (int u = 0; u < PER; ++u) {
+      const int i = min(tid + u * LH_THREADS, N - 1);
+      const int lane = i & 63, ft = i >> 6;
+      const int nt = ft / T, t = ft - nt * T;
+      const int unit = min(16 * nt + (lane & 15), rows_w - 1);
+      v[u] = *reinterpret_cast<const f32x4*>(W + (int64_t)unit * CIN + 16 * t + 4 * (lane >> 4));
+    }
+  }
+  __device__ inline void commit(f32x4* __restrict__ dst, int rows_w, int tid) const {
+#pragma unroll
+    for (int u = 0; u < PER; ++u) {
+      const int i = tid + u * LH_THREADS;
+      const int unit = 16 * ((i >> 6) / T) + (i & 15);
+      if (N % LH_THREADS == 0 || i < N) dst[i] = unit < rows_w ? v[u] : (f32x4){0.f, 0.f, 0.f, 0.f};
+    }
+  }
+};
+template <int LAT>
+struct LhLateralStage {
+  f32x4 v[LAT ? 2 : 1];
+  __device__ inline void request(const float* __restrict__ lw, const float* __restrict__ lpk, int tid) {
+    if constexpr (LAT != 0) {
+#pragma unroll
+      for (int u = 0; u < 2; ++u) {
+        const int i = tid + u * LH_THREADS;
+        if constexpr (LAT == 2) {
+          v[u] = reinterpret_cast<const f32x4*>(lpk)[i];
+        } else {
+          const int lane = i & 63, ft = i >> 6;
+          const int nt = ft >> 2, t = ft & 3;
+          const float* wp = lw + (16 * t + 4 * (lane >> 4)) * 64 + 16 * nt + (lane & 15);
+          v[u] = (f32x4){wp[0], wp[64], wp[128], wp[192]};
+        }
+      }
+    }
+  }
+  __device__ inline void commit(f32x4* __restrict__ lat, int tid) const {
+    if constexpr (LAT != 0) {
+#pragma unroll
+      for (int u = 0; u < 2; ++u) lat[tid + u * LH_THREADS] = v[u];
+    }
+  }
+};
+template <bool LAT, bool IN_BF16>
+struct LhTile {
+  using raw_t = std::conditional_t<IN_BF16, uint2, f32x4>;
+  raw_t x[4], r[LAT ? 4 : 1];
+  uint64_t key;
+  __device__ inline void request(const LocalHeadsArgs& p, int64_t tile, int64_t n, int l15, int g4) {
+    const int64_t rowc = min(tile * 16 + l15, max(n, (int64_t)1) - 1);
+    const int64_t at = rowc * 64 + 4 * g4;
+#pragma unroll
+    for (int t = 0; t < 4; ++t) x[t] = raw(p.x, at + 16 * t);
+    if constexpr (LAT) {
+#pragma unroll
+      for (int t = 0; t < 4; ++t) r[t] = raw(p.lres, at + 16 * t);
+    }
+    key = p.keys[rowc];
+  }
+  __device__ static inline raw_t raw(const float* base, int64_t at) {
+    if constexpr (IN_BF16) return *reinterpret_cast<const uint2*>(reinterpret_cast<const uint16_t*>(base) + at);
+    else return *reinterpret_cast<const f32x4*>(base + at);
+  }
+  __device__ static inline f32x4 wide(const raw_t& h) {
+    if constexpr (IN_BF16) return (f32x4){bf2f(h.x & 0xFFFFu), bf2f(h.x >> 16), bf2f(h.y & 0xFFFFu), bf2f(h.y >> 16)};
+    else return h;
+  }
+};
 constexpr int LH_F_DW0 = 0, LH_F_DW1 = LH_F_DW0 + 6 * 4, LH_F_KW0 = LH_F_DW1 + 8 * 6, LH_F_KW1 = LH_F_KW0 + 2 * 4,
               LH_F_SW0 = LH_F_KW1 + 1 * 2, LH_F_SW1 = LH_F_SW0 + 2 * 4, LH_FRAGS = LH_F_SW1 + 1 * 2;
-__global__ __launch_bounds__(LH_WAVES * 64) void local_heads_kernel(const LocalHeadsArgs p) {
+template <int LAT, bool IN_BF16>
+__global__ __launch_bounds__(LH_THREADS) void local_heads_kernel(const LocalHeadsArgs p) {
   extern __shared__ __attribute__((aligned(16))) f32x4 lh_frags[];
   const int tid = threadIdx.x, lane = tid & 63, wave = tid >> 6;
   const int l15 = lane & 15, g4 = lane >> 4;
-  stage_frags<64, 6>(p.dw0, 96, lh_frags + LH_F_DW0 * 64, tid, LH_WAVES * 64);
-  stage_frags<96, 8>(p.dw1, 128, lh_frags + LH_F_DW1 * 64, tid, LH_WAVES * 64);
-  stage_frags<64, 2>(p.kw0, 32, lh_frags + LH_F_KW0 * 64, tid, LH_WAVES * 64);
-  stage_frags<32, 1>(p.kw1, 3, lh_frags + LH_F_KW1 * 64, tid, LH_WAVES * 64);
-  stage_frags<64, 2>(p.sw0, 32, lh_frags + LH_F_SW0 * 64, tid, LH_WAVES * 64);
-  stage_frags<32, 1>(p.sw1, 1, lh_frags + LH_F_SW1 * 64, tid, LH_WAVES * 64);
-  if (p.lw) stage_frags_t<64, 4>(p.lw, 64, lh_frags + LH_FRAGS * 64, tid, LH_WAVES * 64);
-  __syncthreads();
+  f32x4* const lat = lh_frags + LH_FRAGS * 64;
+  const float* const s_bias = reinterpret_cast<const float*>(lat + (LAT ? 16 * 64 : 0));
+  LhFragStage<64, 6> f_dw0;
+  LhFragStage<96, 8> f_dw1;
+  LhFragStage<64, 2> f_kw0, f_sw0;
+  LhFragStage<32, 1> f_kw1, f_sw1;
+  LhLateralStage<LAT> f_lat;
+  f_dw0.request(p.dw0, 96, tid);
+  f_dw1.request(p.dw1, 128, tid);
+  f_kw0.request(p.kw0, 32, tid);
+  f_kw1.request(p.kw1, 3, tid);
+  f_sw0.request(p.sw0, 32, tid);
+  f_sw1.request(p.sw1, 1, tid);
+  f_lat.request(p.lw, p.lpk, tid);
+  LhBiasStage f_bias;
+  f_bias.request(p, tid);
   int64_t n = p.n;
   if (p.n_dev) n = min((int64_t)*p.n_dev, n);
   const int64_t ntiles = (n + 15) >> 4;
-  for (int64_t tile = (int64_t)blockIdx.x * LH_WAVES + wave; tile < ntiles; tile += (int64_t)gridDim.x * LH_WAVES) {
+  const int64_t tstep = (int64_t)gridDim.x * LH_WAVES;
+  int64_t tile = (int64_t)blockIdx.x * LH_WAVES + wave;
+  LhTile<LAT != 0, IN_BF16> cur, nxt;
+  cur.request(p, tile, n, l15, g4);
+  f_dw0.commit(lh_frags + LH_F_DW0 * 64, 96, tid);
+  f_dw1.commit(lh_frags + LH_F_DW1 * 64, 128, tid);
+  f_kw0.commit(lh_frags + LH_F_KW0 * 64, 32, tid);
+  f_kw1.commit(lh_frags + LH_F_KW1 * 64, 3, tid);
+  f_sw0.commit(lh_frags + LH_F_SW0 * 64, 32, tid);
+  f_sw1.commit(lh_frags + LH_F_SW1 * 64, 1, tid);
+  f_lat.commit(lat, tid);
+  f_bias.commit(const_cast<float*>(s_bias), tid);
+  __syncthreads();
+  for (; tile < ntiles; tile += tstep) {
+    nxt.request(p, tile + tstep, n, l15, g4);
     const int64_t row = tile * 16 + l15;
     const bool ok = row < n;
     f32x4 x[4];
-    auto load4 = [&](const float* base, int t) -> f32x4 {
-      if (!ok) return (f32x4){0.f, 0.f, 0.f, 0.f};
-      if (p.in_bf16) {
-        const uint2 h = *reinterpret_cast<const uint2*>(reinterpret_cast<const uint16_t*>(base) + row * 64 + 16 * t + 4 * g4);
-        return (f32x4){bf2f(h.x & 0xFFFFu), bf2f(h.x >> 16), bf2f(h.y & 0xFFFFu), bf2f(h.y >> 16)};
-      }
-      return *reinterpret_cast<const f32x4*>(base + row * 64 + 16 * t + 4 * g4);
-    };
-#pragma unroll
-    for (int t = 0; t < 4; ++t) x[t] = load4(p.x, t);
-    if (p.lw) {
-      f32x4 r[4], l[4];
-#pragma unroll
-      for (int t = 0; t < 4; ++t) r[t] = load4(p.lres, t);
-      mlp_layer<64, 4>(lh_frags + LH_FRAGS * 64, x, lane, l);
-#pragma unroll
-      for (int t = 0; t < 4; ++t) x[t] = l[t] + r[t];
+#pragma unroll
+    for (int t = 0; t < 4; ++t) x[t] = cur.wide(cur.x[t]);
+    if constexpr (LAT != 0) {
+      f32x4 l[4];
+      mlp_layer<64, 4>(lat, x, lane, l);
+#pragma unroll
+      for (int t = 0; t < 4; ++t) x[t] = l[t] + cur.wide(cur.r[t]);
     }
     {
       f32x4 h[6], o[8];
       mlp_layer<64, 6>(lh_frags + LH_F_DW0 * 64, x, lane, h);
 #pragma unroll
       for (int nt = 0; nt < 6; ++nt) {
-        const f32x4 b = *reinterpret_cast<const f32x4*>(p.db0 + 16 * nt + 4 * g4);
+        const f32x4 b = *reinterpret_cast<const f32x4*>(s_bias + LH_B_DB0 + 16 * nt + 4 * g4);
 #pragma unroll
         for (int r = 0; r < 4; ++r) h[nt][r] = fmaxf(h[nt][r] + b[r], 0.f);
       }
@@ -154,7 +241,7 @@
       float ss = 0.f;
 #pragma unroll
       for (int nt = 0; nt < 8; ++nt) {
-        const f32x4 b = *reinterpret_cast<const f32x4*>(p.db1 + 16 * nt + 4 * g4);
+        const f32x4 b = *reinterpret_cast<const f32x4*>(s_bias + LH_B_DB1 + 16 * nt + 4 * g4);
 #pragma unroll
         for (int r = 0; r < 4; ++r) {
           o[nt][r] += b[r];
@@ -175,16 +262,16 @@
       mlp_layer<64, 2>(lh_frags + LH_F_KW0 * 64, x, lane, h);
 #pragma unroll
       for (int nt = 0; nt < 2; ++nt) {
-        const f32x4 b = *reinterpret_cast<const f32x4*>(p.kb0 + 16 * nt + 4 * g4);
+        const f32x4 b = *reinterpret_cast<const f32x4*>(s_bias + LH_B_KB0 + 16 * nt + 4 * g4);
 #pragma unroll
         for (int r = 0; r < 4; ++r) h[nt][r] = fmaxf(h[nt][r] + b[r], 0.f);
       }
       mlp_layer<32, 1>(lh_frags + LH_F_KW1 * 64, h, lane, o);
       if (ok && g4 == 0) {
-        const float ox = p.ignore_offsets ? 0.f : tanhf(o[0][0] + p.kb1[0]);
-        const float oy = p.ignore_offsets ? 0.f : tanhf(o[0][1] + p.kb1[1]);
-        const float oz = p.ignore_offsets ? 0.f : tanhf(o[0][2] + p.kb1[2]);
-        keypoint_position(p.keys[row], p.level, p.cb, ox, oy, oz, p.mode, p.s0, p.s1, p.s2, p.out_kp + row * 3);
+        const float ox = p.ignore_offsets ? 0.f : tanhf(o[0][0] + s_bias[LH_B_KB1 + 0]);
+        const float oy = p.ignore_offsets ? 0.f : tanhf(o[0][1] + s_bias[LH_B_KB1 + 1]);
+        const float oz = p.ignore_offsets ? 0.f : tanhf(o[0][2] + s_bias[LH_B_KB1 + 2]);
+        keypoint_position(cur.key, p.level, p.cb, ox, oy, oz, p.mode, p.s0, p.s1, p.s2, p.out_kp + row * 3);
       }
     }
     {
@@ -192,13 +279,14 @@
       mlp_layer<64, 2>(lh_frags + LH_F_SW0 * 64, x, lane, h);
 #pragma unroll
       for (int nt = 0; nt < 2; ++nt) {
-        const f32x4 b = *reinterpret_cast<const f32x4*>(p.sb0 + 16 * nt + 4 * g4);
+        const f32x4 b = *reinterpret_cast<const f32x4*>(s_bias + LH_B_SB0 + 16 * nt + 4 * g4);
 #pragma unroll
         for (int r = 0; r < 4; ++r) h[nt][r] = fmaxf(h[nt][r] + b[r], 0.f);
       }
       mlp_layer<32, 1>(lh_frags + LH_F_SW1 * 64, h, lane, o);
-      if (ok && g4 == 0) p.out_sigma[row] = apply_act(o[0][0] + p.sb1[0], ACT_SOFTPLUS);
-    }
+      if (ok && g4 == 0) p.out_sigma[row] = apply_act(o[0][0] + s_bias[LH_B_SB1], ACT_SOFTPLUS);
+    }
+    cur = nxt;
   }
 }
 constexpr int LHS_DW0 = 0, LHS_DW1 = LHS_DW0 + 6 * 2, LHS_KW0 = LHS_DW1 + 8 * 3, LHS_KW1 = LHS_KW0 + 2 * 2, LHS_SW0 = LHS_KW1 + 1 * 1,
@@ -265,44 +353,54 @@
   const void* pack;
   int32_t* flags;
 };
-__global__ __launch_bounds__(LH_WAVES * 64) void local_heads_split_kernel(const LocalHeadsSplitArgs q) {
+template <int LAT, bool IN_BF16>
+__global__ __launch_bounds__(LH_THREADS) void local_heads_split_kernel(const LocalHeadsSplitArgs q) {
   const LocalHeadsArgs& p = q.a;
   extern __shared__ __attribute__((aligned(16))) f32x4 lh_frags[];
   const int tid = threadIdx.x, lane = tid & 63, wave = tid >> 6;
   const int l15 = lane & 15, g4 = lane >> 4;
+  constexpr int NPK = LHS_FRAGS * 2 * 64, PER = (NPK + LH_THREADS - 1) / LH_THREADS;
+  f32x4* const lat = lh_frags + NPK;
+  const float* const s_bias = reinterpret_cast<const float*>(lat + (LAT ? 16 * 64 : 0));
+  f32x4 st[PER];
   {
     const f32x4* src = reinterpret_cast<const f32x4*>(q.pack);
-    for (int i = tid; i < LHS_FRAGS * 2 * 64; i += LH_WAVES * 64) lh_frags[i] = src[i];
-  }
-  f32x4* const lat = lh_frags + LHS_FRAGS * 2 * 64;
-  if (p.lw) stage_frags_t<64, 4>(p.lw, 64, lat, tid, LH_WAVES * 64);
+#pragma unroll
+    for (int u = 0; u < PER; ++u) st[u] = src[min(tid + u * LH_THREADS, NPK - 1)];
+  }
+  LhLateralStage<LAT> f_lat;
+  f_lat.request(p.lw, p.lpk, tid);
+  LhBiasStage f_bias;
+  f_bias.request(p, tid);
   const float* winv = reinterpret_cast<const float*>(reinterpret_cast<const char*>(q.pack) + (size_t)LHS_FRAGS * 2048);
   const float wi0 = winv[0], wi1 = winv[1], wi2 = winv[2], wi3 = winv[3], wi4 = winv[4], wi5 = winv[5];
-  __syncthreads();
   int64_t n = p.n;
   if (p.n_dev) n = min((int64_t)*p.n_dev, n);
   const int64_t ntiles = (n + 15) >> 4;
-  for (int64_t tile = (int64_t)blockIdx.x * LH_WAVES + wave; tile < ntiles; tile += (int64_t)gridDim.x * LH_WAVES) {
+  const int64_t tstep = (int64_t)gridDim.x * LH_WAVES;
+  int64_t tile = (int64_t)blockIdx.x * LH_WAVES + wave;
+  LhTile<LAT != 0, IN_BF16> cur, nxt;
+  cur.request(p, tile, n, l15, g4);
+#pragma unroll
+  for (int u = 0; u < PER; ++u) {
+    const int i = tid + u * LH_THREADS;
+    if (NPK % LH_THREADS == 0 || i < NPK) lh_frags[i] = st[u];
+  }
+  f_lat.commit(lat, tid);
+  f_bias.commit(const_cast<float*>(s_bias), tid);
+  __syncthreads();
+  for (; tile < ntiles; tile += tstep) {
+    nxt.request(p, tile + tstep, n, l15, g4);
     const int64_t row = tile * 16 + l15;
     const bool ok = row < n;
     f32x4 x[4];
-    auto load4 = [&](const float* base, int t) -> f32x4 {
-      if (!ok) return (f32x4){0.f, 0.f, 0.f, 0.f};
-      if (p.in_bf16) {
-        const uint2 h = *reinterpret_cast<const uint2*>(reinterpret_cast<const uint16_t*>(base) + row * 64 + 16 * t + 4 * g4);
-        return (f32x4){bf2f(h.x & 0xFFFFu), bf2f(h.x >> 16), bf2f(h.y & 0xFFFFu), bf2f(h.y >> 16)};
-      }
-      return *reinterpret_cast<const f32x4*>(base + row * 64 + 16 * t + 4 * g4);
-    };
-#pragma unroll
-    for (int t = 0; t < 4; ++t) x[t] = load4(p.x, t);
-    if (p.lw) {
-      f32x4 r[4], l[4];
-#pragma unroll
-      for (int t = 0; t < 4; ++t) r[t] = load4(p.lres, t);
+#pragma unroll
+    for (int t = 0; t < 4; ++t) x[t] = cur.wide(cur.x[t]);
+    if constexpr (LAT != 0) {
+      f32x4 l[4];
       mlp_layer<64, 4>(lat, x, lane, l);
 #pragma unroll
-      for (int t = 0; t < 4; ++t) x[t] = l[t] + r[t];
+      for (int t = 0; t < 4; ++t) x[t] = l[t] + cur.wide(cur.r[t]);
     }
     float guard = 0.f;
     bool outside = false;
@@ -315,7 +413,7 @@
       lhs_layer<64, 6>(lh_frags + LHS_DW0 * 2 * 64, x, lane, wi0, h);
 #pragma unroll
       for (int nt = 0; nt < 6; ++nt) {
-        const f32x4 b = *reinterpret_cast<const f32x4*>(p.db0 + 16 * nt + 4 * g4);
+        const f32x4 b = *reinterpret_cast<const f32x4*>(s_bias + LH_B_DB0 + 16 * nt + 4 * g4);
 #pragma unroll
         for (int r = 0; r < 4; ++r) h[nt][r] = fmaxf(h[nt][r] + b[r], 0.f);
       }
@@ -323,7 +421,7 @@
       float ss = 0.f;
 #pragma unroll
       for (int nt = 0; nt < 8; ++nt) {
-        const f32x4 b = *reinterpret_cast<const f32x4*>(p.db1 + 16 * nt + 4 * g4);
+        const f32x4 b = *reinterpret_cast<const f32x4*>(s_bias + LH_B_DB1 + 16 * nt + 4 * g4);
 #pragma unroll
         for (int r = 0; r < 4; ++r) {
           o[nt][r] += b[r];
@@ -345,17 +443,17 @@
       lhs_layer<64, 2>(lh_frags + LHS_KW0 * 2 * 64, x, lane, wi2, h);
 #pragma unroll
       for (int nt = 0; nt < 2; ++nt) {
-        const f32x4 b = *reinterpret_cast<const f32x4*>(p.kb0 + 16 * nt + 4 * g4);
+        const f32x4 b = *reinterpret_cast<const f32x4*>(s_bias + LH_B_KB0 + 16 * nt + 4 * g4);
 #pragma unroll
         for (int r = 0; r < 4; ++r) h[nt][r] = fmaxf(h[nt][r] + b[r], 0.f);
       }
       lhs_layer<32, 1>(lh_frags + LHS_KW1 * 2 * 64, h, lane, wi3, o);
       if (ok && g4 == 0) {
         guard += split_nonfinite(o[0][0]) + split_nonfinite(o[0][1]) + split_nonfinite(o[0][2]);
-        const float ox = p.ignore_offsets ? 0.f : tanhf(o[0][0] + p.kb1[0]);
-        const float oy = p.ignore_offsets ? 0.f : tanhf(o[0][1] + p.kb1[1]);
-        const float oz = p.ignore_offsets ? 0.f : tanhf(o[0][2] + p.kb1[2]);
-        keypoint_position(p.keys[row], p.level, p.cb, ox, oy, oz, p.mode, p.s0, p.s1, p.s2, p.out_kp + row * 3);
+        const float ox = p.ignore_offsets ? 0.f : tanhf(o[0][0] + s_bias[LH_B_KB1 + 0]);
+        const float oy = p.ignore_offsets ? 0.f : tanhf(o[0][1] + s_bias[LH_B_KB1 + 1]);
+        const float oz = p.ignore_offsets ? 0.f : tanhf(o[0][2] + s_bias[LH_B_KB1 + 2]);
+        keypoint_position(cur.key, p.level, p.cb, ox, oy, oz, p.mode, p.s0, p.s1, p.s2, p.out_kp + row * 3);
       }
     }
     {
@@ -363,30 +461,31 @@
       lhs_layer<64, 2>(lh_frags + LHS_SW0 * 2 * 64, x, lane, wi4, h);
 #pragma unroll
       for (int nt = 0; nt < 2; ++nt) {
-        const f32x4 b = *reinterpret_cast<const f32x4*>(p.sb0 + 16 * nt + 4 * g4);
+        const f32x4 b = *reinterpret_cast<const f32x4*>(s_bias + LH_B_SB0 + 16 * nt + 4 * g4);
 #pragma unroll
         for (int r = 0; r < 4; ++r) h[nt][r] = fmaxf(h[nt][r] + b[r], 0.f);
       }
       lhs_layer<32, 1>(lh_frags + LHS_SW1 * 2 * 64, h, lane, wi5, o);
       if (ok && g4 == 0) {
         guard += split_nonfinite(o[0][0]);
-        p.out_sigma[row] = apply_act(o[0][0] + p.sb1[0], ACT_SOFTPLUS);
+        p.out_sigma[row] = apply_act(o[0][0] + s_bias[LH_B_SB1], ACT_SOFTPLUS);
       }
     }
     if (ok && (outside || guard != 0.f) && q.flags) split_raise(q.flags);
+    cur = nxt;
   }
 }
 
 int local_heads_forward(const float* x, int64_t n, const int32_t* n_dev, const float* const* w ,
                         const uint64_t* keys, int level, int cb, int mode, const float* step, int ignore_offsets,
                         float* out_desc, float* out_kp, float* out_sigma, hipStream_t stream, const float* lateral_w,
-                        const float* lateral_res, int in_bf16, const void* split_pack, int32_t* flags) {
+                        const float* lateral_res, int in_bf16, const void* split_pack, int32_t* flags, const float* lateral_pack) {
   if (n == 0) return EGONN_OK;
   EGONN_REQUIRE((lateral_w == nullptr) == (lateral_res == nullptr), EGONN_ERR_INVALID, "local heads: lateral kernel and residual go together");
+  EGONN_REQUIRE(!lateral_pack || lateral_w, EGONN_ERR_INVALID, "local heads: packed lateral fragments without the lateral");
   LocalHeadsArgs a;
   a.x = x; a.n = n; a.n_dev = n_dev;
-  a.lw = lateral_w; a.lres = lateral_res;
-  a.in_bf16 = in_bf16 ? 1 : 0;
+  a.lw = lateral_w; a.lres = lateral_res; a.lpk = lateral_pack;
   EGONN_REQUIRE(!in_bf16 || lateral_w, EGONN_ERR_INVALID, "local heads: bf16 input rows only through the fused lateral");
   a.dw0 = w[0]; a.db0 = w[1]; a.dw1 = w[2]; a.db1 = w[3];
   a.kw0 = w[4]; a.kb0 = w[5]; a.kw1 = w[6]; a.kb1 = w[7];
@@ -395,29 +494,38 @@
   a.s0 = step[0]; a.s1 = mode ? step[1] : step[0]; a.s2 = mode ? step[2] : step[0];
   a.out_desc = out_desc; a.out_kp = out_kp; a.out_sigma = out_sigma;
   const int64_t tiles = cdiv(n, 16);
-  const size_t lds = (size_t)(LH_FRAGS + (lateral_w ? 16 : 0)) * 64 * sizeof(f32x4);
-  static AttrOnce attr_done;
-  if (attr_done.need()) {
-    HIP_CHECK(hipFuncSetAttribute(reinterpret_cast<const void*>(&local_heads_kernel), hipFuncAttributeMaxDynamicSharedMemorySize, 160 * 1024));
-    attr_done.mark(); 
-  }
+  const int lat = lateral_w ? (lateral_pack ? 2 : 1) : 0;
   const unsigned grid = (unsigned)std::min<int64_t>(cdiv(tiles, LH_WAVES), 256);
+  auto launch = [&](auto kernel, const auto& args, int frags, AttrOnce& once) -> int {
+    if (once.need()) {
+      HIP_CHECK(hipFuncSetAttribute(reinterpret_cast<const void*>(kernel), hipFuncAttributeMaxDynamicSharedMemorySize, 160 * 1024));
+      once.mark();
+    }
+    const size_t lds = (size_t)(frags + (lat ? 16 : 0)) * 64 * sizeof(f32x4) + LH_BIAS_LDS * sizeof(float);
+    hipLaunchKernelGGL(kernel, dim3(grid), dim3(LH_THREADS), lds, stream, args);
+    HIP_CHECK(hipGetLastError());
+    return EGONN_OK;
+  };
+  static AttrOnce once[2][5];
+  const int form = lat == 0 ? 0 : 2 * lat - 1 + (in_bf16 ? 1 : 0);
   if (split_pack) {
-    static AttrOnce attr2;
-    if (attr2.need()) {
-      HIP_CHECK(hipFuncSetAttribute(reinterpret_cast<const void*>(&local_heads_split_kernel), hipFuncAttributeMaxDynamicSharedMemorySize, 160 * 1024));
-      attr2.mark();
-    }
     LocalHeadsSplitArgs q;
     q.a = a; q.pack = split_pack; q.flags = flags;
-    const size_t lds2 = (size_t)(LHS_FRAGS * 2 + (lateral_w ? 16 : 0)) * 64 * sizeof(f32x4);
-    hipLaunchKernelGGL(local_heads_split_kernel, dim3(grid), dim3(LH_WAVES * 64), lds2, stream, q);
-    HIP_CHECK(hipGetLastError());
-    return EGONN_OK;
-  }
-  hipLaunchKernelGGL(local_heads_kernel, dim3(grid), dim3(LH_WAVES * 64), lds, stream, a);
-  HIP_CHECK(hipGetLastError());
-  return EGONN_OK;
+    switch (form) {
+      case 0: return launch(&local_heads_split_kernel<0, false>, q, LHS_FRAGS * 2, once[1][0]);
+      case 1: return launch(&local_heads_split_kernel<1, false>, q, LHS_FRAGS * 2, once[1][1]);
+      case 2: return launch(&local_heads_split_kernel<1, true>, q, LHS_FRAGS * 2, once[1][2]);
+      case 3: return launch(&local_heads_split_kernel<2, false>, q, LHS_FRAGS * 2, once[1][3]);
+      default: return launch(&local_heads_split_kernel<2, true>, q, LHS_FRAGS * 2, once[1][4]);
+    }
+  }
+  switch (form) {
+    case 0: return launch(&local_heads_kernel<0, false>, a, LH_FRAGS, once[0][0]);
+    case 1: return launch(&local_heads_kernel<1, false>, a, LH_FRAGS, once[0][1]);
+    case 2: return launch(&local_heads_kernel<1, true>, a, LH_FRAGS, once[0][2]);
+    case 3: return launch(&local_heads_kernel<2, false>, a, LH_FRAGS, once[0][3]);
+    default: return launch(&local_heads_kernel<2, true>, a, LH_FRAGS, once[0][4]);
+  }
 }
 
 __device__ static inline uint32_t sigma_bits(float v) {
diff --git a/egonn_amd/csrc/kernels.h b/egonn_amd/csrc/kernels.h
--- a/egonn_amd/csrc/kernels.h
+++ b/egonn_amd/csrc/kernels.h
@@ -178,7 +178,8 @@
 int local_heads_forward(const float* x, int64_t n, const int32_t* n_dev, const float* const* w, const uint64_t* keys,
                         int level, int cb, int mode, const float* step, int ignore_offsets, float* out_desc, float* out_kp,
                         float* out_sigma, hipStream_t stream, const float* lateral_w = nullptr, const float* lateral_res = nullptr,
-                        int in_bf16 = 0, const void* split_pack = nullptr, int32_t* flags = nullptr);
+                        int in_bf16 = 0, const void* split_pack = nullptr, int32_t* flags = nullptr,
+                        const float* lateral_pack = nullptr);
 size_t local_heads_pack_bytes();
 int local_heads_pack(const float* const* w6_dev, void* out, hipStream_t stream);
 int select_topk(const float* sigma, const int32_t* boff_dev, int B, int k, const float* kp, const float* desc, int dc,
diff --git a/egonn_amd/csrc/model.hip b/egonn_amd/csrc/model.hip
--- a/egonn_amd/csrc/model.hip
+++ b/egonn_amd/csrc/model.hip
@@ -860,7 +860,8 @@
     if (!switches().no_fused_lateral && LOCAL_CH == 64) {
       EGONN_TRY(local_heads_forward(reinterpret_cast<const float*>(x[3]), n3, cnt + 3, hw, P.lv[3].keys, 3, P.coord_bits, quant_mode,
                                     step, (flags & EGONN_FLAG_IGNORE_KP_REGRESSOR) ? 1 : 0, out_desc, out_kp, out_sigma, st,
-                                    m->l1x1[3], reinterpret_cast<const float*>(u3), bf16, lh_pack, c->dev_fp16_flag));
+                                    m->l1x1[3], reinterpret_cast<const float*>(u3), bf16, lh_pack, c->dev_fp16_flag,
+                                    static_cast<const float*>(m->pk_l1x1[3])));
       return EGONN_OK;
     }
     WALLOC(float, l3, n3 * LOCAL_CH);
@@ -1029,6 +1030,46 @@
   return global_tail(r, pk, g5, rows_capacity, n_dev, row_offsets, batch_size, (Pooling)pooling, p, form == 1, gh, gd, partial, out, st);
 }
 
+static size_t debug_heads_span() {
+  return align_up(local_heads_pack_bytes(), 256) + align_up(6 * sizeof(float*), 256) + align_up((size_t)LOCAL_CH * LOCAL_CH * 4, 256) + 1024;
+}
+API int64_t egonn_debug_local_heads_scratch_bytes(void) { return (int64_t)debug_heads_span(); }
+API int egonn_debug_local_heads(const void* x, int64_t rows_capacity, const int32_t* n_dev, const float* const weights[12],
+                                const uint64_t* keys, const float* lateral_w, const void* lateral_res, int lateral_packed, int in_bf16,
+                                int exact, int coord_bits, float quant_step, float* out_desc, float* out_kp, float* out_sigma,
+                                int32_t* flags, void* scratch, int64_t scratch_bytes, void* stream) {
+  EGONN_REQUIRE(x && n_dev && weights && keys && out_desc && out_kp && out_sigma && scratch, EGONN_ERR_INVALID,
+                "debug_local_heads: null pointer");
+  for (int i = 0; i < 12; ++i) EGONN_REQUIRE(weights[i], EGONN_ERR_INVALID, "debug_local_heads: weights[%d] is null", i);
+  EGONN_REQUIRE(rows_capacity >= 1 && rows_capacity < (1ll << 31) / LOCAL_DIM, EGONN_ERR_INVALID,
+                "debug_local_heads: rows_capacity=%lld outside [1, 2^31 / %d)", (long long)rows_capacity, LOCAL_DIM);
+  EGONN_REQUIRE((lateral_w == nullptr) == (lateral_res == nullptr), EGONN_ERR_INVALID,
+                "debug_local_heads: lateral kernel and residual rows go together");
+  EGONN_REQUIRE(lateral_w || (!lateral_packed && !in_bf16), EGONN_ERR_INVALID,
+                "debug_local_heads: packed fragments / bf16 rows only with a lateral");
+  EGONN_REQUIRE(coord_bits > 3 && coord_bits <= 21, EGONN_ERR_INVALID, "debug_local_heads: coord_bits=%d outside (3, 21]", coord_bits);
+  const size_t need = debug_heads_span();
+  EGONN_REQUIRE(scratch_bytes >= (int64_t)need && ((uintptr_t)scratch & 255) == 0, EGONN_ERR_INVALID,
+                "debug_local_heads: scratch needs %lld bytes, 256-byte aligned", (long long)need);
+  hipStream_t st = (hipStream_t)stream;
+  Arena ws = Arena::view(scratch, need);
+  char* pack = ws.alloc<char>(local_heads_pack_bytes());
+  const float** ptrs = ws.alloc<const float*>(6);
+  float* lpk = ws.alloc<float>((size_t)LOCAL_CH * LOCAL_CH);
+  EGONN_REQUIRE(pack && ptrs && lpk, EGONN_ERR_STATE, "debug_local_heads: scratch span too small");
+  if (!exact) {
+    const float* hp[6] = {weights[0], weights[2], weights[4], weights[6], weights[8], weights[10]};
+    HIP_CHECK(hipMemcpyAsync(ptrs, hp, sizeof(hp), hipMemcpyHostToDevice, st));
+    HIP_CHECK(hipStreamSynchronize(st));
+    EGONN_TRY(local_heads_pack(ptrs, pack, st));
+  }
+  if (lateral_w && lateral_packed) EGONN_TRY(dense_pack_frags(lateral_w, 0, LOCAL_CH, LOCAL_CH, lpk, st));
+  const float step[3] = {quant_step, quant_step, quant_step};
+  return local_heads_forward(static_cast<const float*>(x), rows_capacity, n_dev, weights, keys, 3, coord_bits, 0, step, 0, out_desc,
+                             out_kp, out_sigma, st, lateral_w, static_cast<const float*>(lateral_res), in_bf16, exact ? nullptr : pack,
+                             flags, (lateral_w && lateral_packed) ? lpk : nullptr);
+}
+
 API int egonn_forward_level_features(egonn_ctx* c, int level, float* out, int channels, void* stream) {
   REQUIRE_PLAN(c);
   EGONN_REQUIRE(level >= 0 && level < EGONN_NUM_LEVELS && c->level_feat[level], EGONN_ERR_STATE,
diff --git a/include/egonn_hip.h b/include/egonn_hip.h
--- a/include/egonn_hip.h
+++ b/include/egonn_hip.h
@@ -40,6 +40,11 @@
 int egonn_debug_global_tail(const float* g5, const int32_t* row_offsets, int batch_size, int64_t rows_capacity, const int32_t* n_dev,
                             const float* w0, const float* b0, const float* w1, const float* b1, const float* p, int pooling, int form,
                             float* partial, float* out, void* scratch, int64_t scratch_bytes, void* stream);
+int64_t egonn_debug_local_heads_scratch_bytes(void);
+int egonn_debug_local_heads(const void* x, int64_t rows_capacity, const int32_t* n_dev, const float* const weights[12],
+                            const uint64_t* keys, const float* lateral_w, const void* lateral_res, int lateral_packed, int in_bf16,
+                            int exact, int coord_bits, float quant_step, float* out_desc, float* out_kp, float* out_sigma,
+                            int32_t* flags, void* scratch, int64_t scratch_bytes, void* stream);
 
 int egonn_voxelize(egonn_ctx* ctx, const float* points, const int64_t* scan_offsets, int batch_size, int quant_mode,
                    const float* step, void* stream);
```

New measurement: 23590, median of 6. About the same (+0.9%).
